# BogdanDIA/gr-dvbt

Measured on AMD Instinct MI355X. Metric: RX Msamples/s (baseband in -> TS out), higher is better.
Workload: dtype u8 (Viterbi/RS) + f32 (front end)

## Files before the change

gr_dvbt_amd/csrc/dvbt_blocks.inc:

```

namespace {

struct PinBuf {
  void *p = nullptr; size_t cap = 0;
  int reserve(size_t n) { if (n <= cap) return DVBT_OK; if (p) (void)hipHostFree(p); p = nullptr; cap = 0; HIPCHK(hipHostMalloc(&p, n + 64)); cap = n; return DVBT_OK; }
  ~PinBuf() { if (p) (void)hipHostFree(p); }
};
struct BlockCtx {
  hipStream_t s = nullptr; DevBuf din, dout, aux; PinBuf pin_in, pin_out;
  struct Pending { void *host; size_t off, bytes; };
  std::vector<Pending> pending; size_t pin_in_used = 0, pin_out_used = 0;
  int init() { int r = need_device(); if (r) return r; HIPCHK(hipStreamCreate(&s)); return DVBT_OK; }
  static bool is_pinned(const void *host)
  {
    hipPointerAttribute_t a;
    if (hipPointerGetAttributes(&a, host) != hipSuccess) { (void)hipGetLastError(); return false; }
    return a.type == hipMemoryTypeHost;
  }
  int put(DevBuf &b, const void *host, size_t bytes, size_t offset = 0)
  {
    int r = b.reserve(offset + bytes); if (r) return r;
    if (!bytes) return DVBT_OK;
    if (is_pinned(host)) { HIPCHK(hipMemcpyAsync((char *)b.p + offset, host, bytes, hipMemcpyHostToDevice, s)); return DVBT_OK; }
    if (pin_in_used + bytes > pin_in.cap) {
// ... 177 lines not shown
  if (n > 4096) return fail(DVBT_ERR_CAPACITY, "at most 4096 items per call");
  WCHK(h->c.aux.reserve(64 * 4096 * 4));
  HIPCHK(hipMemcpyAsync((char *)h->c.aux.p + slot, h->idx.data(), (size_t)n * 4, hipMemcpyHostToDevice, s));
  InnerParams ip; memset(&ip, 0, sizeof ip); ip.payload = (int)P; ip.m = 4;
  hipLaunchKernelGGL(inner_kernel<2>, dim3(n), dim3(INNER_THREADS), inner_lds_bytes(P), s, (const float2 *)nullptr, (const uint8_t *)din, ip,
                     (const RxState *)nullptr, n, (const int *)((char *)h->c.aux.p + slot), (const float2 *)nullptr, (const unsigned char *)nullptr,
                     (const uint16_t *)h->T.H, (const uint16_t *)h->T.Hinv, (uint8_t *)nullptr, (uint8_t *)nullptr, (uint8_t *)dout);
  return DVBT_OK;
}
extern "C" int dvbt_symbol_inner_interleaver_work(dvbt_symbol_inner_interleaver *h, int nout, int nin, const void *in, void *out, dvbt_sideband *sb)
{
  if (!h || !in || !out) return fail(DVBT_ERR_INVALID, "null argument");
  sb_begin(sb);
  int n = nout < nin ? nout : nin; if (n <= 0) return 0;
  size_t P = h->p.nsize;
  WCHK(sym_indices(h, n, sb));
  WCHK(h->c.put(h->c.din, in, (size_t)n * P)); WCHK(h->c.dout.reserve((size_t)n * P));
  WCHK(sym_run(h, n, h->c.din.p, h->c.dout.p, h->c.s));
  WCHK(h->c.get(out, h->c.dout.p, (size_t)n * P)); WCHK(h->c.sync());
  if (sb) sb->n_consumed = n;
  return n;
}
extern "C" int dvbt_symbol_inner_interleaver_work_device(dvbt_symbol_inner_interleaver *h, int nout, int nin, const void *in, void *out, dvbt_sideband *sb, void *stream)
{
  if (!h || !in || !out) return fail(DVBT_ERR_INVALID, "null argument");
  sb_begin(sb);
  int n = nout < nin ? nout : nin; if (n <= 0) return 0;
  WCHK(sym_indices(h, n, sb));
  WCHK(sym_run(h, n, in, out, pick(stream, h->c)));
  if (sb) sb->n_consumed = n;
  return n;
}
extern "C" void dvbt_symbol_inner_interleaver_destroy(dvbt_symbol_inner_interleaver *h) { delete h; }

struct dvbt_bit_inner_deinterleaver { dvbt_bit_inner_deinterleaver_params p; BlockCtx c; Dims d; };
extern "C" int dvbt_bit_inner_deinterleaver_create(const dvbt_bit_inner_deinterleaver_params *p, dvbt_bit_inner_deinterleaver **out)
{
  BLK_CREATE_PROLOGUE(dvbt_bit_inner_deinterleaver);
  h->p = *p;
  h->d = make_dims(p->constellation, p->hierarchy, 0, 0, p->transmission_mode);
  if (!h->d.valid || p->nsize <= 0 || p->nsize % 126 || p->nsize > 49152) BLK_FAIL(DVBT_ERR_INVALID, "nsize must be a positive multiple of 126");
  if (p->hierarchy != DVBT_NH && h->d.m == 2) BLK_FAIL(DVBT_ERR_INVALID, "hierarchical QPSK does not exist (the reference's constructor divides by d_v - 2 = 0)");
  *out = h; return DVBT_OK;
}
extern "C" int dvbt_bit_inner_deinterleaver_forecast(const dvbt_bit_inner_deinterleaver *, int n, int *req) { if (req) *req = n; return DVBT_OK; }
static void bit_run(dvbt_bit_inner_deinterleaver *h, int n, const void *din, void *dout, hipStream_t s, void *dout_lp = nullptr)
{
  const size_t P = h->p.nsize;
  InnerParams ip; memset(&ip, 0, sizeof ip); ip.payload = (int)P; ip.m = h->d.m; ip.hier = h->p.hierarchy != DVBT_NH ? 1 : 0;
  hipLaunchKernelGGL(inner_kernel<4>, dim3(n), dim3(INNER_THREADS), inner_lds_bytes(P), s, (const float2 *)nullptr, (const uint8_t *)din, ip,
                     (const RxState *)nullptr, n, (const int *)nullptr, (const float2 *)nullptr, (const unsigned char *)nullptr,
                     (const uint16_t *)nullptr, (const uint16_t *)nullptr, (uint8_t *)nullptr, (uint8_t *)nullptr, (uint8_t *)dout, (uint8_t *)dout_lp);
}
extern "C" int dvbt_bit_inner_deinterleaver_work_hier(dvbt_bit_inner_deinterleaver *h, int nout, int nin, const void *in, void *out_hp, void *out_lp, dvbt_sideband *sb)
{
  if (!h || !in || !out_hp || !out_lp) return fail(DVBT_ERR_INVALID, "null argument");
  if (h->p.hierarchy == DVBT_NH) return fail(DVBT_ERR_STATE, "a non-hierarchical bit_inner_deinterleaver has one output");
  sb_begin(sb);
  int n = nout < nin ? nout : nin; if (n <= 0) return 0;
  size_t P = h->p.nsize;
  WCHK(h->c.put(h->c.din, in, (size_t)n * P)); WCHK(h->c.dout.reserve((size_t)n * P)); WCHK(h->c.aux.reserve((size_t)n * P));
  bit_run(h, n, h->c.din.p, h->c.dout.p, h->c.s, h->c.aux.p);
  WCHK(h->c.get(out_hp, h->c.dout.p, (size_t)n * P)); WCHK(h->c.get(out_lp, h->c.aux.p, (size_t)n * P)); WCHK(h->c.sync());
  if (sb) sb->n_consumed = n;
  return n;
}
extern "C" int dvbt_bit_inner_deinterleaver_work_hier_device(dvbt_bit_inner_deinterleaver *h, int nout, int nin, const void *in, void *out_hp, void *out_lp, dvbt_sideband *sb, void *stream)
{
  if (!h || !in || !out_hp || !out_lp) return fail(DVBT_ERR_INVALID, "null argument");
  if (h->p.hierarchy == DVBT_NH) return fail(DVBT_ERR_STATE, "a non-hierarchical bit_inner_deinterleaver has one output");
  sb_begin(sb);
  int n = nout < nin ? nout : nin; if (n <= 0) return 0;
  bit_run(h, n, in, out_hp, pick(stream, h->c), out_lp);
  if (sb) sb->n_consumed = n;
  return n;
}
extern "C" int dvbt_bit_inner_deinterleaver_work(dvbt_bit_inner_deinterleaver *h, int nout, int nin, const void *in, void *out, dvbt_sideband *sb)
{
  if (!h || !in || !out) return fail(DVBT_ERR_INVALID, "null argument");
  sb_begin(sb);
  int n = nout < nin ? nout : nin; if (n <= 0) return 0;
  size_t P = h->p.nsize;
  WCHK(h->c.put(h->c.din, in, (size_t)n * P)); WCHK(h->c.dout.reserve((size_t)n * P));
  bit_run(h, n, h->c.din.p, h->c.dout.p, h->c.s);
  WCHK(h->c.get(out, h->c.dout.p, (size_t)n * P)); WCHK(h->c.sync());
  if (sb) sb->n_consumed = n;
  return n;
}
extern "C" int dvbt_bit_inner_deinterleaver_work_device(dvbt_bit_inner_deinterleaver *h, int nout, int nin, const void *in, void *out, dvbt_sideband *sb, void *stream)
{
  if (!h || !in || !out) return fail(DVBT_ERR_INVALID, "null argument");
  sb_begin(sb);
  int n = nout < nin ? nout : nin; if (n <= 0) return 0;
  bit_run(h, n, in, out, pick(stream, h->c));
  if (sb) sb->n_consumed = n;
  return n;
}
extern "C" void dvbt_bit_inner_deinterleaver_destroy(dvbt_bit_inner_deinterleaver *h) { delete h; }

struct dvbt_viterbi_decoder {
  dvbt_viterbi_decoder_params p; BlockCtx c; Dims d; VitParams vp;
  size_t hist = 0; long long in_total = 0, steps = 0; int d_init = 0;
  static constexpr size_t kTail = 8192;
  VitProof proof; int *carry = nullptr; int cur = 0; bool have_carry = false; long long grid0 = 0;
  ~dvbt_viterbi_decoder() { if (carry) (void)hipFree(carry); }
};
extern "C" int dvbt_viterbi_decoder_create(const dvbt_viterbi_decoder_params *p, dvbt_viterbi_decoder **out)
{
  BLK_CREATE_PROLOGUE(dvbt_viterbi_decoder);
  h->p = *p;
  h->d = make_dims(p->constellation, p->hierarchy, p->code_rate, 0, 0);
  if (!h->d.valid || p->bsize <= 0 || (2 * h->d.k * p->bsize) % 16 || (p->bsize * h->d.n) % h->d.m || (p->bsize * h->d.k) % 8)
    BLK_FAIL(DVBT_ERR_INVALID, "bsize must make bsize*n/m and bsize*k/8 integral and 2*k*bsize a multiple of 16");
  h->vp = make_vit_params(h->d, p->bsize, 11 * V3_BLK);
  if (hipMalloc((void **)&h->carry, 2 * V3_SLOT * sizeof(int)) != hipSuccess) BLK_FAIL(DVBT_ERR_HIP, "hipMalloc (viterbi_decoder carry)");
  BLK_CHK(h->proof.reserve(256));
  *out = h; return DVBT_OK;
}
extern "C" int dvbt_viterbi_decoder_forecast(const dvbt_viterbi_decoder *h, int n, int *req)
{ if (!h || !req) return DVBT_ERR_INVALID; *req = n * 8 * h->d.n / (h->d.k * h->d.m); return DVBT_OK; }
static int viterbi_call(dvbt_viterbi_decoder *h, int nout, int nin, const void *in, void *out, dvbt_sideband *sb, bool dev, hipStream_t s)
{
  sb_begin(sb);
  const int d_nout = h->vp.d_nbits / 16, d_nsym = h->vp.d_nsymbols;
  int nblocks = nout / d_nout;
  if (nblocks * d_nsym > nin) nblocks = nin / d_nsym;
  if (nblocks <= 0) return 0;
  const dvbt_tag *t = find_tag(sb, DVBT_TAG_SUPERFRAME_START, 0, (int64_t)nblocks * d_nsym);
  if (t) {
    h->d_init = 0; h->steps = 0; h->in_total = 0; h->hist = 0; h->have_carry = false; h->grid0 = 0;
    if (t->rel_offset > 0) { if (sb) sb->n_consumed = (int)t->rel_offset; return 0; }
    HIPCHK(hipMemsetAsync(h->proof.ctl + V3_CTL_ACC, 0, 3 * sizeof(int), s));
  }
  const size_t nbytes = (size_t)nblocks * d_nsym, hist = h->hist;
  WCHK(h->c.din.reserve_keep(dvbt_viterbi_decoder::kTail + nbytes + 64, hist, s));
  if (dev) WCHK(h->c.put_dev(h->c.din, in, nbytes, hist, s)); else { HIPCHK(hipMemcpyAsync((char *)h->c.din.p + hist, in, nbytes, hipMemcpyHostToDevice, s)); }
  const long long in_base = h->in_total - (long long)hist;
  long long out_lo = h->steps / 8 - h->d.ntb; if (out_lo < 0) out_lo = 0;
  h->steps += (long long)nblocks * (h->vp.d_nbits / 2);
  h->in_total += (long long)nbytes;
  long long out_hi = h->steps / 8 - h->d.ntb; if (out_hi < 0) out_hi = 0;
  const long long produced = out_hi - out_lo;
  if (produced > 0) {
    uint8_t *o = (uint8_t *)out;
    if (!dev) { WCHK(h->c.dout.reserve((size_t)produced)); o = (uint8_t *)h->c.dout.p; }
    const int B = h->vp.chunk_bytes;
    const long long g0 = h->have_carry ? h->grid0 : 0, chunks = (out_hi - g0 + B - 1) / B;
    if (chunks + 2 > h->proof.cap) { HIPCHK(hipStreamSynchronize(s)); int acc[3]; HIPCHK(hipMemcpy(acc, h->proof.ctl + V3_CTL_ACC, sizeof acc, hipMemcpyDeviceToHost));
                                     WCHK(h->proof.reserve(2 * chunks + 2)); HIPCHK(hipMemcpy(h->proof.ctl + V3_CTL_ACC, acc, sizeof acc, hipMemcpyHostToDevice)); }
    V3Aux ax = h->proof.aux();
    ax.grid0 = g0; ax.carry_in = h->have_carry ? h->carry + h->cur * V3_SLOT : nullptr;
    const long long b0_last = g0 + (chunks - 1) * B;
    ax.carry_rel = (int)((out_hi - b0_last) / V3_BLK) * V3_BLK; ax.carry_out = h->carry + (h->cur ^ 1) * V3_SLOT;
    launch_viterbi(s, (const uint8_t *)h->c.din.p, o, (const RxState *)nullptr, h->steps, h->vp, in_base, out_lo, produced, &ax, VIT_REPAIR);
    h->cur ^= 1; h->have_carry = true; h->grid0 = b0_last + ax.carry_rel;
    if (!dev) WCHK(h->c.get(out, h->c.dout.p, (size_t)produced));
  }
  {
    const size_t total = hist + nbytes, keep = total < dvbt_viterbi_decoder::kTail ? total : dvbt_viterbi_decoder::kTail;
    if (total > keep) {
      WCHK(h->c.aux.reserve(dvbt_viterbi_decoder::kTail));
      HIPCHK(hipMemcpyAsync(h->c.aux.p, (const char *)h->c.din.p + total - keep, keep, hipMemcpyDeviceToDevice, s));
      HIPCHK(hipMemcpyAsync(h->c.din.p, h->c.aux.p, keep, hipMemcpyDeviceToDevice, s));
    }
    h->hist = keep;
  }
  if (!dev) WCHK(h->c.sync());
  if (h->d_init == 0) { add_tag(sb, 0, DVBT_TAG_SUPERFRAME_START, 1); h->d_init = 1; }
  if (sb) sb->n_consumed = (int)nbytes;
  return (int)produced;
}
extern "C" int dvbt_viterbi_decoder_work(dvbt_viterbi_decoder *h, int nout, int nin, const void *in, void *out, dvbt_sideband *sb)
{
  if (!h || !in || !out) return fail(DVBT_ERR_INVALID, "null argument");
  return viterbi_call(h, nout, nin, in, out, sb, false, h->c.s);
}
extern "C" int dvbt_viterbi_decoder_work_device(dvbt_viterbi_decoder *h, int nout, int nin, const void *in, void *out, dvbt_sideband *sb, void *stream)
{
  if (!h || !in || !out) return fail(DVBT_ERR_INVALID, "null argument");
  return viterbi_call(h, nout, nin, in, out, sb, true, pick(stream, h->c));
}
extern "C" int dvbt_viterbi_decoder_set_warm_windows(dvbt_viterbi_decoder *h, int windows)
{
  if (!h) return fail(DVBT_ERR_INVALID, "null handle");
  if (windows == 0) windows = V3_WARM;
  if (windows < 2 * V3_BLK || windows > 576 || windows % V3_BLK != 0) return fail(DVBT_ERR_INVALID, "warm-up must be 0 (default) or a multiple of 24 in [48, 576]");
  h->vp.warm = windows;
  return DVBT_OK;
}
extern "C" int dvbt_viterbi_decoder_proof(dvbt_viterbi_decoder *h, dvbt_viterbi_proof *out)
{
  if (!h || !out) return fail(DVBT_ERR_INVALID, "null argument");
  int acc[3] = {0, 0, 0};
  HIPCHK(hipMemcpy(acc, h->proof.ctl + V3_CTL_ACC, sizeof acc, hipMemcpyDeviceToHost));
  out->chunks = acc[0]; out->decoded_again = acc[1]; out->sequential = acc[2]; out->not_proven = -1;
  return DVBT_OK;
}
extern "C" void dvbt_viterbi_decoder_destroy(dvbt_viterbi_decoder *h) { delete h; }

struct dvbt_convolutional_deinterleaver { dvbt_convolutional_deinterleaver_params p; BlockCtx c; size_t hist = 0; long long pos = 0; };
extern "C" int dvbt_convolutional_deinterleaver_create(const dvbt_convolutional_deinterleaver_params *p, dvbt_convolutional_deinterleaver **out)
{
  BLK_CREATE_PROLOGUE(dvbt_convolutional_deinterleaver);
  h->p = *p;
  if (p->I != 12 || p->M != 17 || p->blocks != 136) BLK_FAIL(DVBT_ERR_INVALID, "only the DVB-T outer interleaver I=12, M=17, blocks=136 (every RX flowgraph; assert at convolutional_deinterleaver_impl.cc:68)");
  *out = h; return DVBT_OK;
}
extern "C" int dvbt_convolutional_deinterleaver_forecast(const dvbt_convolutional_deinterleaver *h, int n, int *req)
{ if (!h || !req) return DVBT_ERR_INVALID; *req = n * h->p.I * h->p.blocks; return DVBT_OK; }
static int convdeint_call(dvbt_convolutional_deinterleaver *h, int nout, int nin, const void *in, void *out, dvbt_sideband *sb, bool dev, hipStream_t s)
{
  sb_begin(sb);
  const int item = h->p.I * h->p.blocks;
  int n = nout & ~1;
  if ((long long)n * item > nin) n = (nin / item) & ~1;
  if (n <= 0) return 0;
  const dvbt_tag *t = find_tag(sb, DVBT_TAG_SUPERFRAME_START, 0, (int64_t)n * item);
  if (t && t->rel_offset > 0) { if (sb) sb->n_consumed = (int)t->rel_offset; return 0; }
  const size_t nbytes = (size_t)n * item, hist = h->hist, keep_max = 2244;
  WCHK(h->c.din.reserve_keep(keep_max + nbytes + 64, hist, s));
  if (dev) WCHK(h->c.put_dev(h->c.din, in, nbytes, hist, s)); else { HIPCHK(hipMemcpyAsync((char *)h->c.din.p + hist, in, nbytes, hipMemcpyHostToDevice, s)); }
  uint8_t *o = (uint8_t *)out;
  if (!dev) { WCHK(h->c.dout.reserve(nbytes)); o = (uint8_t *)h->c.dout.p; }
  hipLaunchKernelGGL(conv_deint_kernel, dim3(512), dim3(256), 0, s, (const uint8_t *)h->c.din.p, (long long)hist, h->pos, (long long)nbytes, o);
  if (!dev) WCHK(h->c.get(out, h->c.dout.p, nbytes));
  h->pos += (long long)nbytes;
  {
    const size_t total = hist + nbytes, keep = total < keep_max ? total : keep_max;
    if (total > keep) {
      WCHK(h->c.aux.reserve(keep_max));
      HIPCHK(hipMemcpyAsync(h->c.aux.p, (const char *)h->c.din.p + total - keep, keep, hipMemcpyDeviceToDevice, s));
      HIPCHK(hipMemcpyAsync(h->c.din.p, h->c.aux.p, keep, hipMemcpyDeviceToDevice, s));
    }
    h->hist = keep;
  }
  if (!dev) WCHK(h->c.sync());
  if (sb) sb->n_consumed = (int)nbytes;
  return n;
}
extern "C" int dvbt_convolutional_deinterleaver_work(dvbt_convolutional_deinterleaver *h, int nout, int nin, const void *in, void *out, dvbt_sideband *sb)
{
  if (!h || !in || !out) return fail(DVBT_ERR_INVALID, "null argument");
  return convdeint_call(h, nout, nin, in, out, sb, false, h->c.s);
}
extern "C" int dvbt_convolutional_deinterleaver_work_device(dvbt_convolutional_deinterleaver *h, int nout, int nin, const void *in, void *out, dvbt_sideband *sb, void *stream)
{
  if (!h || !in || !out) return fail(DVBT_ERR_INVALID, "null argument");
  return convdeint_call(h, nout, nin, in, out, sb, true, pick(stream, h->c));
}
extern "C" void dvbt_convolutional_deinterleaver_destroy(dvbt_convolutional_deinterleaver *h) { delete h; }

struct dvbt_reed_solomon_dec { dvbt_reed_solomon_dec_params p; BlockCtx c; Tables T; int *cnt = nullptr; ~dvbt_reed_solomon_dec() { if (cnt) (void)hipFree(cnt); } };
extern "C" int dvbt_reed_solomon_dec_create(const dvbt_reed_solomon_dec_params *p, dvbt_reed_solomon_dec **out)
{
  BLK_CREATE_PROLOGUE(dvbt_reed_solomon_dec);
  h->p = *p;
  if (p->p != 2 || p->m != 8 || p->gfpoly != 0x11d || p->n != 255 || p->k != 239 || p->t != 8 || p->s != 51 || p->blocks <= 0)
    BLK_FAIL(DVBT_ERR_INVALID, "only RS(255,239,t=8) over GF(2^8)/0x11d shortened by 51 (the DVB-T outer code)");
  BLK_CHK(h->T.build_rs());
  if (hipMalloc((void **)&h->cnt, 8) != hipSuccess || hipMemset(h->cnt, 0, 8) != hipSuccess) BLK_FAIL(DVBT_ERR_HIP, "hipMalloc");
  *out = h; return DVBT_OK;
}
extern "C" int dvbt_reed_solomon_dec_forecast(const dvbt_reed_solomon_dec *, int n, int *req) { if (req) *req = n; return DVBT_OK; }
static void rs_run(dvbt_reed_solomon_dec *h, long long words, const void *din, void *dout, hipStream_t s)
{
  hipLaunchKernelGGL(deint_rs_kernel, dim3((unsigned)((words + 63) / 64)), dim3(64), 0, s, (const uint8_t *)din, (uint8_t *)nullptr,
                     (uint8_t *)dout, (RxState *)nullptr, words, 1, 0ll, h->T.rs_tables(), h->p.oracle_compat, h->cnt, h->cnt + 1);
}
extern "C" int dvbt_reed_solomon_dec_work(dvbt_reed_solomon_dec *h, int nout, int nin, const void *in, void *out, dvbt_sideband *sb)
{
  if (!h || !in || !out) return fail(DVBT_ERR_INVALID, "null argument");
  sb_begin(sb);
  int n = nout < nin ? nout : nin; if (n <= 0) return 0;
  long long words = (long long)n * h->p.blocks;
  WCHK(h->c.put(h->c.din, in, (size_t)words * 204)); WCHK(h->c.dout.reserve((size_t)words * 188));
  rs_run(h, words, h->c.din.p, h->c.dout.p, h->c.s);
  WCHK(h->c.get(out, h->c.dout.p, (size_t)words * 188)); WCHK(h->c.sync());
  if (sb) sb->n_consumed = n;
  return n;
}
extern "C" int dvbt_reed_solomon_dec_work_device(dvbt_reed_solomon_dec *h, int nout, int nin, const void *in, void *out, dvbt_sideband *sb, void *stream)
{
  if (!h || !in || !out) return fail(DVBT_ERR_INVALID, "null argument");
  sb_begin(sb);
  int n = nout < nin ? nout : nin; if (n <= 0) return 0;
  rs_run(h, (long long)n * h->p.blocks, in, out, pick(stream, h->c));
  if (sb) sb->n_consumed = n;
  return n;
}
extern "C" void dvbt_reed_solomon_dec_destroy(dvbt_reed_solomon_dec *h) { delete h; }

struct dvbt_energy_descramble { dvbt_energy_descramble_params p; BlockCtx c; Tables T; int d_index = 0; RxState *dstate = nullptr; unsigned ring = 0; ~dvbt_energy_descramble() { if (dstate) (void)hipFree(dstate); } };
extern "C" int dvbt_energy_descramble_create(const dvbt_energy_descramble_params *p, dvbt_energy_descramble **out)
{
  BLK_CREATE_PROLOGUE(dvbt_energy_descramble);
  h->p = *p;
  BLK_CHK(h->T.build_rs());
  *out = h; return DVBT_OK;
}
extern "C" int dvbt_energy_descramble_forecast(const dvbt_energy_descramble *, int n, int *req) { if (req) *req = 4 * (n / 1504); return DVBT_OK; }
static int descramble_call(dvbt_energy_descramble *h, int nout, int nin, const void *in, void *out, dvbt_sideband *sb, bool dev, hipStream_t s)
{
  sb_begin(sb);
  nout -= nout % (4 * 1504);
  if (nout <= 0 || nin < nout / 1504) return 0;
  uint8_t probe[16];
  if (dev) {
// ... 261 lines not shown
```

gr_dvbt_amd/csrc/dvbt_hip.hip:

```cpp
#include <hip/hip_runtime.h>
#include <cstdio>
#include <cstdarg>
#include <cstdlib>
#include <cstring>
#include <string>
#include <vector>
#include <map>
#include <deque>
#include <algorithm>
#include "../../include/dvbt_hip.h"
#include "dvbt_tables.hpp"
#include "ts_ring.hpp"
#include "k_frontend.hpp"
#include "k_drift.hpp"
#include "k_backend.hpp"
#include "k_symbol8k.hpp"
#include "k_symbol2k.hpp"
#include "k_resample.hpp"
#include "k_viterbi3.hpp"
#include "k_soft4.hpp"
#include "k_tx.hpp"
#include "k_txblocks.hpp"

using namespace dvbt;
// ... 31 lines not shown
  o->fft_length = d.N; o->cp_length = d.cp; o->Kmax = d.Kmax; o->payload_length = d.payload; o->zeros_on_left = d.zl;
  o->m = d.m; o->cr_k = d.k; o->cr_n = d.n; o->norm = d.norm; o->ntraceback = d.ntb; o->info_bits_per_symbol = d.info_bits_per_symbol;
  return DVBT_OK;
}

template <class T> static int upload(const std::vector<T> &v, T **dptr)
{
  HIPCHK(hipMalloc((void **)dptr, v.size() * sizeof(T) + 16));
  HIPCHK(hipMemcpy(*dptr, v.data(), v.size() * sizeof(T), hipMemcpyHostToDevice));
  return DVBT_OK;
}

struct DevBuf {
  void *p = nullptr; size_t cap = 0;
  int reserve(size_t n) { if (n <= cap) return DVBT_OK; if (p) (void)hipFree(p); p = nullptr; cap = 0; HIPCHK(hipMalloc(&p, n + 64)); cap = n; return DVBT_OK; }
  int reserve_keep(size_t n, size_t keep, hipStream_t st)
  {
    if (n <= cap) return DVBT_OK;
    void *q = nullptr; HIPCHK(hipMalloc(&q, n + 64));
    if (p && keep) HIPCHK(hipMemcpyAsync(q, p, keep, hipMemcpyDeviceToDevice, st));
    if (p) { HIPCHK(hipStreamSynchronize(st)); (void)hipFree(p); }
    p = q; cap = n; return DVBT_OK;
  }
  ~DevBuf() { if (p) (void)hipFree(p); }
};

struct Tables {
  Dims d;
  float2 *tw = nullptr; uint16_t *perm = nullptr;
  int16_t *cpilot = nullptr, *tps = nullptr; float *known = nullptr, *pref = nullptr;
  uint16_t *pay_c = nullptr, *pay_L = nullptr, *pay_R = nullptr, *tps_L = nullptr, *tps_R = nullptr;
  uint16_t *pil_k = nullptr, *pay_Li = nullptr, *pay_Ri = nullptr, *tps_Li = nullptr, *tps_Ri = nullptr; uint8_t *pay_d = nullptr, *tps_d = nullptr; int np[4] = {0, 0, 0, 0};
  uint16_t *tps_bch = nullptr;
  uint32_t *pay_pack = nullptr;
  uint16_t *H = nullptr, *Hinv = nullptr; float2 *points = nullptr; uint8_t *label_tab = nullptr; int nlev = 0; float inv_step = 0.f, guard = 0.f, hshift = 0.f;
  uint8_t *mul_alpha = nullptr, *gexp = nullptr, *glog = nullptr, *prbs = nullptr;
  bool front = false, inner = false, rs = false;

  int build_fft(int N)
  {
    std::vector<float> tw_h = fft_twiddles(N);
    std::vector<float2> t2(N);
    for (int i = 0; i < N; i++) t2[i] = make_float2(tw_h[2 * i], tw_h[2 * i + 1]);
    int r = upload(t2, &tw); if (r) return r;
    return upload(fft_out_perm(N), &perm);
  }
  int build_front()
  {
    std::vector<int> c = cpilot_table(d), t = tps_table(d);
    std::vector<int16_t> c16(c.begin(), c.end()), t16(t.begin(), t.end());
    std::vector<float> pr = pilot_ref_table(d), kn(d.n_cp - 1);
    for (int i = 0; i + 1 < d.n_cp; i++) { float df = pr[c[i + 1]] - pr[c[i]]; kn[i] = df * df; }
    int r;
    if ((r = upload(c16, &cpilot)) || (r = upload(t16, &tps)) || (r = upload(pr, &pref)) || (r = upload(kn, &known))) return r;
    std::vector<uint16_t> pc, pl, prr, tl, trr, pk((size_t)4 * DEMOD_NP, 0), pli, pri, tli, tri;
    std::vector<uint8_t> pd, td;
    std::vector<uint32_t> pp;
    for (int s = 0; s < 4; s++) {
      PatternTables pt = pattern_tables(d, s);
      if ((int)pt.pay_c.size() != d.payload) return fail(DVBT_ERR_INVALID, "payload carrier table size mismatch");
      if ((int)pt.pil_k.size() > DEMOD_NP) return fail(DVBT_ERR_INVALID, "estimation carrier table overflow");
      np[s] = (int)pt.pil_k.size();
      for (size_t i = 0; i < pt.pil_k.size(); i++) pk[(size_t)s * DEMOD_NP + i] = (uint16_t)(pt.pil_k[i] | (pr[pt.pil_k[i]] < 0.f ? 0x8000 : 0));
      pli.insert(pli.end(), pt.pay_Li.begin(), pt.pay_Li.end()); pri.insert(pri.end(), pt.pay_Ri.begin(), pt.pay_Ri.end());
      pd.insert(pd.end(), pt.pay_d.begin(), pt.pay_d.end());
      for (size_t i = 0; i < pt.pay_c.size(); i++) pp.push_back((uint32_t)pt.pay_c[i] | ((uint32_t)pt.pay_Li[i] << 13) | ((uint32_t)pt.pay_d[i] << 23));
      tli.insert(tli.end(), pt.tps_Li.begin(), pt.tps_Li.end()); tri.insert(tri.end(), pt.tps_Ri.begin(), pt.tps_Ri.end());
      td.insert(td.end(), pt.tps_d.begin(), pt.tps_d.end());
      pc.insert(pc.end(), pt.pay_c.begin(), pt.pay_c.end()); pl.insert(pl.end(), pt.pay_L.begin(), pt.pay_L.end());
      prr.insert(prr.end(), pt.pay_R.begin(), pt.pay_R.end()); tl.insert(tl.end(), pt.tps_L.begin(), pt.tps_L.end());
      trr.insert(trr.end(), pt.tps_R.begin(), pt.tps_R.end());
    }
    if ((r = upload(pc, &pay_c)) || (r = upload(pl, &pay_L)) || (r = upload(prr, &pay_R)) || (r = upload(tl, &tps_L)) || (r = upload(trr, &tps_R))) return r;
    if ((r = upload(pk, &pil_k)) || (r = upload(pli, &pay_Li)) || (r = upload(pri, &pay_Ri)) || (r = upload(pd, &pay_d)) || (r = upload(tli, &tps_Li)) ||
        (r = upload(tri, &tps_Ri)) || (r = upload(td, &tps_d)) || (r = upload(pp, &pay_pack))) return r;
    if ((r = upload(tps_bch_table_host(), &tps_bch))) return r;
    front = true;
    return DVBT_OK;
  }
  int build_inner(float gain)
  {
    int r;
    if (!H) {
      std::vector<uint16_t> h = symbol_H(d), hi(h.size());
      for (size_t q = 0; q < h.size(); q++) hi[h[q]] = (uint16_t)q;
      if ((r = upload(h, &H)) || (r = upload(hi, &Hinv))) return r;
    }
    std::vector<float> p = constellation_points(d, gain);
    std::vector<float2> p2(64, make_float2(0.f, 0.f));
    for (int i = 0; i < d.csize; i++) p2[i] = make_float2(p[2 * i], p[2 * i + 1]);
    std::vector<uint8_t> lab(64, 0);
    nlev = 0; hshift = 0.f;
    if (gain > 0.f) {
      int n = 1 << (d.m / 2);
      float step = 2.0f * gain * d.norm;
      const float sh = (float)(d.alpha - 1) * gain * d.norm;
      bool ok = true;
      for (int i = 0; i < d.csize && ok; i++) {
        const float ux = p2[i].x - (p2[i].x > 0 ? sh : -sh), uy = p2[i].y - (p2[i].y > 0 ? sh : -sh);
        float fi = ux / step + 0.5f * (n - 1), fq = uy / step + 0.5f * (n - 1);
        int ii = (int)std::lround(fi), qq = (int)std::lround(fq);
        if (ii < 0 || ii >= n || qq < 0 || qq >= n || std::fabs(fi - ii) > 1e-3f || std::fabs(fq - qq) > 1e-3f) ok = false;
        else lab[ii * 8 + qq] = (uint8_t)i;
      }
      if (ok) { nlev = n; inv_step = 1.0f / step; guard = 1.0e4f * step; hshift = sh; }
    }
    if (points) { (void)hipFree(points); points = nullptr; }
    if (label_tab) { (void)hipFree(label_tab); label_tab = nullptr; }
    if ((r = upload(p2, &points)) || (r = upload(lab, &label_tab))) return r;
    inner = true;
    return DVBT_OK;
  }
  InnerParams inner_params(int payload) const { InnerParams ip; ip.payload = payload; ip.m = d.m; ip.csize = d.csize; ip.nlev = nlev; ip.inv_step = inv_step; ip.guard = guard;
                                                  ip.hshift = hshift; ip.hier = d.hierarchy != 0 ? 1 : 0; return ip; }
  int build_rs()
  {
    std::vector<uint8_t> ex(512), lg(256), mul = rs_division_table();
    gf_tables(ex.data(), lg.data());
    int r;
    if ((r = upload(ex, &gexp)) || (r = upload(lg, &glog)) || (r = upload(mul, &mul_alpha)) || (r = upload(energy_prbs(), &prbs))) return r;
    rs = true;
    return DVBT_OK;
  }
  DemodTables demod_tables() const { DemodTables T; T.cpilot = cpilot; T.known_diff = known; T.tps = tps; T.pilot_ref = pref;
    T.pay_c = pay_c; T.pay_L = pay_L; T.pay_R = pay_R; T.tps_L = tps_L; T.tps_R = tps_R;
    T.pil_k = pil_k; for (int i = 0; i < 4; i++) T.np[i] = np[i];
    T.pay_Li = pay_Li; T.pay_Ri = pay_Ri; T.pay_d = pay_d; T.tps_Li = tps_Li; T.tps_Ri = tps_Ri; T.tps_d = tps_d; T.pay_pack = pay_pack; return T; }
  RsTables rs_tables() const { RsTables T; T.div_tab = mul_alpha; T.gexp = gexp; T.glog = glog; return T; }
  ~Tables()
  {
    void *all[] = {tw, perm, cpilot, tps, known, pref, pay_c, pay_L, pay_R, tps_L, tps_R, pil_k, pay_Li, pay_Ri, pay_d, tps_Li, tps_Ri, tps_d, pay_pack, tps_bch, H, Hinv, points, label_tab, mul_alpha, gexp, glog, prbs};
    for (void *q : all) if (q) (void)hipFree(q);
  }
};

#define V3_NTB_SWITCH(ntb, CALL) switch (ntb) { case 5: CALL(5); break; case 9: CALL(9); break; case 10: CALL(10); break; case 15: CALL(15); break; default: CALL(24); break; }
struct VitProof {
  int *snap = nullptr, *ctl = nullptr; long long cap = 0;
  int reserve(long long chunks)
  {
    if (chunks <= cap) return DVBT_OK;
    if (snap) (void)hipFree(snap); if (ctl) (void)hipFree(ctl);
    snap = ctl = nullptr; cap = 0;
    HIPCHK(hipMalloc((void **)&snap, v3_snap_words(chunks) * sizeof(int))); HIPCHK(hipMalloc((void **)&ctl, v3_ctl_words(chunks) * sizeof(int)));
    HIPCHK(hipMemset(ctl, 0, v3_ctl_words(chunks) * sizeof(int)));
    cap = chunks; return DVBT_OK;
  }
  V3Aux aux() const { V3Aux a; memset(&a, 0, sizeof a); a.snap = snap; a.ctl = ctl; a.cap = cap; a.carry_rel = -1; return a; }
  ~VitProof() { if (snap) (void)hipFree(snap); if (ctl) (void)hipFree(ctl); }
};
enum { VIT_PLAIN = -1, VIT_REPAIR = 0, VIT_REPAIR_COUNT = 1, VIT_PROOF_ONLY = 2, VIT_FORCE_SEQ = 3, VIT_FORCE_CONFLICT = 4 };
constexpr unsigned V3_REPAIR_GRID = 64;

static void launch_viterbi(hipStream_t s, const uint8_t *in, uint8_t *out, const RxState *st, long long steps_fixed, const VitParams &vp,
                           long long in_base, long long out_lo, long long max_out_bytes, const V3Aux *ax = nullptr, int mode = VIT_PLAIN)
{
  const bool proof = ax && mode != VIT_PLAIN;
  const long long grid0 = proof ? ax->grid0 : out_lo;
  long long chunks = (out_lo + max_out_bytes - grid0 + vp.chunk_bytes - 1) / vp.chunk_bytes;
  if (chunks < 1) chunks = 1;
  const dim3 grid((unsigned)((chunks + 4 * V3_WGW - 1) / (4 * V3_WGW))), blk(64 * V3_WGW);
  V3Aux none; memset(&none, 0, sizeof none);
  if (proof) {
    V3Aux a = *ax;
    if (mode == VIT_FORCE_CONFLICT) { a.debug = 1; mode = VIT_REPAIR_COUNT; }
    const dim3 cgrid((unsigned)((chunks + 255) / 256));
    if (vp.warm == V3_WARM) {
#define V3_CALL(N) hipLaunchKernelGGL((viterbi3_kernel<N, V3_WARM, 1>), grid, blk, 0, s, in, out, st, steps_fixed, vp, a, in_base, out_lo)
      V3_NTB_SWITCH(vp.ntb, V3_CALL)
#undef V3_CALL
    } else {
#define V3_CALL(N) hipLaunchKernelGGL((viterbi3_kernel<N, 0, 1>), grid, blk, 0, s, in, out, st, steps_fixed, vp, a, in_base, out_lo)
      V3_NTB_SWITCH(vp.ntb, V3_CALL)
#undef V3_CALL
    }
    if (chunks <= V3_FIX_SMALL && mode != VIT_PROOF_ONLY) {
#define V3_CALL(N) hipLaunchKernelGGL(viterbi_fix_kernel<N>, dim3(1), blk, 0, s, in, out, st, steps_fixed, vp, a, in_base, out_lo, mode == VIT_FORCE_SEQ ? 1 : 0)
      V3_NTB_SWITCH(vp.ntb, V3_CALL)
#undef V3_CALL
      if (mode != VIT_REPAIR) {
        hipLaunchKernelGGL(viterbi_check_kernel, dim3(1), dim3(256), 0, s, a, st, steps_fixed, vp, 1);
        hipLaunchKernelGGL(viterbi_count_kernel, cgrid, dim3(256), 0, s, a, st, steps_fixed, vp);
      }
      return;
    }
    hipLaunchKernelGGL(viterbi_check_kernel, cgrid, dim3(256), 0, s, a, st, steps_fixed, vp, 0);
    if (mode == VIT_REPAIR || mode == VIT_REPAIR_COUNT) {
#define V3_CALL(N) hipLaunchKernelGGL(viterbi_repair_kernel<N>, dim3(V3_REPAIR_GRID), blk, 0, s, in, out, st, steps_fixed, vp, a, in_base, out_lo)
      V3_NTB_SWITCH(vp.ntb, V3_CALL)
#undef V3_CALL
    }
    if (mode != VIT_PROOF_ONLY) {
      const int force = mode == VIT_FORCE_SEQ ? 1 : 0;
#define V3_CALL(N) hipLaunchKernelGGL(viterbi_repair_seq_kernel<N>, dim3(1), dim3(64), 0, s, in, out, st, steps_fixed, vp, a, in_base, out_lo, force)
      V3_NTB_SWITCH(vp.ntb, V3_CALL)
#undef V3_CALL
    }
    if (mode != VIT_REPAIR) {
      hipLaunchKernelGGL(viterbi_check_kernel, dim3(1), dim3(256), 0, s, a, st, steps_fixed, vp, 1);
      hipLaunchKernelGGL(viterbi_count_kernel, cgrid, dim3(256), 0, s, a, st, steps_fixed, vp);
    }
    return;
  }
  if (vp.warm != V3_WARM) {
#define V3_CALL(N) hipLaunchKernelGGL((viterbi3_kernel<N, 0, 0>), grid, blk, 0, s, in, out, st, steps_fixed, vp, none, in_base, out_lo)
    V3_NTB_SWITCH(vp.ntb, V3_CALL)
#undef V3_CALL
    return;
  }
#define V3_CALL(N) hipLaunchKernelGGL((viterbi3_kernel<N, V3_WARM, 0>), grid, blk, 0, s, in, out, st, steps_fixed, vp, none, in_base, out_lo)
  V3_NTB_SWITCH(vp.ntb, V3_CALL)
#undef V3_CALL
}

__global__ void tail_patch_kernel(RxState *st, long long items)
{
  st->n_rs_items = items; st->n_rs_words = items * 8; st->stream_rs_items = items;
  st->rs_fail = 0; st->rs_corr = 0; st->rs_list_n = 0; st->sym_off = 0;
}

static FrontParams make_front_params(const Dims &d, float snr_db)
{
  FrontParams p; memset(&p, 0, sizeof p);
  p.N = d.N; p.cp = d.cp; p.K = d.K; p.zl = d.zl; p.payload = d.payload; p.n_cp = d.n_cp; p.n_tps = d.n_tps; p.fi_start = d.fi_start;
  p.R = ACQ_R;
  float snr = (float)pow(10, snr_db / 10.0);
  float rho = (float)(snr / (snr + 1.0));
  p.half_rho = (float)(rho / 2.0);
  return p;
}
static int set_lds(const void *fn, size_t bytes)
{
  if (bytes > 48 * 1024) HIPCHK(hipFuncSetAttribute(fn, hipFuncAttributeMaxDynamicSharedMemorySize, (int)bytes));
  return DVBT_OK;
}

enum { ST_ACQ = 0, ST_FFT, ST_DEMOD, ST_INNER, ST_VIT, ST_RS, ST_END, ST_COUNT };
static const char *kStageNames[] = {"acq", "fft", "demod", "inner", "viterbi", "rs"};

struct ResamplerDesign {
  int ri = 0, rd = 0, nt = 0; std::vector<float> taps; float *br = nullptr;
  int build(int interp, int decim)
  {
    if (interp <= 0 || decim <= 0) return fail(DVBT_ERR_INVALID, "bad resampler ratio");
    taps = resampler_taps(interp, decim, ri, rd);
    std::vector<float> b = resampler_branches(taps, ri, nt);
    if ((long long)ri * nt > RS_MAX_BRANCH_FLOATS || 256ll * rd / ri + nt + 2 > RS_TILE_IN) return fail(DVBT_ERR_INVALID, "resampler ratio outside the supported range");
    HIPCHK(hipMalloc((void **)&br, b.size() * sizeof(float)));
    HIPCHK(hipMemcpy(br, b.data(), b.size() * sizeof(float), hipMemcpyHostToDevice));
    return DVBT_OK;
  }
  ~ResamplerDesign() { if (br) (void)hipFree(br); }
};

struct dvbt_rx {
  dvbt_rx_params prm; Dims d; Tables T; FrontParams fp; VitParams vp;
  hipStream_t own_stream = nullptr, cur_stream = nullptr;
  hipStream_t front_stream = nullptr; hipEvent_t front_ev[2] = {nullptr, nullptr};
  size_t max_samples = 0; int max_calls = 0;
  float2 *d_iq = nullptr;
  ResamplerDesign rsd; float2 *rs_iq = nullptr; size_t chain_max = 0;
  AcqState *acq_carry = nullptr; bool use_carry = false;
  float2 *g_init = nullptr; float *l_init = nullptr; float2 *g_trk = nullptr; float *l_trk = nullptr;
  SymMeta *meta = nullptr; RxState *st = nullptr, *st_host = nullptr; TpsState *tps_state = nullptr;
  static constexpr int NCTX = 3;
  RxState *st_ctx[NCTX] = {nullptr, nullptr, nullptr}; SymMeta *meta_ctx[NCTX] = {nullptr, nullptr, nullptr}; int ctx = 0;
  int *trk_flags_ctx[NCTX] = {nullptr, nullptr, nullptr}, *sym_ticket_ctx[NCTX] = {nullptr, nullptr, nullptr}, *drift_flags_ctx[NCTX] = {nullptr, nullptr, nullptr}; RxState *st_host_ctx[NCTX] = {nullptr, nullptr, nullptr};
  hipStream_t aux_stream = nullptr; hipEvent_t aux_ev = nullptr;
  int *trk_cp_a = nullptr, *trk_cp_b = nullptr, *trk_flags = nullptr; float *trk_eps = nullptr; TpsEdge *tps_edges = nullptr;
  int *centre = nullptr, *anchor_pos = nullptr;
  float2 *acq_tap = nullptr, *fft_out = nullptr, *eq = nullptr, *tpsval = nullptr; SymInfo *info = nullptr; int *maj = nullptr, *sym_index = nullptr;
  uint8_t *labels = nullptr, *symdeint_tap = nullptr, *bitdeint = nullptr, *vit = nullptr, *deint_tap = nullptr, *rs_out = nullptr, *ts_out = nullptr;
  uint8_t *bitdeint_lp = nullptr;
  uint8_t *bd_log = nullptr; std::vector<dvbt_period_tap> plog; size_t plog_bytes = 0;
  VitProof vproof; bool vit_checked = false;
  size_t vit_cap = 0; RsDefer *rs_defer = nullptr; int rs_defer_cap = 0;
  unsigned long long *rs_sync = nullptr;
  unsigned soft_grid = 0;
  float *csi = nullptr; int8_t *soft_a = nullptr; uint16_t *soft_tab = nullptr; unsigned *soft_scratch = nullptr;
  int timing = 0;
  bool pending = false;
  hipEvent_t ev[ST_COUNT]; double acc_ms[ST_COUNT] = {0}; long n_timed = 0; bool ev_ready = false, ev_recorded = false;
  dvbt_rx_report last; bool have_last = false;
  dvbt_rx_cut cut = {0, 0, 0};
  float2 *tps_prev = nullptr, *tps_prev_snap[2] = {nullptr, nullptr}; TpsState *tps_snap[2] = {nullptr, nullptr};  DescrRun *descr_runs = nullptr; int *descr_nruns = nullptr;
  int n_periods = 1; size_t seg_offset = 0;
  std::vector<dvbt_lock_period> periods;
  DriftBufs drift = {nullptr, nullptr, nullptr, nullptr, nullptr, nullptr, nullptr, nullptr}; double *drift_mem = nullptr;
  struct GraphEntry { const void *iq; size_t n; hipStream_t s; long long sym_off; int delay, phase; hipGraphExec_t exec; };
  std::vector<GraphEntry> graphs;
  int ncu = 256;
  long long n_small = 0, n_general = 0;
  int sym_grid = 512;
  int *sym_ticket = nullptr;
};

constexpr long long kVitMaxChunk = 3000;
static int vit_chunk_bytes(const dvbt_rx *h, long long max_vit);

static void drop_graphs(dvbt_rx *h)
{
  for (auto &ge : h->graphs) if (ge.exec) (void)hipGraphExecDestroy(ge.exec);
  h->graphs.clear();
}

static void rx_free(dvbt_rx *h)
{
  void *all[] = {h->bd_log, h->bitdeint_lp, h->st_ctx[0], h->st_ctx[1], h->st_ctx[2], h->meta_ctx[0], h->meta_ctx[1], h->meta_ctx[2], h->tps_prev_snap[0], h->tps_prev_snap[1], h->tps_snap[0], h->tps_snap[1], h->csi, h->soft_a, h->soft_tab, h->soft_scratch, h->rs_defer, h->rs_sync, h->drift_mem, h->drift.delta, h->drift_flags_ctx[0], h->drift_flags_ctx[1], h->drift_flags_ctx[2], h->tps_prev, h->descr_runs, h->descr_nruns, h->centre, h->anchor_pos, h->sym_ticket_ctx[0], h->sym_ticket_ctx[1], h->sym_ticket_ctx[2], h->tps_edges, h->trk_cp_a, h->trk_cp_b, h->trk_flags_ctx[0], h->trk_flags_ctx[1], h->trk_flags_ctx[2], h->trk_eps, h->d_iq, h->rs_iq, h->acq_carry, h->g_init, h->l_init, h->g_trk, h->l_trk, h->tps_state, h->acq_tap, h->fft_out, h->eq, h->tpsval,
                 h->info, h->maj, h->sym_index, h->labels, h->symdeint_tap, h->bitdeint, h->vit, h->deint_tap, h->rs_out, h->ts_out};
  for (void *q : all) if (q) (void)hipFree(q);
  for (auto &ge : h->graphs) if (ge.exec) (void)hipGraphExecDestroy(ge.exec);
  for (int i = 0; i < dvbt_rx::NCTX; i++) if (h->st_host_ctx[i]) (void)hipHostFree(h->st_host_ctx[i]);
  if (h->aux_ev) (void)hipEventDestroy(h->aux_ev);
  if (h->aux_stream) (void)hipStreamDestroy(h->aux_stream);
  if (h->ev_ready) for (int i = 0; i < ST_COUNT; i++) (void)hipEventDestroy(h->ev[i]);
  if (h->own_stream) (void)hipStreamDestroy(h->own_stream);
  for (int i = 0; i < 2; i++) if (h->front_ev[i]) (void)hipEventDestroy(h->front_ev[i]);
  if (h->front_stream) (void)hipStreamDestroy(h->front_stream);
  delete h;
}

extern "C" int dvbt_rx_create(const dvbt_rx_params *p, dvbt_rx **out)
{
  if (!p || !out) return fail(DVBT_ERR_INVALID, "null argument");
  int r = need_device(); if (r) return r;
  Dims d = make_dims(p->constellation, p->hierarchy, p->code_rate, p->guard_interval, p->transmission_mode);
  if (!d.valid) return fail(DVBT_ERR_INVALID, "bad DVB-T parameters");
  if (p->viterbi_bsize <= 0 || (2 * d.k * p->viterbi_bsize) % 16 != 0 || (p->viterbi_bsize * d.n) % d.m != 0)
    return fail(DVBT_ERR_INVALID, "viterbi_bsize must make bsize*n/m integral and 2*k*bsize a multiple of 16");
  if (d.hierarchy != 0 && d.m == 2) return fail(DVBT_ERR_INVALID, "hierarchical QPSK does not exist (the reference's bit_inner_deinterleaver divides by d_v - 2 = 0 in its constructor)");
  if (d.hierarchy != 0 && p->soft_decision) return fail(DVBT_ERR_INVALID, "soft decisions are built for the non-hierarchical modes");
  if (p->hier_stream < 0 || p->hier_stream > 1) return fail(DVBT_ERR_INVALID, "hier_stream must be 0 (HP) or 1 (LP)");
  if (p->viterbi_warm_windows != 0 && (p->viterbi_warm_windows < 2 * V3_BLK || p->viterbi_warm_windows > V3_WARM_MAX || p->viterbi_warm_windows % V3_BLK != 0))
    return fail(DVBT_ERR_INVALID, "viterbi_warm_windows must be 0 (default) or a multiple of 24 in [48, 1152]");
  if (p->viterbi_warm_windows != 0 && p->soft_decision) return fail(DVBT_ERR_INVALID, "viterbi_warm_windows applies to the hard-decision decoder");
  if (p->viterbi_verify < VIT_PLAIN || p->viterbi_verify > VIT_FORCE_CONFLICT) return fail(DVBT_ERR_INVALID, "viterbi_verify must lie in [-1, 4]");
  if (p->viterbi_verify > 0 && p->soft_decision) return fail(DVBT_ERR_INVALID, "viterbi_verify applies to the hard-decision decoder");
  HIPCHK(hipSetDevice(p->device));
  dvbt_rx *h = new dvbt_rx();
  h->prm = *p; h->d = d; h->T.d = d;
  size_t chain_max = p->max_samples;
  if (p->resample_interp > 0 || p->resample_decim > 0) {
    int r2 = h->rsd.build(p->resample_interp, p->resample_decim); if (r2) { delete h; return r2; }
    chain_max = (size_t)(((unsigned long long)p->max_samples * h->rsd.ri + h->rsd.rd - 1) / h->rsd.rd);
  }
  if (chain_max < (size_t)(2 * d.N + d.cp + 16)) { delete h; return fail(DVBT_ERR_INVALID, "max_samples smaller than one acquisition window"); }
  h->chain_max = chain_max;
  h->fp = make_front_params(d, p->snr_db);
  int cb = p->viterbi_chunk_bytes > 0 ? p->viterbi_chunk_bytes : 768;
  h->vp = make_vit_params(d, p->viterbi_bsize, cb);
  if (p->viterbi_warm_windows > 0) h->vp.warm = p->viterbi_warm_windows;
  h->max_samples = p->max_samples;
  h->max_calls = (int)((chain_max - (2 * d.N + d.cp + 16)) / (d.N + d.cp) + 1);
#define RXCHK(x) do { int r_ = (x); if (r_) { rx_free(h); return r_; } } while (0)
#define RXHIP(x) do { hipError_t e_ = (x); if (e_ != hipSuccess) { g_err = std::string(#x) + ": " + hipGetErrorString(e_); rx_free(h); return DVBT_ERR_HIP; } } while (0)
  RXCHK(h->T.build_fft(d.N)); RXCHK(h->T.build_front()); RXCHK(h->T.build_inner(1.0f)); RXCHK(h->T.build_rs());
  RXHIP(hipStreamCreate(&h->own_stream));
  if (p->front_priority) {
    int least = 0, greatest = 0; RXHIP(hipDeviceGetStreamPriorityRange(&least, &greatest));
    RXHIP(hipStreamCreateWithPriority(&h->front_stream, hipStreamNonBlocking, greatest));
    for (int i = 0; i < 2; i++) RXHIP(hipEventCreateWithFlags(&h->front_ev[i], hipEventDisableTiming));
  }
  if (h->rsd.ri) RXHIP(hipMalloc((void **)&h->rs_iq, sizeof(float2) * (chain_max + 16)));
  const size_t C = (size_t)h->max_calls, N = d.N, P = d.payload;
  RXHIP(hipMalloc((void **)&h->g_init, sizeof(float2) * ACQ_INIT_TRIES_MAX * N)); RXHIP(hipMalloc((void **)&h->l_init, sizeof(float) * ACQ_INIT_TRIES_MAX * N));
  RXHIP(hipMalloc((void **)&h->g_trk, sizeof(float2) * C * 2 * ACQ_R)); RXHIP(hipMalloc((void **)&h->l_trk, sizeof(float) * C * 2 * ACQ_R));
  for (int i = 0; i < dvbt_rx::NCTX; i++) { RXHIP(hipMalloc((void **)&h->meta_ctx[i], sizeof(SymMeta) * C)); RXHIP(hipMalloc((void **)&h->st_ctx[i], sizeof(RxState))); RXHIP(hipMemset(h->st_ctx[i], 0, sizeof(RxState))); }
  h->meta = h->meta_ctx[0]; h->st = h->st_ctx[0]; h->ctx = 0;
  RXHIP(hipMalloc((void **)&h->trk_cp_a, sizeof(int) * C)); RXHIP(hipMalloc((void **)&h->trk_cp_b, sizeof(int) * C));
  RXHIP(hipMalloc((void **)&h->trk_eps, sizeof(float) * C));
  for (int i = 0; i < dvbt_rx::NCTX; i++) { RXHIP(hipMalloc((void **)&h->trk_flags_ctx[i], sizeof(int) * 16)); RXHIP(hipMemset(h->trk_flags_ctx[i], 0, sizeof(int) * 16)); }
  h->trk_flags = h->trk_flags_ctx[0];
  RXHIP(hipStreamCreate(&h->aux_stream)); RXHIP(hipEventCreateWithFlags(&h->aux_ev, hipEventDisableTiming));
  RXHIP(hipMalloc((void **)&h->tps_prev, sizeof(float2) * d.n_tps)); RXHIP(hipMemset(h->tps_prev, 0, sizeof(float2) * d.n_tps));
  for (int i = 0; i < 2; i++) { RXHIP(hipMalloc((void **)&h->tps_prev_snap[i], sizeof(float2) * d.n_tps)); RXHIP(hipMalloc((void **)&h->tps_snap[i], sizeof(TpsState))); }
  RXHIP(hipMalloc((void **)&h->descr_runs, sizeof(DescrRun) * DESCR_MAX_RUNS)); RXHIP(hipMalloc((void **)&h->descr_nruns, sizeof(int)));
  RXHIP(hipMalloc((void **)&h->centre, sizeof(int) * (C + 1))); RXHIP(hipMalloc((void **)&h->anchor_pos, sizeof(int) * (C / ACQ_ANCHOR + 4)));
  RXHIP(hipMalloc((void **)&h->tps_edges, sizeof(TpsEdge) * (C / TPS_SEG + 2)));
  for (int i = 0; i < dvbt_rx::NCTX; i++) { RXHIP(hipHostMalloc((void **)&h->st_host_ctx[i], sizeof(RxState))); memset(h->st_host_ctx[i], 0, sizeof(RxState)); }
  h->st_host = h->st_host_ctx[0];
  RXHIP(hipMalloc((void **)&h->acq_carry, sizeof(AcqState))); RXHIP(hipMalloc((void **)&h->tps_state, sizeof(TpsState)));
  RXHIP(hipMalloc((void **)&h->labels, C * P + 64));
  RXHIP(hipMalloc((void **)&h->tpsval, sizeof(float2) * C * d.n_tps)); RXHIP(hipMalloc((void **)&h->info, sizeof(SymInfo) * C));
  RXHIP(hipMalloc((void **)&h->maj, sizeof(int) * C)); RXHIP(hipMalloc((void **)&h->sym_index, sizeof(int) * C));
  RXHIP(hipMalloc((void **)&h->bitdeint, C * P + 64));
  if (d.hierarchy != 0) RXHIP(hipMalloc((void **)&h->bitdeint_lp, C * P + 64));
  { int ncu = 256; (void)hipDeviceGetAttribute(&ncu, hipDeviceAttributeMultiprocessorCount, h->prm.device); h->sym_grid = s8_grid(ncu); h->ncu = ncu; }
  if (p->viterbi_verify != VIT_PLAIN && !p->soft_decision) {
    const long long mv = (long long)C * P * d.m * d.k / (8 * d.n) + 1;
    long long chunks;
    if (p->viterbi_chunk_bytes > 0) chunks = mv / vit_chunk_bytes(h, mv) + 2;
    else { const long long slots = (long long)h->ncu * V3_WAVES_PER_CU * 4; chunks = slots * ((mv + slots * kVitMaxChunk - 1) / (slots * kVitMaxChunk)) + 4; }
    RXCHK(h->vproof.reserve(chunks));
  }
  h->vit_cap = C * P * d.m * d.k / (8 * d.n) + 4096 + (2u << 20);
  h->rs_defer_cap = (int)((h->vit_cap / 204 / 64 + 2) * (RS_LANE_MIN - 1));
  RXHIP(hipMalloc((void **)&h->rs_defer, sizeof(RsDefer) * (size_t)h->rs_defer_cap));
  RXHIP(hipMalloc((void **)&h->rs_sync, sizeof(unsigned long long) * (h->vit_cap / 204 / 64 + 2)));
  RXHIP(hipMalloc((void **)&h->vit, h->vit_cap)); RXHIP(hipMalloc((void **)&h->rs_out, h->vit_cap)); RXHIP(hipMalloc((void **)&h->ts_out, h->vit_cap));
  RXHIP(hipMemset(h->st, 0, sizeof(RxState)));
  for (int i = 0; i < ST_COUNT; i++) RXHIP(hipEventCreate(&h->ev[i]));
  h->ev_ready = true;
  for (int i = 0; i < dvbt_rx::NCTX; i++) { RXHIP(hipMalloc((void **)&h->sym_ticket_ctx[i], 64)); RXHIP(hipMemset(h->sym_ticket_ctx[i], 0, 64)); }
  h->sym_ticket = h->sym_ticket_ctx[0];
  if (p->soft_decision) {
    RXHIP(hipMalloc((void **)&h->eq, sizeof(float2) * C * P)); RXHIP(hipMalloc((void **)&h->csi, sizeof(float) * C * P));
    RXHIP(hipMalloc((void **)&h->soft_a, C * P * d.m + 64)); RXHIP(hipMalloc((void **)&h->soft_tab, sizeof(uint16_t) * 2 * P * d.m));
    const long long max_vit_soft = (long long)C * P * d.m * d.k / (8 * d.n) + 1;
    h->soft_grid = s4_grid_bound(max_vit_soft);
    RXHIP(hipMalloc((void **)&h->soft_scratch, sizeof(unsigned) * (size_t)h->soft_grid * S4_WAVES * S4_SLOT_WORDS));
    hipLaunchKernelGGL(soft_tab_kernel, dim3(64), dim3(256), 0, h->own_stream, h->T.inner_params(d.payload), (const uint16_t *)h->T.H, (const uint16_t *)h->T.Hinv, h->soft_tab);
    RXHIP(hipStreamSynchronize(h->own_stream));
  }
  {
    RXHIP(hipMalloc((void **)&h->drift_mem, sizeof(double) * (C * (DRIFT_TAB + 4) + 8)));
    h->drift.tabs = h->drift_mem; h->drift.ex_run = h->drift.tabs + C * DRIFT_TAB; h->drift.ex_entry = h->drift.ex_run + C;
    h->drift.d = h->drift.ex_entry + C; h->drift.S = h->drift.d + C; h->drift.A0 = h->drift.S + C;
    RXHIP(hipMalloc((void **)&h->drift.delta, sizeof(float) * C * (N / 32))); for (int i = 0; i < dvbt_rx::NCTX; i++) { RXHIP(hipMalloc((void **)&h->drift_flags_ctx[i], 16)); RXHIP(hipMemset(h->drift_flags_ctx[i], 0, 16)); }
    h->drift.flags = h->drift_flags_ctx[0];
  }
  RXCHK(set_lds((const void *)symbol8k_kernel<false, false>, S8_LDS_BYTES)); RXCHK(set_lds((const void *)symbol8k_kernel<false, true>, S8_LDS_BYTES));
  RXCHK(set_lds((const void *)symbol8k_kernel<true, false>, S8_LDS_BYTES)); RXCHK(set_lds((const void *)symbol8k_kernel<true, true>, S8_LDS_BYTES));
  RXCHK(set_lds((const void *)symbol2k_kernel<false, false>, S2_LDS_BYTES)); RXCHK(set_lds((const void *)symbol2k_kernel<false, true>, S2_LDS_BYTES));
  RXCHK(set_lds((const void *)symbol2k_kernel<true, false>, S2_LDS_BYTES)); RXCHK(set_lds((const void *)symbol2k_kernel<true, true>, S2_LDS_BYTES));
  RXCHK(set_lds((const void *)inner_kernel<6>, inner_lds_bytes(P)));
  RXCHK(set_lds((const void *)acq_anchor_kernel, acq_anchor_lds_bytes((int)N, d.cp)));
  RXCHK(set_lds((const void *)acq_small_kernel, (size_t)acq_small_cpc(d.cp) * 2 * (d.cp + 2 * ACQ_R) * sizeof(float2)));
  *out = h;
  return DVBT_OK;
}

extern "C" int dvbt_rx_set_cut(dvbt_rx *h, const dvbt_rx_cut *cut)
{
  if (!h || !cut) return fail(DVBT_ERR_INVALID, "null argument");
  if (cut->stream_symbol_offset < 0 || cut->stream_symbol_offset % 272) return fail(DVBT_ERR_INVALID, "stream_symbol_offset must be a non-negative multiple of 272 (whole superframes)");
  if (cut->start_delay_symbols < 0 || cut->start_delay_symbols >= 272 || cut->descr_call_phase < 0 || cut->descr_call_phase > 16) return fail(DVBT_ERR_INVALID, "start_delay_symbols must lie in [0, 272), descr_call_phase in [0, 16]");
  h->cut = *cut;
  return DVBT_OK;
}

extern "C" int dvbt_rx_enable_timing(dvbt_rx *h, int enable)
{
  if (!h) return DVBT_ERR_INVALID;
  h->timing = enable == 2 ? 2 : (enable != 0 ? 1 : 0);
  drop_graphs(h);
  if (enable) { for (int i = 0; i <= ST_END; i++) h->acc_ms[i] = 0.0; h->n_timed = 0; }
  return DVBT_OK;
}

static int rx_reserve_vit(dvbt_rx *h, size_t cap)
{
  if (cap <= h->vit_cap) return DVBT_OK;
  HIPCHK(hipDeviceSynchronize());
  drop_graphs(h);
  const size_t old = h->vit_cap;
  uint8_t **bufs[] = {&h->vit, &h->rs_out, &h->ts_out, &h->deint_tap};
  for (uint8_t **b : bufs) {
    if (!*b) continue;
    uint8_t *q = nullptr; HIPCHK(hipMalloc((void **)&q, cap));
    HIPCHK(hipMemcpy(q, *b, old, hipMemcpyDeviceToDevice));
    (void)hipFree(*b); *b = q;
  }
  const int dcap = (int)((cap / 204 / 64 + 2) * (RS_LANE_MIN - 1));
  { RsDefer *q = nullptr; HIPCHK(hipMalloc((void **)&q, sizeof(RsDefer) * (size_t)dcap)); (void)hipFree(h->rs_defer); h->rs_defer = q; h->rs_defer_cap = dcap; }
  { unsigned long long *q = nullptr; HIPCHK(hipMalloc((void **)&q, sizeof(unsigned long long) * (cap / 204 / 64 + 2)));
    HIPCHK(hipMemcpy(q, h->rs_sync, sizeof(unsigned long long) * (old / 204 / 64 + 2), hipMemcpyDeviceToDevice)); (void)hipFree(h->rs_sync); h->rs_sync = q; }
  h->vit_cap = cap;
  return DVBT_OK;
}

static int ensure_taps(dvbt_rx *h)
{
  const size_t C = (size_t)h->max_calls, N = h->d.N, P = h->d.payload;
  if (!h->acq_tap) HIPCHK(hipMalloc((void **)&h->acq_tap, sizeof(float2) * C * N));
  if (!h->fft_out) HIPCHK(hipMalloc((void **)&h->fft_out, sizeof(float2) * C * N));
  if (!h->eq) HIPCHK(hipMalloc((void **)&h->eq, sizeof(float2) * C * P));
  if (!h->symdeint_tap) HIPCHK(hipMalloc((void **)&h->symdeint_tap, C * P + 64));
  if (!h->deint_tap) HIPCHK(hipMalloc((void **)&h->deint_tap, h->vit_cap));
  return DVBT_OK;
}
extern "C" int dvbt_rx_enable_taps(dvbt_rx *h, int enable)
{
  if (!h) return DVBT_ERR_INVALID;
  if (h->pending) return fail(DVBT_ERR_STATE, "dvbt_rx_enable_taps: a segment is in flight (dvbt_rx_segment_finish first)");
  drop_graphs(h);
  if (enable == 2 && !h->bd_log) HIPCHK(hipMalloc((void **)&h->bd_log, (size_t)h->max_calls * h->d.payload + 64));
  if (enable) return ensure_taps(h);
  if (h->bd_log) { (void)hipFree(h->bd_log); h->bd_log = nullptr; }
  void **all[] = {(void **)&h->acq_tap, (void **)&h->fft_out, h->prm.soft_decision ? (void **)nullptr : (void **)&h->eq, (void **)&h->symdeint_tap, (void **)&h->deint_tap};
  for (void **q : all) if (q && *q) { (void)hipFree(*q); *q = nullptr; }
  return DVBT_OK;
}

struct EnqOpt {
  bool acq_only = false;
  int init_tries = ACQ_INIT_TRIES;
  bool skip_acq = false;
  bool use_carry = false;
  float carry_avg = 0.f;
  long long hist = 0;
  bool continuation = false;
  bool keep_last = false;
  size_t vit_off = 0;
  bool tail = true;
  long long avail = 0;
  bool no_small = false;
  bool tps_init = false;
  bool cut_set = false;
  long long sym_off = 0; int delay = 0;
};

static int prepare_chain(dvbt_rx *h, const float2 *iq, size_t nsamples, hipStream_t s, const float2 **chain, size_t *chain_n)
{
  if (nsamples > h->max_samples) return fail(DVBT_ERR_CAPACITY, "segment longer than max_samples");
  *chain = iq; *chain_n = nsamples;
  if (h->rsd.ri) {
    const long long cnt = (long long)(((unsigned long long)nsamples * h->rsd.ri + h->rsd.rd - 1) / h->rsd.rd);
    hipLaunchKernelGGL(resample_scale_kernel, dim3((unsigned)((cnt + 255) / 256)), dim3(256), 0, s, iq, 0ll, (long long)nsamples, 0ll, cnt, h->rsd.ri, h->rsd.rd,
                       h->rsd.nt, (const float *)h->rsd.br, h->prm.front_scale == 0.f ? 1.0f : h->prm.front_scale, h->rs_iq);
    *chain = h->rs_iq; *chain_n = (size_t)cnt;
  }
  return DVBT_OK;
}

static int vit_chunk_bytes(const dvbt_rx *h, long long max_vit)
{
  long long B = h->prm.viterbi_chunk_bytes;
  if (B <= 0) {
    const long long slots = (long long)h->ncu * V3_WAVES_PER_CU * 4;
    long long rounds = (max_vit + slots * kVitMaxChunk - 1) / (slots * kVitMaxChunk);
    if (rounds < 1) rounds = 1;
    B = (max_vit + slots * rounds - 1) / (slots * rounds);
    if (B < 256) B = 256;
  }
  if (h->prm.viterbi_verify != VIT_PLAIN && !h->prm.soft_decision) B = std::min<long long>((B + V3_BLK - 1) / V3_BLK * V3_BLK, (1ll << 30) / V3_BLK * V3_BLK);
  return (int)B;
}

static int enqueue_tail(dvbt_rx *h, hipStream_t s, long long max_words, long long words_fixed)
{
  if (words_fixed >= 0) {
    const long long items = (words_fixed / 8) & ~1ll;
    hipLaunchKernelGGL(tail_patch_kernel, dim3(1), dim3(1), 0, s, h->st, items);
  }
  hipLaunchKernelGGL(deint_rs_kernel, dim3((unsigned)((max_words + 63) / 64)), dim3(64), 0, s, (const uint8_t *)h->vit, h->deint_tap, h->rs_out,
                     h->st, 0ll, 0, 0ll, h->T.rs_tables(), h->prm.rs_oracle_compat, &h->st->rs_fail, &h->st->rs_corr, h->rs_defer, &h->st->rs_list_n, h->rs_defer_cap,
                     h->rs_sync);
  hipLaunchKernelGGL(rs_fix_kernel, dim3(512), dim3(64), 0, s, (const RsDefer *)h->rs_defer, (const int *)&h->st->rs_list_n, h->rs_defer_cap, h->rs_out,
                     h->T.rs_tables(), h->prm.rs_oracle_compat, &h->st->rs_fail, &h->st->rs_corr, h->rs_sync);
  if (h->prm.descramble) {
    hipLaunchKernelGGL(descramble_scan_kernel, dim3(1), dim3(1024), 0, s, (const uint8_t *)h->rs_out, h->st, h->descr_runs, h->descr_nruns,
                       (const unsigned long long *)h->rs_sync, h->cut.descr_call_phase - 1);
    hipLaunchKernelGGL(descramble_runs_kernel, dim3(1024), dim3(256), 0, s, (const uint8_t *)h->rs_out, (const uint8_t *)h->T.prbs,
                       (const RxState *)h->st, (const DescrRun *)h->descr_runs, (const int *)h->descr_nruns, h->ts_out);
  }
  return DVBT_OK;
}

static int enqueue(dvbt_rx *h, const float2 *iq, size_t nsamples, hipStream_t s, const EnqOpt &o = EnqOpt())
{
  const Dims &d = h->d;
  if (nsamples > h->chain_max) return fail(DVBT_ERR_CAPACITY, "segment longer than max_samples");
  if (nsamples < (size_t)(2 * d.N + d.cp + 16)) return fail(DVBT_ERR_INVALID, "segment shorter than one acquisition window");
  FrontParams fp = h->fp;
  const long long cut_sym_off = o.cut_set ? o.sym_off : (long long)h->cut.stream_symbol_offset;
  const int cut_delay = o.cut_set ? o.delay : h->cut.start_delay_symbols;
  fp.hunt_known = cut_delay > 0 ? 1 : 0;
  fp.si_start = cut_delay % 68; fp.fi_start = (d.fi_start + cut_delay / 68) % 4;
  fp.ncalls = (int)((nsamples - (2 * d.N + d.cp + 16)) / (d.N + d.cp) + 1);
  fp.hist = o.hist; fp.keep_last = o.keep_last ? 1 : 0; fp.avail = o.avail > 0 ? o.avail : (long long)nsamples;
  const int C = fp.ncalls, N = d.N;
  h->cur_stream = s;
  hipStream_t const s_user = s;
  const bool split = h->front_stream && !o.acq_only && !o.skip_acq && !o.continuation && h->timing != 1 && C >= 512 && !h->prm.launch_graph;
  if (split) { HIPCHK(hipEventRecord(h->front_ev[0], s_user)); HIPCHK(hipStreamWaitEvent(h->front_stream, h->front_ev[0], 0)); s = h->front_stream; }
  auto join_front = [&]() -> int { if (split && s != s_user) { HIPCHK(hipEventRecord(h->front_ev[1], s)); s = s_user; HIPCHK(hipStreamWaitEvent(s, h->front_ev[1], 0)); } return DVBT_OK; };
  const bool tm = h->timing == 1 && !o.acq_only, tmv = h->timing != 0 && !o.acq_only;
  if (tm) HIPCHK(hipEventRecord(h->ev[ST_ACQ], s));
  if (o.skip_acq) {
    if (!o.continuation && !o.tps_init) HIPCHK(hipMemsetAsync(h->tps_state, 0, sizeof(TpsState), s));
  } else {
  const AcqState *carry = nullptr;
  int tries = C < o.init_tries ? C : o.init_tries;
  hipLaunchKernelGGL(acq_metric_kernel, dim3((N + 255) / 256, tries), dim3(256), 0, s, iq, fp, (const RxState *)h->st, 0, h->g_init, h->l_init, 0);
  const AcqReset rz = {h->trk_flags, h->sym_ticket, (o.acq_only || o.continuation || o.tps_init) ? nullptr : reinterpret_cast<int *>(h->tps_state), (int)(sizeof(TpsState) / 4),
                       o.carry_avg, o.use_carry ? 1 : 0};
  hipLaunchKernelGGL(acq_init_fsm_kernel, dim3(1), dim3(1024), (size_t)N * 5, s, fp, h->st, (const float2 *)h->g_init, (const float *)h->l_init, carry, 0, tries, rz);
  if (o.acq_only && !o.no_small && C <= ACQ_SMALL_MAX_CALLS) {
    const int cpc = acq_small_cpc(d.cp);
    h->n_small++;
    hipLaunchKernelGGL(acq_small_kernel, dim3(1), dim3(64 * (1 + cpc / 2)), (size_t)cpc * 2 * (d.cp + 2 * ACQ_R) * sizeof(float2), s, iq, fp, h->st, h->meta, cpc, h->drift.flags);
  } else {
  if (o.acq_only) h->n_general++;
  {
    const int n_anchors = (C - 1) / ACQ_ANCHOR;
    if (n_anchors > 0) hipLaunchKernelGGL(acq_anchor_kernel, dim3(n_anchors), dim3(1024), acq_anchor_lds_bytes(N, d.cp), s, iq, fp, (const RxState *)h->st, h->anchor_pos);
    hipLaunchKernelGGL(acq_centre_kernel, dim3((C + 1023) / 1024), dim3(1024), 0, s, fp, (const RxState *)h->st, (const int *)h->anchor_pos, n_anchors, h->centre);
  }
  hipLaunchKernelGGL(acq_track_metric_kernel, dim3((C + ACQ_TM_CALLS - 1) / ACQ_TM_CALLS), dim3(256), 0, s, iq, fp, (const RxState *)h->st, (const int *)h->centre, h->g_trk, h->l_trk);
  constexpr int kIters = TRK_ROUNDS;
  hipLaunchKernelGGL(acq_track_fused_kernel, dim3((C + TRK_OWN - 1) / TRK_OWN), dim3(256), 0, s, fp, (const RxState *)h->st, (const float2 *)h->g_trk,
                     (const float *)h->l_trk, h->trk_cp_a, h->trk_eps, h->trk_flags, (const int *)h->centre);
  hipLaunchKernelGGL(acq_finalize_kernel, dim3((C + 1023) / 1024), dim3(1024), 0, s, fp, h->st, (const int *)h->trk_cp_a, (const float *)h->trk_eps,
                     (const int *)h->trk_flags, kIters - 1, h->meta, h->trk_flags + kIters, (const float *)h->l_trk, (const int *)h->centre);
  hipLaunchKernelGGL(acq_track_light_kernel, dim3(1), dim3(64), 0, s, fp, h->st, (const float2 *)h->g_trk, (const float *)h->l_trk, h->meta,
                     (const int *)(h->trk_flags + kIters), h->trk_flags + kIters + 1, (const int *)h->centre, iq);
  hipLaunchKernelGGL(acq_track_kernel, dim3(1), dim3(64), 0, s, fp, h->st, (const float2 *)h->g_trk, (const float *)h->l_trk, h->meta,
                     (const int *)(h->trk_flags + kIters + 1), (AcqState *)nullptr, (const int *)h->centre, iq);
  }
  if (o.acq_only) {
    HIPCHK(hipMemcpyAsync(h->st_host, h->st, sizeof(RxState), hipMemcpyDeviceToHost, s));
    HIPCHK(hipGetLastError());
    return DVBT_OK;
  }
  }
  if (tm) HIPCHK(hipEventRecord(h->ev[ST_FFT], s));
  const bool drift_off = o.skip_acq && h->st_host->drift_known_off;
  if (!drift_off) {
    const DriftBufs &D = h->drift;
    hipLaunchKernelGGL(drift_prep_kernel, dim3((C + 255) / 256), dim3(256), 0, s, fp, (const RxState *)h->st, (const SymMeta *)h->meta, D);
    hipLaunchKernelGGL(drift_exact_kernel, dim3(1), dim3(1024), 0, s, fp, (const RxState *)h->st, (const SymMeta *)h->meta, D);
    const dim3 rg((C + 255) / 256);
    hipLaunchKernelGGL(drift_round_kernel<0>, rg, dim3(256), 0, s, fp, (const RxState *)h->st, (const SymMeta *)h->meta, D, (const double *)nullptr, D.d);
    hipLaunchKernelGGL(drift_round_kernel<1>, rg, dim3(256), 0, s, fp, (const RxState *)h->st, (const SymMeta *)h->meta, D, (const double *)D.d, D.S);
    hipLaunchKernelGGL(drift_round_kernel<1>, rg, dim3(256), 0, s, fp, (const RxState *)h->st, (const SymMeta *)h->meta, D, (const double *)D.S, D.d);
    hipLaunchKernelGGL(drift_round_kernel<2>, rg, dim3(256), 0, s, fp, (const RxState *)h->st, (const SymMeta *)h->meta, D, (const double *)D.d, D.S);
    hipLaunchKernelGGL(drift_table_kernel, dim3(C), dim3(N / 32 < 256 ? N / 32 : 256), 0, s, fp, (const RxState *)h->st, (const SymMeta *)h->meta, D);
  }
  const bool taps = h->acq_tap || h->fft_out || h->eq;
#define SYM_ARGS iq, fp, (const RxState *)h->st, (const SymMeta *)h->meta, (const float2 *)h->T.tw, h->acq_tap, h->fft_out, h->T.demod_tables(), h->eq, h->tpsval, h->info, \
                 h->T.inner_params(d.payload), (const float2 *)h->T.points, (const unsigned char *)h->T.label_tab, h->labels, h->sym_ticket, (const float *)h->drift.delta, (const int *)h->drift.flags, h->csi
  const int g8 = std::min(h->sym_grid, C), g2 = std::min(h->sym_grid, (C + S2_Q - 1) / S2_Q);
  if (N == S8_N && !taps) {
    hipLaunchKernelGGL((symbol8k_kernel<false, false>), dim3(g8), dim3(S8_T), S8_LDS_BYTES, s, SYM_ARGS);
    if (!drift_off) hipLaunchKernelGGL((symbol8k_kernel<false, true>), dim3(g8), dim3(S8_T), S8_LDS_BYTES, s, SYM_ARGS);
  } else if (N == S8_N) {
    hipLaunchKernelGGL((symbol8k_kernel<true, false>), dim3(g8), dim3(S8_T), S8_LDS_BYTES, s, SYM_ARGS);
    if (!drift_off) hipLaunchKernelGGL((symbol8k_kernel<true, true>), dim3(g8), dim3(S8_T), S8_LDS_BYTES, s, SYM_ARGS);
  } else if (N == S2_N && !taps) {
    hipLaunchKernelGGL((symbol2k_kernel<false, false>), dim3(g2), dim3(S2_T * S2_Q), S2_LDS_BYTES, s, SYM_ARGS);
    if (!drift_off) hipLaunchKernelGGL((symbol2k_kernel<false, true>), dim3(g2), dim3(S2_T * S2_Q), S2_LDS_BYTES, s, SYM_ARGS);
  } else if (N == S2_N) {
    hipLaunchKernelGGL((symbol2k_kernel<true, false>), dim3(g2), dim3(S2_T * S2_Q), S2_LDS_BYTES, s, SYM_ARGS);
    if (!drift_off) hipLaunchKernelGGL((symbol2k_kernel<true, true>), dim3(g2), dim3(S2_T * S2_Q), S2_LDS_BYTES, s, SYM_ARGS);
  }
#undef SYM_ARGS
  if (tm) HIPCHK(hipEventRecord(h->ev[ST_DEMOD], s));
  if (!o.continuation) {
    hipLaunchKernelGGL(tps_vote_kernel, dim3((C + 63) / 64), dim3(256), 0, s, (const float2 *)h->tpsval, d.n_tps, (const RxState *)h->st, 0,
                       (const float2 *)nullptr, h->maj, fp.keep_last);
    hipLaunchKernelGGL(tps_fsm_par_kernel, dim3((C + TPS_THREADS * TPS_SEG - 1) / (TPS_THREADS * TPS_SEG)), dim3(TPS_THREADS), 0, s, fp, (const RxState *)h->st, (const SymInfo *)h->info,
                       (const int *)h->maj, h->sym_index, h->tps_edges, h->trk_flags + 8, &h->st->tps_bits, (const unsigned short *)h->T.tps_bch,
                       o.tps_init ? (const TpsState *)h->tps_state : (const TpsState *)nullptr);
    hipLaunchKernelGGL(tps_tail_kernel, dim3(1), dim3(256), 0, s, fp, h->st, (const SymInfo *)h->info, (const int *)h->maj, h->tps_state, h->sym_index,
                       (const TpsEdge *)h->tps_edges, (const int *)(h->trk_flags + 8), h->trk_flags + 9, 0, h->vp, cut_sym_off);
  } else {
    hipLaunchKernelGGL(tps_vote_kernel, dim3((C + 63) / 64), dim3(256), 0, s, (const float2 *)h->tpsval, d.n_tps, (const RxState *)h->st, 0,
                       (const float2 *)h->tps_prev, h->maj, fp.keep_last);
    hipLaunchKernelGGL(tps_tail_kernel, dim3(1), dim3(256), 0, s, fp, h->st, (const SymInfo *)h->info, (const int *)h->maj, h->tps_state, h->sym_index,
                       (const TpsEdge *)nullptr, (const int *)nullptr, (int *)nullptr, 1, h->vp, cut_sym_off);
  }
  if (tm) HIPCHK(hipEventRecord(h->ev[ST_INNER], s));
  InnerParams ip = h->T.inner_params(d.payload);
  long long max_vit = (long long)C * d.payload * d.m * d.k / (8 * d.n) + 1;
  if (o.vit_off + (size_t)max_vit > h->vit_cap) return fail(DVBT_ERR_CAPACITY, "Viterbi stream buffer too small for the segment's lock periods");
  if (h->prm.soft_decision) {
    const float step = 2.0f * d.norm;
    hipLaunchKernelGGL(soft_demap_kernel, dim3(C), dim3(256), (size_t)d.payload * d.m, s, (const float2 *)h->eq, (const float *)h->csi, (const RxState *)h->st, ip, (const float2 *)h->T.points,
                       1.0f / (step * step), (const int *)h->sym_index, (const uint16_t *)h->soft_tab, h->soft_a);
    { int r = join_front(); if (r) return r; }
    if (tmv) HIPCHK(hipEventRecord(h->ev[ST_VIT], s));
    const S4Plan sp = s4_plan(max_vit, d.ntb);
    const unsigned grid = std::min(s4_grid(max_vit, d.ntb), h->soft_grid);
    hipLaunchKernelGGL(viterbi_soft4_kernel, dim3(grid), dim3(64 * S4_WAVES), 0, s, (const int8_t *)h->soft_a, h->vit + o.vit_off, (const RxState *)h->st, h->vp,
                       h->soft_scratch, sp.B, sp.nsteps);
  } else {
  hipLaunchKernelGGL(inner_kernel<6>, dim3(C), dim3(INNER_THREADS), inner_lds_bytes((size_t)d.payload), s, (const float2 *)nullptr, (const uint8_t *)h->labels, ip,
                     (const RxState *)h->st, 0, (const int *)h->sym_index, (const float2 *)nullptr, (const unsigned char *)nullptr,
                     (const uint16_t *)h->T.H, (const uint16_t *)h->T.Hinv, (uint8_t *)nullptr, h->symdeint_tap, h->bitdeint, h->bitdeint_lp);
  { int r = join_front(); if (r) return r; }
  if (tmv) HIPCHK(hipEventRecord(h->ev[ST_VIT], s));
  VitParams vp = h->vp;
  vp.chunk_bytes = vit_chunk_bytes(h, max_vit);
  const bool proof = h->vproof.snap && h->prm.viterbi_verify != VIT_PLAIN;
  V3Aux ax = h->vproof.aux();
  if (proof) {
    if (max_vit / vp.chunk_bytes + 2 > h->vproof.cap) return fail(DVBT_ERR_CAPACITY, "Viterbi proof: state buffer too small for this segment's chunks");
    h->vit_checked = true;
  }
  launch_viterbi(s, (const uint8_t *)((h->prm.hier_stream && h->bitdeint_lp) ? h->bitdeint_lp : h->bitdeint), h->vit + o.vit_off, (const RxState *)h->st, 0ll, vp, 0ll, 0ll, max_vit,
                 proof ? &ax : nullptr, h->prm.viterbi_verify);
  }
  if (tmv) HIPCHK(hipEventRecord(h->ev[ST_RS], s));
  if (o.tail) { int r = enqueue_tail(h, s, max_vit / 204 + 1, -1); if (r) return r; }
  if (tm) HIPCHK(hipEventRecord(h->ev[ST_END], s));
  if (tmv) h->ev_recorded = true;
  HIPCHK(hipMemcpyAsync(h->st_host, h->st, sizeof(RxState), hipMemcpyDeviceToHost, s));
  HIPCHK(hipGetLastError());
  h->pending = true;
  return DVBT_OK;
}

extern "C" int dvbt_rx_segment_enqueue_device(dvbt_rx *h, const void *iq_device, size_t nsamples, void *stream)
{
  if (!h || !iq_device) return fail(DVBT_ERR_INVALID, "null argument");
  HIPCHK(hipSetDevice(h->prm.device));
  hipStream_t s = stream ? (hipStream_t)stream : h->own_stream;
  const float2 *chain; size_t chain_n;
  int r = prepare_chain(h, (const float2 *)iq_device, nsamples, s, &chain, &chain_n); if (r) return r;
  h->n_periods = 1; h->seg_offset = 0;
  if (h->prm.launch_graph && !h->timing && !h->rsd.ri && !(h->acq_tap || h->fft_out || h->symdeint_tap || h->deint_tap)) {
    for (auto &ge : h->graphs)
      if (ge.iq == chain && ge.n == chain_n && ge.s == s && ge.sym_off == h->cut.stream_symbol_offset && ge.delay == h->cut.start_delay_symbols && ge.phase == h->cut.descr_call_phase) {
        HIPCHK(hipGraphLaunch(ge.exec, s));
        h->cur_stream = s; h->pending = true;
        return DVBT_OK;
      }
    if (h->graphs.size() < 16) {
      hipGraph_t gr = nullptr; hipGraphExec_t ex = nullptr;
      HIPCHK(hipStreamBeginCapture(s, hipStreamCaptureModeThreadLocal));
      const int r = enqueue(h, chain, chain_n, s);
      const hipError_t e = hipStreamEndCapture(s, &gr);
      if (r) { if (gr) (void)hipGraphDestroy(gr); return r; }
      if (e != hipSuccess || !gr) return fail(DVBT_ERR_HIP, std::string("hipStreamEndCapture: ") + hipGetErrorString(e));
      const hipError_t e2 = hipGraphInstantiate(&ex, gr, nullptr, nullptr, 0);
      (void)hipGraphDestroy(gr);
      if (e2 != hipSuccess) return fail(DVBT_ERR_HIP, std::string("hipGraphInstantiate: ") + hipGetErrorString(e2));
      h->graphs.push_back(dvbt_rx::GraphEntry{chain, chain_n, s, (long long)h->cut.stream_symbol_offset, h->cut.start_delay_symbols, h->cut.descr_call_phase, ex});
      HIPCHK(hipGraphLaunch(ex, s));
      h->cur_stream = s; h->pending = true;
      return DVBT_OK;
    }
  }
  return enqueue(h, chain, chain_n, s);
}

static void fill_report(dvbt_rx *h, const RxState &s, dvbt_rx_report &r)
{
  memset(&r, 0, sizeof r);
  r.status = s.status; r.n_symbols = s.n_symbols; r.first_out_symbol = s.first_out; r.n_out_symbols = s.n_out_symbols;
  r.cp_start0 = s.cp_start0; r.first_call = s.call0;
  r.resume_sample = ((s.status & 2) && !(s.status & 1)) ? (int64_t)(s.call0 + s.n_symbols) * (h->d.N + h->d.cp) + (h->d.N + h->d.cp) / 2 : 0;
  r.n_viterbi_bytes = s.n_vit_bytes; r.n_rs_items = s.n_rs_items; r.n_rs_bytes = s.n_rs_words * 188;
  r.n_ts_bytes = s.n_ts_bytes; r.rs_fail_words = s.rs_fail; r.rs_corrected_symbols = s.rs_corr;
  r.stream_symbol_offset = s.sym_off; r.ts_first_packet = s.ts_first_packet; r.stream_rs_items = s.stream_rs_items;
  r.tps_valid = (int32_t)(s.tps_bits >> 63); r.tps_bits = s.tps_bits & ~(1ull << 63);
  if (r.tps_valid) {
    auto fld = [&](int first, int last) { int v = 0; for (int i = first; i <= last; i++) v = (v << 1) | (int)((s.tps_bits >> i) & 1ull); return v; };
    r.tps_length_indicator = fld(17, 22); r.tps_constellation = fld(25, 26); r.tps_hierarchy = fld(27, 29);
    r.tps_code_rate_hp = fld(30, 32); r.tps_code_rate_lp = fld(33, 35); r.tps_guard_interval = fld(36, 37);
    r.tps_transmission_mode = fld(38, 39); r.tps_cell_id = fld(40, 47);
    const dvbt_rx_params &q = h->prm;
    r.tps_mismatch = (r.tps_constellation != q.constellation ? 1 : 0) | (r.tps_hierarchy != q.hierarchy ? 2 : 0) | (r.tps_code_rate_hp != q.code_rate ? 4 : 0) |
                     (r.tps_guard_interval != q.guard_interval ? 8 : 0) | (r.tps_transmission_mode != q.transmission_mode ? 16 : 0);
    if (r.tps_mismatch) r.status |= 16;
  }
}

extern "C" int dvbt_rx_segment_finish(dvbt_rx *h, dvbt_rx_report *rep)
{
  if (!h) return fail(DVBT_ERR_INVALID, "null handle");
  if (!h->pending) return fail(DVBT_ERR_STATE, "no segment enqueued");
  HIPCHK(hipStreamSynchronize(h->cur_stream));
  h->pending = false;
  if (h->timing && h->ev_recorded) {
    for (int i = h->timing == 2 ? ST_VIT : 0; i < (h->timing == 2 ? ST_RS : ST_END); i++) { float ms = 0; if (hipEventElapsedTime(&ms, h->ev[i], h->ev[i + 1]) == hipSuccess) h->acc_ms[i] += ms; }
    float ms = 0; if (h->timing == 1 && hipEventElapsedTime(&ms, h->ev[0], h->ev[ST_END]) == hipSuccess) h->acc_ms[ST_END] += ms;
    h->n_timed++; h->ev_recorded = false;
  }
  dvbt_rx_report r;
  fill_report(h, *h->st_host, r);
  r.n_lock_periods = r.first_out_symbol >= 0 ? 1 : 0;
  h->last = r; h->have_last = true;
  if (rep) *rep = r;
  return DVBT_OK;
}

struct LockPeriod { size_t off; int n_symbols; float avg_in; bool carry; int call0, cp_start0; bool lost; };
static void set_ctx(dvbt_rx *h, int k)
{
  if (k != h->ctx && !h->graphs.empty()) drop_graphs(h);
  h->ctx = k; h->st = h->st_ctx[k]; h->meta = h->meta_ctx[k]; h->trk_flags = h->trk_flags_ctx[k]; h->sym_ticket = h->sym_ticket_ctx[k]; h->drift.flags = h->drift_flags_ctx[k];
  h->st_host = h->st_host_ctx[k];
}

static int segment_periods(dvbt_rx *h, const float2 *chain, size_t chain_n, hipStream_t s, dvbt_rx_report *rep)
{
  const Dims &d = h->d;
  const size_t L = (size_t)(d.N + d.cp), win = (size_t)(2 * d.N + d.cp + 16);
  std::vector<LockPeriod> per;
  h->plog.clear(); h->plog_bytes = 0;
  bool capped = false;
  h->periods.clear();
  struct Book {
    size_t acc = 0; int delivering = 0, processed = 0; bool any = false; dvbt_rx_report first_rep; RxState last_st; int total_symbols = 0; size_t last_off = 0;
  } bk, snap[2];
  memset(&bk.first_rep, 0, sizeof bk.first_rep); bk.first_rep.first_out_symbol = -1;
  memset(&bk.last_st, 0, sizeof bk.last_st); bk.last_st.first_out = -1; bk.last_st.status = 1;
  bool snap_assumed[2] = {false, false};
  bool need_full = false;
  int ctx_last = -1;
  auto acq_ctx = [&]() -> int {
    const int k = ctx_last < 0 ? h->ctx : (ctx_last == 0 ? 1 : 0);
    if (k != h->ctx) set_ctx(h, k);
    return DVBT_OK;
  };
  hipStream_t s2 = h->aux_stream;
  HIPCHK(hipEventRecord(h->aux_ev, s)); HIPCHK(hipStreamWaitEvent(s2, h->aux_ev, 0));
  struct Pend { bool on = false; size_t p = 0, vit_off = 0; int ctx = 0; hipStream_t st = nullptr; } pend;
  unsigned long long tps_keep = 0;
  int snap_period[2] = {-1, -1}, sn = 0;
  auto decode_finish = [&]() -> int {
    if (!pend.on) return DVBT_OK;
    HIPCHK(hipStreamSynchronize(pend.st));
    pend.on = false; h->pending = false;
    const size_t p = pend.p;
    const RxState &st = *h->st_host_ctx[pend.ctx];
    if (st.tps_bits) tps_keep = st.tps_bits;
    bk.processed++; bk.any = true; bk.last_st = st; bk.last_off = per[p].off;
    h->periods[p].first_out_symbol = 0;
    if (h->bd_log) {
      size_t base = 0; for (size_t q = 0; q < p; q++) base += (size_t)std::max(per[q].n_symbols, 0);
      if (h->plog.size() <= p) h->plog.resize(p + 1, dvbt_period_tap{0, 0, 0, 0});
      dvbt_period_tap e = {(int64_t)(base * d.payload), 0, (int64_t)pend.vit_off, 0};
      if (st.first_out >= 0 && st.n_out_symbols > 0) {
        e.bitdeint_bytes = (int64_t)st.n_out_symbols * d.payload; e.viterbi_bytes = st.n_vit_bytes;
        HIPCHK(hipMemcpy(h->bd_log + e.bitdeint_offset, (h->prm.hier_stream && h->bitdeint_lp) ? h->bitdeint_lp : h->bitdeint, (size_t)e.bitdeint_bytes, hipMemcpyDeviceToDevice));
        h->plog_bytes = std::max(h->plog_bytes, (size_t)(e.bitdeint_offset + e.bitdeint_bytes));
      }
      h->plog[p] = e;
    }
    if (st.first_out >= 0) {
      h->periods[p].first_out_symbol = st.first_out + 1;
      if (bk.delivering == 0) { fill_report(h, st, bk.first_rep); bk.first_rep.segment_offset = (int64_t)per[p].off; }
      bk.acc = pend.vit_off + (size_t)st.n_vit_bytes; bk.delivering++;
    }
    return DVBT_OK;
  };
  auto decode_launch = [&](size_t p, bool later, bool reuse, hipStream_t ds) -> int {
    const int usable = per[p].n_symbols - (later ? 0 : 1);
    bk.total_symbols += per[p].n_symbols;
    if (usable < 1) return DVBT_OK;
    if (!reuse) { int r = acq_ctx(); if (r) return r; }
    EnqOpt o; o.use_carry = per[p].carry; o.carry_avg = per[p].avg_in; o.hist = (long long)per[p].off; o.avail = (long long)(chain_n - per[p].off); o.continuation = bk.processed > 0; o.keep_last = later; o.tail = false; o.skip_acq = reuse;
// ... 554 lines not shown
```

gr_dvbt_amd/csrc/k_backend.hpp:

```cpp
#pragma once
#include <hip/hip_runtime.h>
#include <stdint.h>
#include "k_frontend.hpp"

namespace dvbt {

struct InnerParams { int payload, m, csize; int nlev; float inv_step, guard; float hshift; int hier; };
__device__ __forceinline__ float hier_unshift(float x, float hshift) { return copysignf(fmaxf(fabsf(x) - hshift, 0.f), x); }

__device__ __forceinline__ int demap_all(float2 v, const float2 *pts, int csize)
{
  float dr = v.x - pts[0].x, di = v.y - pts[0].y;
  float best = dr * dr + di * di; int idx = 0;
  for (int j = 1; j < csize; j++) {
    dr = v.x - pts[j].x; di = v.y - pts[j].y;
    float d = dr * dr + di * di;
    if (d < best) { best = d; idx = j; }
  }
  return idx;
}

__device__ __forceinline__ int demap_fast(float2 v, const float2 *pts, const unsigned char *label_of, const InnerParams &p)
{
  const bool in_range = p.nlev != 0 && fabsf(v.x) < p.guard && fabsf(v.y) < p.guard;
  const int n = p.nlev;
  const float gx = p.hshift != 0.f ? hier_unshift(v.x, p.hshift) : v.x, gy = p.hshift != 0.f ? hier_unshift(v.y, p.hshift) : v.y;
  int ji = (int)floorf(gx * p.inv_step + 0.5f * (float)n), jq = (int)floorf(gy * p.inv_step + 0.5f * (float)n);
  ji = ji < 0 ? 0 : ji > n - 1 ? n - 1 : ji; jq = jq < 0 ? 0 : jq > n - 1 ? n - 1 : jq;
  const int L00 = label_of[ji * 8 + jq];
  const float px0 = pts[L00].x, py0 = pts[L00].y;
  int ji2 = ji + (v.x > px0 ? 1 : -1), jq2 = jq + (v.y > py0 ? 1 : -1);
  ji2 = (ji2 < 0 || ji2 > n - 1) ? ji : ji2; jq2 = (jq2 < 0 || jq2 > n - 1) ? jq : jq2;
  const int L10 = label_of[ji2 * 8 + jq], L01 = label_of[ji * 8 + jq2], L11 = label_of[ji2 * 8 + jq2];
  const float px1 = pts[L10].x, py1 = pts[L01].y;
  const float dx0 = v.x - px0, dx1 = v.x - px1, dy0 = v.y - py0, dy1 = v.y - py1;
  const float ax0 = dx0 * dx0, ax1 = dx1 * dx1, ay0 = dy0 * dy0, ay1 = dy1 * dy1;
  const float d00 = ax0 + ay0, d01 = ax0 + ay1, d10 = ax1 + ay0, d11 = ax1 + ay1;
  const float best = fminf(fminf(d00, d01), fminf(d10, d11));
  int idx = 255;
  idx = d00 == best ? min(idx, L00) : idx; idx = d01 == best ? min(idx, L01) : idx;
  idx = d10 == best ? min(idx, L10) : idx; idx = d11 == best ? min(idx, L11) : idx;
  return in_range ? idx : -1;
}
__device__ __forceinline__ int demap_one(float2 v, const float2 *pts, const unsigned char *label_of, const InnerParams &p)
{
  const int f = demap_fast(v, pts, label_of, p);
  return f >= 0 ? f : demap_all(v, pts, p.csize);
}

constexpr int IB = 126, IBS = 132;
__host__ __device__ inline size_t inner_lds_bytes(size_t payload) { return ((((payload + IB - 1) / IB) * IBS + 15) & ~(size_t)15) + 64 * 8 + 64; }
__device__ __forceinline__ int ipos(int d) { const int b = d / IB; return d + b * (IBS - IB); }

#ifndef DVBT_INNER_THREADS
#define DVBT_INNER_THREADS 256
#endif
template <int VB> __device__ __forceinline__ void bit_deint_words(const uint8_t *v, uint8_t *o, int payload, int tid)
{
  constexpr int hv = VB / 2;
  const int nitems = (payload / 126) * 32;
  for (int it = tid; it < nitems; it += DVBT_INNER_THREADS) {
    const int blk = it >> 5, j = it & 31;
    const unsigned *bw = reinterpret_cast<const unsigned *>(v + blk * 132);
    unsigned val = 0;
#pragma unroll
    for (int k = 0; k < VB; k++) {
      constexpr int offs[6] = {0, 63, 105, 42, 21, 84};
      const int eidx = k / hv + 2 * (k % hv);
      int w = 4 * j - offs[eidx]; if (w < 0) w += 126;
      const unsigned lo = bw[w >> 2], hi = bw[(w >> 2) + 1];
      const unsigned word = __builtin_amdgcn_alignbyte(hi, lo, (unsigned)(w & 3));
      val |= ((word >> (VB - 1 - eidx)) & 0x01010101u) << (VB - 1 - k);
    }
    uint8_t *dst = o + blk * 126 + 4 * j;
    *reinterpret_cast<uint16_t *>(dst) = (uint16_t)val;
    if (j < 31) *reinterpret_cast<uint16_t *>(dst + 2) = (uint16_t)(val >> 16);
  }
}

__device__ __forceinline__ void bit_deint_hier(const uint8_t *v, uint8_t *o_hp, uint8_t *o_lp, int payload, int m, int tid)
{
  constexpr int offs[6] = {0, 63, 105, 42, 21, 84};
  for (int idx = tid; idx < payload; idx += DVBT_INNER_THREADS) {
    const int blk = idx / 126, i = idx - blk * 126;
    const uint8_t *bb = v + blk * 132;
    auto bit = [&](int f) -> int { const int e = f / 126, j = f - e * 126; int w = j - offs[e]; if (w < 0) w += 126; return (bb[w] >> (m - 1 - e)) & 1; };
    const int t0 = m * i;
    const int hp = (bit((t0 & 1) * 126 + t0 / 2) << 1) | bit(((t0 + 1) & 1) * 126 + (t0 + 1) / 2);
    int lp = 0;
    for (int k = 2; k < m - 2; k++) {
      const int t = t0 + k, e = (t % (m - 2)) / ((m - 2) / 2) + 2 * (t % ((m - 2) / 2)) + 2, f = e * 126 + t / (m - 2);
      lp = (lp << 1) | (f < m * 126 ? bit(f) : 0);
    }
    o_hp[idx] = (uint8_t)hp;
    if (o_lp) o_lp[idx] = (uint8_t)lp;
  }
}

constexpr int INNER_NB = 12;
constexpr int INNER_THREADS = DVBT_INNER_THREADS;
template <int MODE> __global__ __launch_bounds__(INNER_THREADS) void inner_kernel(const float2 *__restrict__ eq, const uint8_t *__restrict__ in_bytes, InnerParams p,
                                                   const RxState *st, int nitems_fixed, const int *__restrict__ sym_index,
                                                   const float2 *__restrict__ points, const unsigned char *__restrict__ label_tab,
                                                   const uint16_t *__restrict__ H, const uint16_t *__restrict__ Hinv,
                                                   uint8_t *__restrict__ tap_demap, uint8_t *__restrict__ tap_symdeint,
                                                   uint8_t *__restrict__ out, uint8_t *__restrict__ out_lp = nullptr)
{
  extern __shared__ __attribute__((aligned(16))) unsigned char smem_raw[];
  uint8_t *v = smem_raw;
  float2 *pts = reinterpret_cast<float2 *>(smem_raw + ((((p.payload + IB - 1) / IB) * IBS + 15) & ~15));
  unsigned char *label_of = reinterpret_cast<unsigned char *>(pts + 64);
  const int u = blockIdx.x, tid = threadIdx.x;
  constexpr int mode = MODE;
  int first = 0, nout = nitems_fixed;
  if (st) { first = st->first_out; nout = st->n_out_symbols; if (first < 0) return; }
  if (u >= nout) return;
  const int s = first + u;
  if (mode & 1) {
    for (int j = tid; j < p.csize; j += INNER_THREADS) pts[j] = points[j];
    if (tid < 64) label_of[tid] = label_tab[tid];
  }
  __syncthreads();
  const bool odd = (mode & 2) ? (sym_index[s] & 1) : false;
  const float2 *e = eq ? eq + (size_t)s * p.payload : nullptr;
  const uint8_t *ib = in_bytes ? in_bytes + (size_t)s * p.payload : nullptr;
  const uint16_t *ptab = odd ? H : Hinv;
  for (int q0 = tid; q0 < p.payload; q0 += INNER_NB * INNER_THREADS) {
    unsigned pk[INNER_NB];
#pragma unroll
    for (int k = 0; k < INNER_NB; k++) {
      const int q = q0 + k * INNER_THREADS, qc = q < p.payload ? q : p.payload - 1;
      pk[k] = (mode & 2) ? (unsigned)ptab[qc] : (unsigned)qc;
      if (!(mode & 1)) pk[k] |= (unsigned)ib[qc] << 16;
    }
#pragma unroll
    for (int k = 0; k < INNER_NB; k++) {
      const int q = q0 + k * INNER_THREADS;
      if (q < p.payload) {
        const int lab = (mode & 1) ? demap_one(e[q], pts, label_of, p) : (int)(pk[k] >> 16);
        const int dst = (int)(pk[k] & 0xffffu);
        const int blk = dst / IB, r = dst - blk * IB, at = blk * IBS + r;
        v[at] = (uint8_t)lab;
        if (r < IBS - IB) v[at + IB] = (uint8_t)lab;
        if (tap_demap && (mode & 1)) tap_demap[(size_t)u * p.payload + q] = (uint8_t)lab;
      }
    }
  }
  __syncthreads();
  uint8_t *o = out + (size_t)u * p.payload;
  if (tap_symdeint) for (int q = tid; q < p.payload; q += INNER_THREADS) tap_symdeint[(size_t)u * p.payload + q] = v[ipos(q)];
  if (!(mode & 4)) { for (int q = tid; q < p.payload; q += INNER_THREADS) o[q] = v[ipos(q)]; return; }
  if (p.hier) bit_deint_hier(v, o, out_lp ? out_lp + (size_t)u * p.payload : nullptr, p.payload, p.m, tid);
  else if (p.m == 2) bit_deint_words<2>(v, o, p.payload, tid);
  else if (p.m == 4) bit_deint_words<4>(v, o, p.payload, tid);
  else bit_deint_words<6>(v, o, p.payload, tid);
}

struct VitParams {
  int m, k, n, plen, ntb, bsize;
  int d_nsymbols;
  int d_nbits;
  int chunk_bytes;
  int payload;
  unsigned punct_mask;
  int warm;
  unsigned long long prefix_nib;
  unsigned long long magic_plen, magic_m;
  unsigned long long punct_rep;
  unsigned magic16_plen;
  uint8_t punct[16], prefix[16];
};

__device__ __forceinline__ void plan_body(RxState *st, const VitParams &vp, long long sym_off)
{
  const long long ibits = (long long)vp.payload * vp.m * vp.k / vp.n;
  const long long nin_g = (sym_off + (long long)st->n_out_symbols) * vp.payload;
  const long long nblocks_g = nin_g / vp.d_nsymbols;
  long long nin = nblocks_g * vp.d_nsymbols - sym_off * vp.payload;
  long long steps = nblocks_g * (vp.d_nbits / 2) - sym_off * ibits;
  if (nin < 0 || steps < 0) { nin = 0; steps = 0; }
  st->n_vit_in = nin;
  st->n_vit_steps = steps;
  long long nb_g = nblocks_g * (vp.d_nbits / 2) / 8 - vp.ntb;
  if (nb_g < 0) nb_g = 0;
  long long nb = steps / 8 - vp.ntb;
  if (nb < 0) nb = 0;
  st->n_vit_bytes = nb;
  const long long items_g = (nb_g / 1632) & ~1ll;
  long long words = items_g * 8 - sym_off * ibits / (8 * 204);
  if (words < 0) words = 0;
  st->stream_rs_items = items_g;
  st->n_rs_words = words;
  st->n_rs_items = words / 8;
  st->sym_off = sym_off;
  st->n_ts_bytes = 0; st->rs_fail = 0; st->rs_corr = 0; st->ts_first_packet = 0; st->rs_list_n = 0;
}
__global__ __launch_bounds__(256) void tps_tail_kernel(FrontParams p, RxState *st, const SymInfo *info, const int *maj, TpsState *ts, int *sym_index,
                                                      const TpsEdge *edges, const int *first_cand, int *need_seq, int clear_d_init, VitParams vp, long long sym_off)
{
  int seq = 1;
  if (edges) seq = tps_finalize_body(st, edges, first_cand, need_seq, p.keep_last, ts);
  if (seq) tps_fsm_body(p, st, 0, info, maj, ts, sym_index, (int *)nullptr, (const unsigned char *)nullptr, clear_d_init);
  if (threadIdx.x == 0) plan_body(st, vp, sym_off);
}

struct RsTables { const uint8_t *div_tab;  const uint8_t *gexp;  const uint8_t *glog;  };

constexpr int RS_SYN_STRIDE = 65;
__device__ inline int rs_decode_word_wave(uint8_t *cw, const uint8_t *syn, const uint8_t *gexp, const uint8_t *glog,
                                          int compat, uint8_t *scr, int lane)
{
  auto gmul = [&](int a, int b) -> int { return (a == 0 || b == 0) ? 0 : gexp[glog[a] + glog[b]]; };
  auto gdiv = [&](int a, int b) -> int { return (a == 0 || b == 0) ? 0 : gexp[255 + glog[a] - glog[b]]; };
  auto wxor = [&](int v) -> int { for (int o = 16; o > 0; o >>= 1) v ^= __shfl_xor(v, o); return v; };
  int sig = lane == 0 ? 1 : 0, bb = sig, el = 0;
  for (int r = 1; r <= 16; r++) {
    int term = (lane < r && lane <= 16) ? gmul(sig, syn[(r - 1 - lane) * RS_SYN_STRIDE]) : 0;
    const int discr = __shfl(wxor(term), 0);
    int bup = __shfl_up(bb, 1); if (lane == 0) bup = 0;
    if (discr == 0) bb = bup;
    else {
      const int T = sig ^ gmul(discr, bup);
      if (2 * el <= r - 1) { el = r - el; bb = gdiv(sig, discr); } else bb = bup;
      sig = lane <= 16 ? T : 0;
    }
  }
  const unsigned long long nz = __ballot(sig != 0 && lane <= 16);
  const int deg_sigma = nz ? 63 - __clzll(nz) : 0;
  uint8_t *s_sig = scr, *s_root = scr + 17, *s_om = scr + 34;
  if (lane <= 16) s_sig[lane] = (uint8_t)sig;
  __builtin_amdgcn_fence(__ATOMIC_SEQ_CST, "wavefront");
  int found[4]; int nroots = 0;
  unsigned long long bal[4];
  for (int k = 0; k < 4; k++) {
    const int i = lane + 1 + 64 * k;
    int q = 1;
    if (i <= 255) {
      for (int j = 1; j <= deg_sigma; j++) { int sg = s_sig[j]; if (sg) q ^= gexp[(glog[sg] + (j * i) % 255) % 255]; }
    }
    found[k] = (i <= 255) && (q == 0);
    bal[k] = __ballot(found[k]);
  }
  {
    int before = 0;
    for (int k = 0; k < 4; k++) {
      if (found[k]) { int rank = before + __popcll(bal[k] & ((1ull << lane) - 1)); if (rank < 17 && rank < deg_sigma) s_root[rank] = (uint8_t)(lane + 1 + 64 * k); }
      before += __popcll(bal[k]);
    }
    nroots = before < deg_sigma ? before : deg_sigma;
  }
  if (nroots != deg_sigma) return -1;
  {
    int tmp = 0;
    if (lane < 16) { int jm = deg_sigma < lane ? deg_sigma : lane; for (int j = jm; j >= 0; j--) tmp ^= gmul(syn[(lane - j) * RS_SYN_STRIDE], s_sig[j]); s_om[lane] = (uint8_t)tmp; }
    const unsigned long long oz = __ballot(lane < 16 && tmp != 0);
    __builtin_amdgcn_fence(__ATOMIC_SEQ_CST, "wavefront");
    const int deg_omega = oz ? 63 - __clzll(oz) : 0;
    int err = 0, den = 1, loc = 0;
    if (lane < nroots) {
      const int root = s_root[lane];
      int num1 = 0;
      for (int i = deg_omega; i >= 0; i--) { int om = s_om[i]; if (om) num1 ^= gexp[(glog[om] + (i * root) % 255) % 255]; }
      const int num2 = gexp[(255 - root) % 255];
      den = 0;
      const int deg_max = deg_sigma < 15 ? deg_sigma : 15;
      for (int i = 1; i <= deg_max; i += 2) { int sg = s_sig[i]; if (sg) den ^= gexp[(glog[sg] + ((i - 1) * root) % 255) % 255]; }
      err = gdiv(gmul(num1, num2), den);
      loc = (compat && lane == 0) ? 0 : root - 1;
    }
    const unsigned long long dz = __ballot(lane < nroots && den == 0);
    const int kz = dz ? 63 - __clzll(dz) : -1;
    if (lane < nroots && lane > kz && loc >= 51) cw[loc - 51] ^= (uint8_t)err;
    __builtin_amdgcn_fence(__ATOMIC_SEQ_CST, "wavefront");
    return kz >= 0 ? -1 : nroots;
  }
}


__device__ inline int rs_decode_word_lane(uint8_t *cw, const uint8_t *syn_col , const uint8_t *gexp, const uint8_t *glog, int compat,
                                          uint8_t *root_col , bool active)
{
  auto gmul = [&](int a, int b) -> int { return (a == 0 || b == 0) ? 0 : gexp[glog[a] + glog[b]]; };
  int syn[16];
#pragma unroll
  for (int i = 0; i < 16; i++) syn[i] = active ? syn_col[i * RS_SYN_STRIDE] : 0;
  int sg[17], bb[17];
#pragma unroll
  for (int i = 0; i < 17; i++) { sg[i] = i == 0 ? 1 : 0; bb[i] = sg[i]; }
  int el = 0;
#pragma unroll
  for (int r = 1; r <= 16; r++) {
    int discr = 0;
#pragma unroll
    for (int i = 0; i < r; i++) discr ^= gmul(sg[i], syn[r - i - 1]);
    if (__any(discr != 0)) {
      const int dl = glog[discr];
      const bool grow = discr != 0 && 2 * el <= r - 1;
      int T[17];
      T[0] = sg[0];
#pragma unroll
      for (int i = 0; i < 16; i++) T[i + 1] = sg[i + 1] ^ ((discr == 0 || bb[i] == 0) ? 0 : gexp[dl + glog[bb[i]]]);
#pragma unroll
      for (int i = 16; i >= 0; i--) {
        const int shifted = i == 0 ? 0 : bb[i - 1];
        const int divd = (sg[i] == 0 || discr == 0) ? 0 : gexp[255 + glog[sg[i]] - dl];
        bb[i] = grow ? divd : shifted;
      }
      if (grow) el = r - el;
// ... 351 lines not shown
```

gr_dvbt_amd/csrc/k_viterbi3.hpp:

```cpp
#pragma once
#include <hip/hip_runtime.h>
#include <stdint.h>
#include <limits.h>
#include <string.h>
#include "dvbt_tables.hpp"
#include "k_backend.hpp"

namespace dvbt {

inline VitParams make_vit_params(const Dims &d, int bsize, int chunk_bytes)
{
  VitParams v; memset(&v, 0, sizeof v);
  v.m = d.m; v.k = d.k; v.n = d.n; v.plen = d.plen; v.ntb = d.ntb; v.bsize = bsize;
  v.d_nsymbols = bsize * d.n / d.m; v.d_nbits = 2 * d.k * bsize;
  v.chunk_bytes = chunk_bytes > 0 ? chunk_bytes : 768; v.payload = d.payload; v.warm = 72;
  memcpy(v.punct, d.punct, 16); memcpy(v.prefix, d.prefix, 16);
  v.punct_mask = 0; v.prefix_nib = 0;
  for (int i = 0; i < d.plen; i++) { v.punct_mask |= (unsigned)d.punct[i] << i; v.prefix_nib |= (unsigned long long)d.prefix[i] << (4 * i); }
  v.magic_plen = ~0ull / (unsigned)d.plen + 1; v.magic_m = ~0ull / (unsigned)d.m + 1;
  for (int i = 0; i < 64; i++) v.punct_rep |= (unsigned long long)d.punct[i % d.plen] << i;
  v.magic16_plen = (65536u + (unsigned)d.plen - 1) / (unsigned)d.plen;
  return v;
}

// ... 113 lines not shown
#else
#define V3_YIELD()
#endif

__device__ __forceinline__ int lo16(int x) { return (x << 16) >> 16; }
__device__ __forceinline__ int hi16(int x) { return x >> 16; }
template <int CTRL> __device__ __forceinline__ int max_dpp(int v) { return max(v, dppb<CTRL>(v)); }
template <int CTRL> __device__ __forceinline__ int min_dpp(int v) { return min(v, dppb<CTRL>(v)); }

template <int PE, bool RENORM> __device__ __forceinline__ int v3_window_end(int (&v)[2], const V3Lane &L)
{
  const int kp = pk_max((v[0] & (int)0xfe00fe00) | L.kc[PE / 2][0], (v[1] & (int)0xfe00fe00) | L.kc[PE / 2][1]);
  int k = max(lo16(kp), hi16(kp));
  k = max_dpp<DPP_XOR1>(k); k = max_dpp<DPP_XOR2>(k); k = max_dpp<DPP_HALF_MIRROR>(k); k = max_dpp<DPP_MIRROR>(k);
  if (RENORM) {
    const unsigned sub = (unsigned)((k & ~0x1ff) - (48 << 8));
    const int mn = (int)__builtin_amdgcn_perm(sub, sub, 0x01000100u);
    v[0] = pk_sub(v[0], mn); v[1] = pk_sub(v[1], mn);
  }
  return k;
}

template <int NW> constexpr int V3_ROW = NW * 4 * 64;
template <int NW> constexpr int V3_RMASK = (V3_RINGW * V3_ROW<NW> - 1) & ~63;
struct V3Trace {
  int z[2];
  int wsh[2];
  int osh[2];
  unsigned long long ok[2];
  int oend[2];
  int ob[2];
};
__device__ __forceinline__ void v3_hop_read(const V3Trace &T, const unsigned char *tab, unsigned (&t)[2])
{
#pragma unroll
  for (int q = 0; q < 2; q++) t[q] = tab[T.z[q]];
}
template <int NW> __device__ __forceinline__ void v3_hop_merge(V3Trace &T, const unsigned (&t)[2])
{
#pragma unroll
  for (int q = 0; q < 2; q++) {
    T.wsh[q] -= V3_ROW<NW>;
    asm("v_bfi_b32 %0, %1, %2, %3" : "=v"(T.z[q]) : "s"(V3_RMASK<NW>), "v"(T.wsh[q]), "v"(t[q]));
  }
}
template <int NW> __device__ __forceinline__ void v3_hop(V3Trace &T, const unsigned char *tab) { unsigned t[2]; v3_hop_read(T, tab, t); v3_hop_merge<NW>(T, t); }
__device__ __forceinline__ void v3_trace_read(const V3Trace &T, const unsigned char *tab, unsigned (&t)[2])
{
#pragma unroll
  for (int q = 0; q < 2; q++) t[q] = tab[T.z[q]];
}
template <bool MASKED> __device__ __forceinline__ void v3_trace_store(const V3Trace &T, const unsigned (&t)[2], uint8_t *outb)
{
#pragma unroll
  for (int q = 0; q < 2; q++) {
    const unsigned zz = (t[q] ^ (((t[q] >> 4) & 1u) * 12u)) & 63u;
    unsigned by = (((zz | (zz << 6)) >> T.osh[q]) & 0xfcu) | (t[q] >> 6);
    if (MASKED) {
      unsigned long long sv;
      asm volatile("s_and_saveexec_b64 %0, %1\n\tglobal_store_byte %2, %3, off\n\ts_mov_b64 exec, %0" : "=&s"(sv) : "s"(T.ok[q]), "v"(outb + T.ob[q]), "v"(by) : "memory", "scc");
    } else if ((T.ok[q] >> (threadIdx.x & 63)) & 1) outb[T.ob[q]] = (unsigned char)by;
  }
}
__device__ __forceinline__ void v3_trace_out(const V3Trace &T, const unsigned char *tab, uint8_t *outb) { unsigned t[2]; v3_trace_read(T, tab, t); v3_trace_store<false>(T, t, outb); }

__device__ __forceinline__ void v3_load_words(const unsigned *wp_, unsigned (&W)[8])
{
  const uint4 *wp = reinterpret_cast<const uint4 *>(wp_);
  const uint4 t0 = wp[0], t1 = wp[1];
  W[0] = t0.x; W[1] = t0.y; W[2] = t0.z; W[3] = t0.w; W[4] = t1.x; W[5] = t1.y; W[6] = t1.z; W[7] = t1.w;
}
template <int V6, bool HOPS, int HOP0, int NTB, int NW, bool PREF> __device__ __forceinline__ void v3_fwd_window(int (&v)[2], const V3Lane &L, const unsigned *wrow, unsigned char *tab, unsigned char *tabw,
                                                                                           unsigned char *bests, int j0, int dd, int pl, V3Trace &T, unsigned (&W)[8], unsigned (&Wn)[8], uint8_t *outb)
{
  constexpr bool HOPA = HOPS && HOP0 + 2 * V6 < NTB - 1, HOPB = HOPS && HOP0 + 2 * V6 + 1 < NTB - 1;
  constexpr bool FINA = HOPS && HOP0 + 2 * V6 == NTB - 1, FINB = HOPS && HOP0 + 2 * V6 + 1 == NTB - 1;
  unsigned th[2], tout[2];
  if (HOPA) v3_hop_read(T, tab, th);
  if (FINA) v3_trace_read(T, tab, tout);
  const int jr = (j0 + V6) & (V3_RINGW - 1);
#if V3_EXP & 256
  for (int i = 0; i < 8; i++) { W[i] = (unsigned)(j0 * 0x01010101 + i * 0x00020406 + pl); asm volatile("" : "+v"(W[i])); }
#else
  if (PREF) v3_load_words(wrow + (V6 + 1) * 8, Wn);
#endif
  constexpr int P0 = (8 * V6) % 6;
  int raw[2];
#if V3_EXP & 32
  if (V6 & 1) __builtin_amdgcn_s_setprio(1); else __builtin_amdgcn_s_setprio(0);
#endif
#if V3_EXP & 128
  __builtin_amdgcn_s_sleep(1);
#endif
  v3_step<(P0 + 0) % 6, 0>(v, W[0], L, raw); V3_YIELD(); v3_step<(P0 + 1) % 6, 0>(v, W[1], L, raw); V3_YIELD(); v3_step<(P0 + 2) % 6, 3>(v, W[2], L, raw); V3_YIELD();
  if (HOPA) { v3_hop_merge<NW>(T, th); if (HOPB) v3_hop_read(T, tab, th); }
  if (FINB) v3_trace_read(T, tab, tout);
  if (FINA) v3_trace_store<true>(T, tout, outb);
  v3_step<(P0 + 3) % 6, 0>(v, W[3], L, raw); V3_YIELD(); v3_step<(P0 + 4) % 6, 0>(v, W[4], L, raw); V3_YIELD(); v3_step<(P0 + 5) % 6, 1>(v, W[5], L, raw); V3_YIELD();
  v3_step<(P0 + 6) % 6, 4>(v, W[6], L, raw); V3_YIELD(); v3_step<(P0 + 7) % 6, 2>(v, W[7], L, raw);
  if (HOPB) v3_hop_merge<NW>(T, th);
  if (FINB) v3_trace_store<true>(T, tout, outb);
  if (!(V3_EXP & 4)) *reinterpret_cast<unsigned *>(tabw + jr * V3_ROW<NW>) = __builtin_amdgcn_perm((unsigned)raw[1], (unsigned)raw[0], 0x06040200u);
  if (V3_EXP & 2) { if (raw[0] == 0x12345) bests[jr] = 1; return; }
  const int s = v3_window_end<(P0 + 2) % 6, (V6 & 1) == 1>(v, L);
  bests[dd * V3_RINGW + jr] = (unsigned char)s;
}
template <bool HOPS, int HOP0, int NTB, int NW, bool MORE> __device__ __forceinline__ void v3_fwd_six(int (&v)[2], const V3Lane &L, const unsigned *wrow, unsigned char *tab, unsigned char *tabw,
                                                                                  unsigned char *bests, int j0, int dd, int pl, V3Trace &T, unsigned (&Wa)[8], unsigned (&Wb)[8], uint8_t *outb)
{
  v3_fwd_window<0, HOPS, HOP0, NTB, NW, true>(v, L, wrow, tab, tabw, bests, j0, dd, pl, T, Wa, Wb, outb); v3_fwd_window<1, HOPS, HOP0, NTB, NW, true>(v, L, wrow, tab, tabw, bests, j0, dd, pl, T, Wb, Wa, outb);
  v3_fwd_window<2, HOPS, HOP0, NTB, NW, true>(v, L, wrow, tab, tabw, bests, j0, dd, pl, T, Wa, Wb, outb); v3_fwd_window<3, HOPS, HOP0, NTB, NW, true>(v, L, wrow, tab, tabw, bests, j0, dd, pl, T, Wb, Wa, outb);
  v3_fwd_window<4, HOPS, HOP0, NTB, NW, true>(v, L, wrow, tab, tabw, bests, j0, dd, pl, T, Wa, Wb, outb); v3_fwd_window<5, HOPS, HOP0, NTB, NW, MORE>(v, L, wrow, tab, tabw, bests, j0, dd, pl, T, Wb, Wa, outb);
}

#if V3_EXP & 16
__device__ unsigned long long *v3_dbg;
#endif

constexpr int V3_SLOT = 32;
constexpr int V3_CTL_CHUNKS = 0;
constexpr int V3_CTL_MISMATCH = 1;
constexpr int V3_CTL_CONFLICT = 2;
constexpr int V3_CTL_UNPROVEN = 3;
constexpr int V3_CTL_SEQ = 4;
constexpr int V3_CTL_ACC = 8;
constexpr int V3_CTL_HDR = 16;
struct V3Aux {
  int *snap;
  int *ctl;
  long long cap;
  long long grid0;
  const int *carry_in;
  int *carry_out; int carry_rel;
  int debug;
};
__device__ __forceinline__ int *v3_own(const V3Aux &ax, long long c) { return ax.snap + (3 * c) * V3_SLOT; }
__device__ __forceinline__ int *v3_pred(const V3Aux &ax, long long c) { return ax.snap + (3 * c + 1) * V3_SLOT; }
__device__ __forceinline__ int *v3_fix(const V3Aux &ax, long long c) { return ax.snap + (3 * c + 2) * V3_SLOT; }
inline size_t v3_snap_words(long long cap) { return (size_t)(cap + 2) * 3 * V3_SLOT; }
inline size_t v3_ctl_words(long long cap) { return (size_t)V3_CTL_HDR + 2 * (size_t)(cap + 2); }

struct V3Lds { unsigned char *tab; unsigned *wbuf; unsigned char *bests; const unsigned *lut; int wv; };
__device__ __forceinline__ void v3_init_lut(unsigned *lut, int lane)
{
  if (lane < 16) {
    const int k0 = (lane >> 2) & 1, k1 = (lane >> 3) & 1, t1 = (lane >> 1) & 1, t0 = lane & 1;
    const int u0 = k0 ? 1 - 2 * t1 : 0, u1 = k1 ? 1 - 2 * (k0 ? t0 : t1) : 0;
    const unsigned d0 = (unsigned)(2 * (u0 + u1)) & 0xff, d1 = (unsigned)(2 * (-u0 + u1)) & 0xff;
    const unsigned d2 = (unsigned)(2 * (u0 - u1)) & 0xff, d3 = (unsigned)(2 * (-u0 - u1)) & 0xff;
    lut[lane] = d0 | (d1 << 8) | (d2 << 16) | (d3 << 24);
  }
}

template <int NTB, int WARM, int MODE, int NW>
__device__ __forceinline__ void v3_decode(const uint8_t *__restrict__ in, uint8_t *__restrict__ out, long long total_steps, long long total_out, const VitParams &vp,
                                          long long in_base, long long out_lo, long long b0, bool dec_active, const V3Lds &S, const V3Lane &L, int (&v)[2], int (&endv)[2],
                                          int *own, int *predn, const int *inject, int *carry, int carry_rel)
{
  unsigned char *const tab = S.tab; unsigned *const wbuf = S.wbuf; unsigned char *const bests = S.bests; const unsigned *const lut = S.lut;
  unsigned *const cbits = wbuf;
  constexpr int V3_CBS = V3_BLK * 8;
  static_assert(V3_CBW <= V3_CBS, "bit stream does not fit the step-word row");
  const int lane = threadIdx.x & 63, dd = lane >> 4, pl = lane & 15;
  const int rowl = S.wv * 256 + dd * 64;
  unsigned char *const tabw = tab + rowl + pl * 4;
  const int B = vp.chunk_bytes, m = vp.m;
  constexpr int ntb = NTB;
  const long long b1 = (b0 + B < total_out) ? b0 + B : total_out;
  const int warm = MODE == 2 ? 0 : WARM > 0 ? WARM : vp.warm;
  const long long w0 = b0 + 2 - warm;
  const int J = ((warm + B + ntb - 1 + V3_BLK - 1) / V3_BLK) * V3_BLK;
  const long long n_in_bytes = (total_steps * 2 / vp.plen * vp.n + vp.m - 1) / vp.m;
  const int nload = ((384 + 2 * m - 2) / m + 3 + 15) / 16;

  uint8_t *const outb = out + (b0 - out_lo);
  const int ob_end = !dec_active ? INT_MIN : (int)(b1 - b0 > INT_MIN / 2 ? b1 - b0 : INT_MIN / 2);
  const int ob_lo = MODE != 1 || out_lo <= b0 ? 0 : (int)(out_lo - b0 < INT_MAX / 2 ? out_lo - b0 : INT_MAX / 2);
  const long long tb0 = 8 * (w0 - 1) - 2;
  constexpr int BLKBITS = 2 * 8 * V3_BLK;
  const int inc_q = BLKBITS / vp.plen, inc_ph = BLKBITS - inc_q * vp.plen;
  const unsigned magic16_m = (65536u + (unsigned)m - 1) / (unsigned)m;

  int u_first, u_last;
  {
    const long long r = total_steps - 8 * V3_BLK - tb0;
    int first = tb0 >= 0 ? 0 : (int)((-tb0 + 7) >> 3 < J ? (-tb0 + 7) >> 3 : J), last = !dec_active || r < 0 ? -1 : (int)(r >> 3 < J ? r >> 3 : J);
    u_first = max(max(__builtin_amdgcn_readlane(first, 0), __builtin_amdgcn_readlane(first, 16)), max(__builtin_amdgcn_readlane(first, 32), __builtin_amdgcn_readlane(first, 48)));
    u_last = min(min(__builtin_amdgcn_readlane(last, 0), __builtin_amdgcn_readlane(last, 16)), min(__builtin_amdgcn_readlane(last, 32), __builtin_amdgcn_readlane(last, 48)));
  }
  auto pfx = [&](int ph) { return (int)__popc(vp.punct_mask & ((1u << ph) - 1u)); };
  int ph0 = 0, pf0 = 0, bo0 = 0, off = 0; long long byte0 = 0; uint4 q = make_uint4(0, 0, 0, 0);
  auto stage_load = [&](int jb) {
    const long long tb = tb0 + (long long)jb * 8;
    if (jb > 0 && jb - V3_BLK >= u_first) {
      const int pf_old = pf0;
      ph0 += inc_ph;
      const int wrap = ph0 >= vp.plen ? 1 : 0;
      ph0 -= wrap ? vp.plen : 0;
      pf0 = pfx(ph0);
      const int r = bo0 + (inc_q + wrap) * vp.n + pf0 - pf_old;
      const int dby = (int)(((unsigned)r * magic16_m) >> 16);
      bo0 = r - dby * m; byte0 += dby;
    } else {
      const unsigned long long pbit = 2ull * (unsigned long long)(tb > 0 ? tb : 0);
      const unsigned long long pq = __umul64hi(pbit, vp.magic_plen);
      ph0 = (int)(pbit - pq * (unsigned)vp.plen); pf0 = pfx(ph0);
      const unsigned long long rb = pq * (unsigned)vp.n + (unsigned)pf0;
      const unsigned long long by = __umul64hi(rb, vp.magic_m);
      byte0 = (long long)by; bo0 = (int)(rb - by * (unsigned)m);
    }
    off = (int)(((unsigned long long)(uintptr_t)in + (unsigned long long)(byte0 - in_base)) & 3ull);
    const long long src = byte0 - off + pl * 16;
    q = make_uint4(0, 0, 0, 0);
    if (dec_active && pl < nload) {
      if (src >= in_base && src + 16 <= n_in_bytes) q = *reinterpret_cast<const uint4 *>(in + (src - in_base));
      else {
        unsigned w[4] = {0, 0, 0, 0};
        for (int i = 0; i < 16; i++) {
          const long long bb = src + i;
          const unsigned bv = (bb >= in_base && bb < n_in_bytes) ? in[bb - in_base] : 0;
          w[i >> 2] |= bv << (8 * (i & 3));
        }
        q = make_uint4(w[0], w[1], w[2], w[3]);
      }
    }
  };
  auto stage_words = [&](int jb) {
    {
      const unsigned mk = (1u << m) - 1;
      auto grp = [&](unsigned d) { return ((d & mk) << (3 * m)) | (((d >> 8) & mk) << (2 * m)) | (((d >> 16) & mk) << m) | ((d >> 24) & mk); };
      const unsigned g0 = grp(q.x), g1 = grp(q.y), g2 = grp(q.z), g3 = grp(q.w);
      unsigned *cb = cbits + dd * V3_CBS;
      if (pl < nload) {
        if (m == 2) cb[pl] = (g0 << 24) | (g1 << 16) | (g2 << 8) | g3;
        else if (m == 4) { cb[2 * pl] = (g0 << 16) | g1; cb[2 * pl + 1] = (g2 << 16) | g3; }
        else { cb[3 * pl] = (g0 << 8) | (g1 >> 16); cb[3 * pl + 1] = (g1 << 16) | (g2 >> 8); cb[3 * pl + 2] = (g2 << 24) | g3; }
      }
    }
    __builtin_amdgcn_fence(__ATOMIC_SEQ_CST, "wavefront");
    constexpr int SPL = V3_BLK * 8 / 16;
    const long long tb = tb0 + (long long)jb * 8;
    const int ub0 = pl * SPL;
    int lo = 0, hi = SPL;
    int x = ph0 + 2 * ub0;
    if (jb < u_first || jb > u_last) {
      const long long tbr = tb > 0 ? tb : 0;
      const long long t = tb + ub0;
      if (t < 0) lo = (-t < SPL) ? (int)(-t) : SPL;
      const long long rem = total_steps - t;
      hi = !dec_active ? 0 : rem <= 0 ? 0 : rem < SPL ? (int)rem : SPL;
      if (hi < lo) hi = lo;
      x = ph0 + 2 * (int)((t + lo) - tbr);
      if (x < 0) x = 0;
    }
    const int dq = (int)(((unsigned)x * vp.magic16_plen) >> 16);
    const int ph = x - dq * vp.plen;
    const int pos = off * m + bo0 + dq * vp.n + pfx(ph) - pf0;
    const unsigned kmask = ((unsigned)(vp.punct_rep >> ph) << (2 * lo)) & (((1u << (2 * hi)) - 1u) & ~((1u << (2 * lo)) - 1u));
    const unsigned *cb = cbits + dd * V3_CBS;
    const unsigned cw0 = cb[pos >> 5], cw1 = cb[(pos >> 5) + 1];
    unsigned win = (unsigned)(((((unsigned long long)cw0) << 32) | cw1) >> (32 - (pos & 31)));
    unsigned idx[SPL], sw[SPL];
#pragma unroll
    for (int i = 0; i < SPL; i++) {
      const unsigned k2 = (kmask >> (2 * i)) & 3u;
      idx[i] = (k2 << 2) | (win >> 30);
      win <<= __popc(k2);
    }
#pragma unroll
    for (int i = 0; i < SPL; i++) sw[i] = lut[idx[i]];
    static_assert(SPL % 4 == 0, "a lane's step words are whole 16-byte groups (its offset dd * 768 + pl * 48 bytes is 16-byte aligned)");
    uint4 *const wdst = reinterpret_cast<uint4 *>(wbuf + dd * (V3_BLK * 8) + ub0);
#pragma unroll
    for (int i = 0; i < SPL / 4; i++) wdst[i] = make_uint4(sw[4 * i], sw[4 * i + 1], sw[4 * i + 2], sw[4 * i + 3]);
    __builtin_amdgcn_fence(__ATOMIC_SEQ_CST, "wavefront");
  };
  V3Trace T;
  int tsh[2];
#pragma unroll
  for (int c = 0; c < 2; c++) {
    T.oend[c] = c * 16 + pl < V3_BLK ? ob_end : INT_MIN; tsh[c] = (2 * ((c * 16 + pl + 1) % 3) + 4) % 6; T.osh[c] = (6 - 2 * ((c * 16 + pl + 3 * ntb - (ntb - 1)) % 3)) % 6;
  }
  static_assert(V3_BLK % 3 == 0, "phases per lane");
  auto bests_read = [&](int jp, unsigned (&bb)[2]) {
#pragma unroll
    for (int c = 0; c < 2; c++) bb[c] = bests[dd * V3_RINGW + ((jp + c * 16 + pl) & (V3_RINGW - 1))];
  };
  auto trace_init = [&](int jp, const unsigned (&bb)[2]) {
#pragma unroll
    for (int c = 0; c < 2; c++) {
      const int jj = jp + c * 16 + pl;
      T.ob[c] = jj - (warm + ntb - 1);
      T.ok[c] = __builtin_amdgcn_ballot_w64(T.ob[c] >= ob_lo && T.ob[c] < T.oend[c]);
      T.wsh[c] = jj * V3_ROW<NW> + rowl;
      const unsigned R = (bb[c] | (bb[c] << 6)) >> tsh[c];
      T.z[c] = (int)((R ^ 51u ^ (((R >> 4) & 1u) * 12u)) & 63u) | (T.wsh[c] & V3_RMASK<NW>);
    }
  };
  unsigned bb[2];

  stage_load(0);
  for (int jb = 0; jb < J; jb += V3_BLK) {
    if (MODE == 1 && dec_active) {
      if (jb == warm) { if (inject) { v[0] = inject[0]; v[1] = inject[1]; } own[0] = v[0]; own[1] = v[1]; }
      if (jb == warm + B) { predn[0] = v[0]; predn[1] = v[1]; }
      if (carry && jb == warm + carry_rel) { carry[0] = v[0]; carry[1] = v[1]; }
    }
    if (MODE == 2) {
      if (jb == 0 && dec_active) { own[0] = v[0]; own[1] = v[1]; }
      if (jb == B) { endv[0] = v[0]; endv[1] = v[1]; }
      if (carry && dec_active && jb == carry_rel) { carry[0] = v[0]; carry[1] = v[1]; }
    }
    bests_read(jb - V3_BLK, bb);
    if (!(V3_EXP & 8) || jb == 0) stage_words(jb);
    if (jb + V3_BLK < J && !(V3_EXP & 8)) stage_load(jb + V3_BLK);
    const bool tr = jb > 0 && !(V3_EXP & 1);
    if (tr) trace_init(jb - V3_BLK, bb);
    const unsigned *wrow = wbuf + dd * (V3_BLK * 8);
    unsigned Wa[8], Wb[8];
    v3_load_words(wrow, Wa);
    if (tr) {
      v3_fwd_six<true, 0, NTB, NW, true>(v, L, wrow, tab, tabw, bests, jb, dd, pl, T, Wa, Wb, outb);
      v3_fwd_six<true, 12, NTB, NW, true>(v, L, wrow + 48, tab, tabw, bests, jb + 6, dd, pl, T, Wa, Wb, outb);
    } else {
      v3_fwd_six<false, 0, NTB, NW, true>(v, L, wrow, tab, tabw, bests, jb, dd, pl, T, Wa, Wb, outb);
      v3_fwd_six<false, 0, NTB, NW, true>(v, L, wrow + 48, tab, tabw, bests, jb + 6, dd, pl, T, Wa, Wb, outb);
    }
    static_assert(V3_BLK == 24, "the second half of the block is written out: two groups of six windows, straight-line like the first half");
    static_assert(NTB - 1 < 24, "the chains' last read takes a hop slot of the first twelve windows");
    v3_fwd_six<false, 0, NTB, NW, true>(v, L, wrow + 96, tab, tabw, bests, jb + 12, dd, pl, T, Wa, Wb, outb);
    v3_fwd_six<false, 0, NTB, NW, false>(v, L, wrow + 144, tab, tabw, bests, jb + 18, dd, pl, T, Wa, Wb, outb);
  }
  __builtin_amdgcn_fence(__ATOMIC_SEQ_CST, "wavefront");
  bests_read(J - V3_BLK, bb);
  trace_init(J - V3_BLK, bb);
  for (int h = 0; h < ntb - 1; h++) v3_hop<NW>(T, tab);
  v3_trace_out(T, tab, outb);
}

template <int NW> struct V3Shared {
  alignas(16) unsigned char tab[V3_RINGW * V3_ROW<NW>];
  alignas(16) unsigned wbuf[NW][4 * V3_BLK * 8];
  unsigned char bests[NW][4 * V3_RINGW];
  unsigned lut[16];
};
static_assert(sizeof(V3Shared<4>) <= 81920 && V3_RMASK<4> == 0xffc0 && V3_RMASK<1> == 0x3fc0, "two four-wave workgroups per CU beside the symbol kernel's 76 KB");
#define V3_LDS_DECL(NW) __shared__ V3Shared<NW> sh_;
#define V3_LDS(NW, wv) V3Lds{sh_.tab, sh_.wbuf[wv], sh_.bests[wv], sh_.lut, wv}

template <int NTB, int WARM = V3_WARM, int MODE = 0> __global__ __launch_bounds__(64 * V3_WGW) void viterbi3_kernel(const uint8_t *__restrict__ in, uint8_t *__restrict__ out, const RxState *st,
                                                      long long steps_fixed, VitParams vp, V3Aux ax, long long in_base, long long out_lo)
{
  V3_LDS_DECL(V3_WGW)
  const int wv = V3_WGW > 1 ? (int)(threadIdx.x >> 6) : 0;
  const V3Lds S = V3_LDS(V3_WGW, wv);
  const int lane = threadIdx.x & 63, dd = lane >> 4, pl = lane & 15;
  const long long total_steps = st ? st->n_vit_steps : steps_fixed;
  const long long total_out = total_steps / 8 - vp.ntb;
  const int B = vp.chunk_bytes;
  if (MODE == 1 && blockIdx.x == 0 && threadIdx.x == 0) {
    ax.ctl[V3_CTL_MISMATCH] = 0; ax.ctl[V3_CTL_CONFLICT] = 0; ax.ctl[V3_CTL_UNPROVEN] = -1; ax.ctl[V3_CTL_SEQ] = 0;
  }
  const long long grid0 = MODE == 1 ? ax.grid0 : out_lo;
  const long long chunk0 = ((long long)blockIdx.x * V3_WGW + wv) * 4;
  if (grid0 + chunk0 * B >= total_out) return;
  const long long c = chunk0 + dd, b0 = grid0 + c * B;
  const bool dec_active = b0 < total_out;
  v3_init_lut(sh_.lut, lane);
#if V3_EXP & 16
  const unsigned long long dbg_t0 = wall_clock64();
#endif
  V3Lane L; v3_init_lane(pl, L);
  int v[2] = {L.arm_org[0][0], L.arm_org[0][1]}, endv[2];
  int *own = nullptr, *predn = nullptr, *carry = nullptr; const int *inject = nullptr;
  if (MODE == 1) {
    own = v3_own(ax, c) + 2 * pl; predn = v3_pred(ax, c + 1) + 2 * pl;
    if (c == 0 && ax.carry_in) inject = ax.carry_in + 2 * pl;
    if (ax.carry_out && b0 + B >= total_out) carry = ax.carry_out + 2 * pl;
  }
  v3_decode<NTB, WARM, MODE, V3_WGW>(in, out, total_steps, total_out, vp, in_base, out_lo, b0, dec_active, S, L, v, endv, own, predn, inject, carry, ax.carry_rel);
#if V3_EXP & 16
  if (lane == 0) {
    unsigned id, xcc;
    asm volatile("s_getreg_b32 %0, hwreg(HW_REG_HW_ID)" : "=s"(id));
    asm volatile("s_getreg_b32 %0, hwreg(HW_REG_XCC_ID)" : "=s"(xcc));
    unsigned long long *d = v3_dbg + 3 * ((long long)blockIdx.x * V3_WGW + wv);
    d[0] = (id & 0xffffu) | ((xcc & 0xfu) << 16); d[1] = dbg_t0; d[2] = wall_clock64();
  }
#endif
}

__device__ __forceinline__ long long v3_nchunks(long long total_out, long long grid0, int B) { return total_out > grid0 ? (total_out - grid0 + B - 1) / B : 0; }
__device__ __forceinline__ bool v3_slots_equal(const int *a_, const int *b_)
{
  const int4 *a = reinterpret_cast<const int4 *>(a_), *b = reinterpret_cast<const int4 *>(b_);
  bool same = true;
#pragma unroll
  for (int i = 0; i < 8; i++) { const int4 x = a[i], y = b[i]; same = same && x.x == y.x && x.y == y.y && x.z == y.z && x.w == y.w; }
  return same;
}

__global__ __launch_bounds__(256) void viterbi_check_kernel(V3Aux ax, const RxState *st, long long steps_fixed, VitParams vp, int pass)
{
  const long long total_steps = st ? st->n_vit_steps : steps_fixed;
  const long long nch = v3_nchunks(total_steps / 8 - vp.ntb, ax.grid0, vp.chunk_bytes);
  if (blockIdx.x == 0 && threadIdx.x == 0) { ax.ctl[V3_CTL_CHUNKS] = (int)(nch < INT_MAX ? nch : INT_MAX); if (pass == 1) ax.ctl[V3_CTL_UNPROVEN] = 0; }
  const long long c = (long long)blockIdx.x * 256 + threadIdx.x + 1;
  if (c >= nch || c > ax.cap) return;
  const bool same = v3_slots_equal(v3_own(ax, c), v3_pred(ax, c));
  if (pass == 0) {
    ax.ctl[V3_CTL_HDR + (ax.cap + 2) + c] = 0;
    if (!same) ax.ctl[V3_CTL_HDR + atomicAdd(ax.ctl + V3_CTL_MISMATCH, 1)] = (int)c;
  }
}
__global__ __launch_bounds__(256) void viterbi_count_kernel(V3Aux ax, const RxState *st, long long steps_fixed, VitParams vp)
{
  const long long total_steps = st ? st->n_vit_steps : steps_fixed;
  const long long nch = v3_nchunks(total_steps / 8 - vp.ntb, ax.grid0, vp.chunk_bytes);
  const long long c = (long long)blockIdx.x * 256 + threadIdx.x + 1;
  if (c >= nch || c > ax.cap) return;
  if (!v3_slots_equal(v3_own(ax, c), v3_pred(ax, c))) atomicAdd(ax.ctl + V3_CTL_UNPROVEN, 1);
}

__device__ __forceinline__ bool v3_row_equal(const int (&a)[2], const int (&b)[2], int dd)
{
  const unsigned long long ne = __ballot(a[0] != b[0] || a[1] != b[1]);
  return ((ne >> (16 * dd)) & 0xffffull) == 0;
}

template <int NTB, int NW> __device__ __forceinline__ void v3_repair_rows(const uint8_t *__restrict__ in, uint8_t *__restrict__ out, long long total_steps, const VitParams &vp, const V3Aux &ax,
                                                                  long long in_base, long long out_lo, const V3Lds &S, const V3Lane &L, long long rows, long long row0, int n)
{
  const int lane = threadIdx.x & 63, dd = lane >> 4, pl = lane & 15;
  const long long total_out = total_steps / 8 - vp.ntb;
  const int B = vp.chunk_bytes;
  const long long nch = v3_nchunks(total_out, ax.grid0, B);
  for (long long i0 = row0; i0 < n; i0 += rows) {
    const bool act = i0 + dd < n;
    const long long c = act ? ax.ctl[V3_CTL_HDR + i0 + dd] : 1;
    const long long b0 = ax.grid0 + c * B;
    int v[2], endv[2] = {0, 0};
    { const int *p = v3_pred(ax, c) + 2 * pl; v[0] = p[0]; v[1] = p[1]; }
    int *carry = (act && ax.carry_out && b0 + B >= total_out) ? ax.carry_out + 2 * pl : nullptr;
    v3_decode<NTB, 0, 2, NW>(in, out, total_steps, total_out, vp, in_base, out_lo, b0, act && b0 < total_out, S, L, v, endv, v3_own(ax, c) + 2 * pl, nullptr, nullptr, carry, ax.carry_rel);
    int pn[2] = {endv[0], endv[1]};
    if (act && c + 1 < nch) { const int *p = v3_pred(ax, c + 1) + 2 * pl; pn[0] = p[0]; pn[1] = p[1]; }
    if (!v3_row_equal(endv, pn, dd) || ((ax.debug & 1) && act && c + 1 < nch)) {
      int *f = v3_fix(ax, c + 1) + 2 * pl; f[0] = endv[0]; f[1] = endv[1];
      if (pl == 0) { ax.ctl[V3_CTL_HDR + (ax.cap + 2) + c + 1] = 1; atomicAdd(ax.ctl + V3_CTL_CONFLICT, 1); }
    }
    __builtin_amdgcn_fence(__ATOMIC_SEQ_CST, "wavefront");
  }
}
template <int NTB> __global__ __launch_bounds__(64 * V3_WGW) void viterbi_repair_kernel(const uint8_t *__restrict__ in, uint8_t *__restrict__ out, const RxState *st,
                                                      long long steps_fixed, VitParams vp, V3Aux ax, long long in_base, long long out_lo)
{
  V3_LDS_DECL(V3_WGW)
  const int n = ax.ctl[V3_CTL_MISMATCH];
  const int wv = V3_WGW > 1 ? (int)(threadIdx.x >> 6) : 0;
  const long long rows = (long long)gridDim.x * V3_WGW * 4, row0 = ((long long)blockIdx.x * V3_WGW + wv) * 4;
  if (row0 >= n) return;
  const V3Lds S = V3_LDS(V3_WGW, wv);
  v3_init_lut(sh_.lut, threadIdx.x & 63);
  V3Lane L; v3_init_lane(threadIdx.x & 15, L);
  v3_repair_rows<NTB, V3_WGW>(in, out, st ? st->n_vit_steps : steps_fixed, vp, ax, in_base, out_lo, S, L, rows, row0, n);
}

template <int NTB, int NW> __device__ __forceinline__ void v3_seq_walk(const uint8_t *__restrict__ in, uint8_t *__restrict__ out, long long total_steps, const VitParams &vp, const V3Aux &ax,
                                                               long long in_base, long long out_lo, const V3Lds &S, const V3Lane &L, int force)
{
  const int lane = threadIdx.x & 63, dd = lane >> 4, pl = lane & 15;
  if (lane == 0) { ax.ctl[V3_CTL_ACC] += ax.ctl[V3_CTL_CHUNKS]; ax.ctl[V3_CTL_ACC + 1] += ax.ctl[V3_CTL_MISMATCH]; }
  if (!force && ax.ctl[V3_CTL_CONFLICT] == 0) return;
  const long long total_out = total_steps / 8 - vp.ntb;
  const int B = vp.chunk_bytes;
  long long nch = v3_nchunks(total_out, ax.grid0, B);
  if (nch > ax.cap) nch = ax.cap;
  const int *cflag = ax.ctl + V3_CTL_HDR + (ax.cap + 2);
  int done = 0;
  long long pos = 0;
  for (;;) {
    long long cn = -1;
    for (long long c0 = pos + 1; c0 < nch && cn < 0; c0 += 64) {
      const long long c = c0 + lane;
      bool hit = false;
      if (c < nch) hit = cflag[c] != 0 || (force && !v3_slots_equal(v3_own(ax, c), v3_pred(ax, c)));
      const unsigned long long b = __ballot(hit);
      if (b) cn = c0 + __builtin_ctzll(b);
    }
    if (cn < 0) break;
    long long c = cn;
    int v[2];
    { const int *p = (cflag[c] ? v3_fix(ax, c) : v3_pred(ax, c)) + 2 * pl; v[0] = p[0]; v[1] = p[1]; }
    for (;;) {
      const long long b0 = ax.grid0 + c * B;
      const bool act = dd == 0;
      int st0[2] = {v[0], v[1]}, endv[2] = {0, 0};
      if (act) { int *p = v3_pred(ax, c) + 2 * pl; p[0] = v[0]; p[1] = v[1]; }
      int *carry = (act && ax.carry_out && b0 + B >= total_out) ? ax.carry_out + 2 * pl : nullptr;
      v3_decode<NTB, 0, 2, NW>(in, out, total_steps, total_out, vp, in_base, out_lo, b0, act, S, L, st0, endv, v3_own(ax, c) + 2 * pl, nullptr, nullptr, carry, ax.carry_rel);
      __builtin_amdgcn_fence(__ATOMIC_SEQ_CST, "wavefront");
      done++;
      if (c + 1 >= nch) { pos = nch; break; }
      int on[2]; { const int *p = v3_own(ax, c + 1) + 2 * pl; on[0] = p[0]; on[1] = p[1]; }
      const bool eq = (__ballot(on[0] != endv[0] || on[1] != endv[1]) & 0xffffull) == 0;
      if (act) { int *p = v3_pred(ax, c + 1) + 2 * pl; p[0] = endv[0]; p[1] = endv[1]; }
      if (eq) { pos = c + 1; break; }
      c++; v[0] = endv[0]; v[1] = endv[1];
    }
  }
  if (lane == 0) { ax.ctl[V3_CTL_SEQ] = done; ax.ctl[V3_CTL_ACC + 2] += done; }
}
template <int NTB> __global__ __launch_bounds__(64) void viterbi_repair_seq_kernel(const uint8_t *__restrict__ in, uint8_t *__restrict__ out, const RxState *st,
                                                      long long steps_fixed, VitParams vp, V3Aux ax, long long in_base, long long out_lo, int force)
{
  V3_LDS_DECL(1)
  const V3Lds S = V3_LDS(1, 0);
  v3_init_lut(sh_.lut, threadIdx.x & 63);
  V3Lane L; v3_init_lane(threadIdx.x & 15, L);
  v3_seq_walk<NTB, 1>(in, out, st ? st->n_vit_steps : steps_fixed, vp, ax, in_base, out_lo, S, L, force);
}

constexpr long long V3_FIX_SMALL = 1024;
template <int NTB> __global__ __launch_bounds__(64 * V3_WGW) void viterbi_fix_kernel(const uint8_t *__restrict__ in, uint8_t *__restrict__ out, const RxState *st,
                                                      long long steps_fixed, VitParams vp, V3Aux ax, long long in_base, long long out_lo, int force)
{
  V3_LDS_DECL(V3_WGW)
  const int wv = V3_WGW > 1 ? (int)(threadIdx.x >> 6) : 0;
  const long long total_steps = st ? st->n_vit_steps : steps_fixed;
  const long long nch = v3_nchunks(total_steps / 8 - vp.ntb, ax.grid0, vp.chunk_bytes);
  if (threadIdx.x == 0) ax.ctl[V3_CTL_CHUNKS] = (int)(nch < INT_MAX ? nch : INT_MAX);
  for (long long c = 1 + threadIdx.x; c < nch && c <= ax.cap; c += 64 * V3_WGW) {
    ax.ctl[V3_CTL_HDR + (ax.cap + 2) + c] = 0;
    if (!v3_slots_equal(v3_own(ax, c), v3_pred(ax, c))) ax.ctl[V3_CTL_HDR + atomicAdd(ax.ctl + V3_CTL_MISMATCH, 1)] = (int)c;
  }
  __threadfence(); __syncthreads();
  const int n = *(volatile int *)(ax.ctl + V3_CTL_MISMATCH);
  const V3Lds S = V3_LDS(V3_WGW, wv);
  v3_init_lut(sh_.lut, threadIdx.x & 63);
  V3Lane L; v3_init_lane(threadIdx.x & 15, L);
  if (!force && n > 0) v3_repair_rows<NTB, V3_WGW>(in, out, total_steps, vp, ax, in_base, out_lo, S, L, 4 * V3_WGW, 4 * wv, n);
  __threadfence(); __syncthreads();
  if (wv == 0) v3_seq_walk<NTB, V3_WGW>(in, out, total_steps, vp, ax, in_base, out_lo, S, L, force);
}

}
```

Before: 37600.

## Emit packed Viterbi branch codes from inner kernel and decode from codes

The inner deinterleave kernel now also compacts the bit-deinterleaved symbols into precomputed per-step packed code words (uint32), written to a new device buffer. The hard-decision Viterbi kernels (decode, fix, repair, seq) are templated on input kind, so the RX path reads these codes instead of re-gathering and depuncturing bytes. The standalone decoder block keeps the byte path. This moves depuncture and branch-input preparation into the producer kernel and shrinks Viterbi input traffic, at the cost of more LDS and work in the inner kernel and an extra buffer.

```diff
diff --git a/gr_dvbt_amd/csrc/dvbt_blocks.inc b/gr_dvbt_amd/csrc/dvbt_blocks.inc
--- a/gr_dvbt_amd/csrc/dvbt_blocks.inc
+++ b/gr_dvbt_amd/csrc/dvbt_blocks.inc
@@ -353,7 +353,7 @@
     ax.grid0 = g0; ax.carry_in = h->have_carry ? h->carry + h->cur * V3_SLOT : nullptr;
     const long long b0_last = g0 + (chunks - 1) * B;
     ax.carry_rel = (int)((out_hi - b0_last) / V3_BLK) * V3_BLK; ax.carry_out = h->carry + (h->cur ^ 1) * V3_SLOT;
-    launch_viterbi(s, (const uint8_t *)h->c.din.p, o, (const RxState *)nullptr, h->steps, h->vp, in_base, out_lo, produced, &ax, VIT_REPAIR);
+    launch_viterbi(s, (const uint8_t *)h->c.din.p, o, (const RxState *)nullptr, h->steps, h->vp, in_base, out_lo, produced, ax);
     h->cur ^= 1; h->have_carry = true; h->grid0 = b0_last + ax.carry_rel;
     if (!dev) WCHK(h->c.get(out, h->c.dout.p, (size_t)produced));
   }
diff --git a/gr_dvbt_amd/csrc/dvbt_hip.hip b/gr_dvbt_amd/csrc/dvbt_hip.hip
--- a/gr_dvbt_amd/csrc/dvbt_hip.hip
+++ b/gr_dvbt_amd/csrc/dvbt_hip.hip
@@ -207,63 +207,84 @@
 enum { VIT_PLAIN = -1, VIT_REPAIR = 0, VIT_REPAIR_COUNT = 1, VIT_PROOF_ONLY = 2, VIT_FORCE_SEQ = 3, VIT_FORCE_CONFLICT = 4 };
 constexpr unsigned V3_REPAIR_GRID = 64;
 
-static void launch_viterbi(hipStream_t s, const uint8_t *in, uint8_t *out, const RxState *st, long long steps_fixed, const VitParams &vp,
-                           long long in_base, long long out_lo, long long max_out_bytes, const V3Aux *ax = nullptr, int mode = VIT_PLAIN)
-{
-  const bool proof = ax && mode != VIT_PLAIN;
-  const long long grid0 = proof ? ax->grid0 : out_lo;
+template <bool CODES> struct V3Kern {
+  template <int N, int W, int M> static constexpr auto decode() { if constexpr (CODES) return &viterbi3_kernel<N, W, M>; else return &viterbi3_bytes_kernel<N, W, M>; }
+  template <int N> static constexpr auto fix() { if constexpr (CODES) return &viterbi_fix_kernel<N>; else return &viterbi_fix_bytes_kernel<N>; }
+  template <int N> static constexpr auto repair() { if constexpr (CODES) return &viterbi_repair_kernel<N>; else return &viterbi_repair_bytes_kernel<N>; }
+  template <int N> static constexpr auto seq() { if constexpr (CODES) return &viterbi_repair_seq_kernel<N>; else return &viterbi_repair_seq_bytes_kernel<N>; }
+};
+static dim3 v3_grid(const VitParams &vp, long long grid0, long long out_lo, long long max_out_bytes, long long *chunks_out)
+{
   long long chunks = (out_lo + max_out_bytes - grid0 + vp.chunk_bytes - 1) / vp.chunk_bytes;
   if (chunks < 1) chunks = 1;
-  const dim3 grid((unsigned)((chunks + 4 * V3_WGW - 1) / (4 * V3_WGW))), blk(64 * V3_WGW);
-  V3Aux none; memset(&none, 0, sizeof none);
-  if (proof) {
-    V3Aux a = *ax;
-    if (mode == VIT_FORCE_CONFLICT) { a.debug = 1; mode = VIT_REPAIR_COUNT; }
-    const dim3 cgrid((unsigned)((chunks + 255) / 256));
-    if (vp.warm == V3_WARM) {
-#define V3_CALL(N) hipLaunchKernelGGL((viterbi3_kernel<N, V3_WARM, 1>), grid, blk, 0, s, in, out, st, steps_fixed, vp, a, in_base, out_lo)
-      V3_NTB_SWITCH(vp.ntb, V3_CALL)
+  *chunks_out = chunks;
+  return dim3((unsigned)((chunks + 4 * V3_WGW - 1) / (4 * V3_WGW)));
+}
+template <bool CODES> static void launch_viterbi_proving(hipStream_t s, const uint8_t *in, uint8_t *out, const RxState *st, long long steps_fixed, const VitParams &vp,
+                                                         long long in_base, long long out_lo, long long max_out_bytes, const V3Aux &ax, int mode)
+{
+  using K = V3Kern<CODES>;
+  long long chunks;
+  const dim3 grid = v3_grid(vp, ax.grid0, out_lo, max_out_bytes, &chunks), blk(64 * V3_WGW);
+  V3Aux a = ax;
+  if (mode == VIT_FORCE_CONFLICT) { a.debug = 1; mode = VIT_REPAIR_COUNT; }
+  const dim3 cgrid((unsigned)((chunks + 255) / 256));
+  if (vp.warm == V3_WARM) {
+#define V3_CALL(N) hipLaunchKernelGGL((K::template decode<N, V3_WARM, 1>()), grid, blk, 0, s, in, out, st, steps_fixed, vp, a, in_base, out_lo)
+    V3_NTB_SWITCH(vp.ntb, V3_CALL)
 #undef V3_CALL
-    } else {
-#define V3_CALL(N) hipLaunchKernelGGL((viterbi3_kernel<N, 0, 1>), grid, blk, 0, s, in, out, st, steps_fixed, vp, a, in_base, out_lo)
-      V3_NTB_SWITCH(vp.ntb, V3_CALL)
+  } else {
+#define V3_CALL(N) hipLaunchKernelGGL((K::template decode<N, 0, 1>()), grid, blk, 0, s, in, out, st, steps_fixed, vp, a, in_base, out_lo)
+    V3_NTB_SWITCH(vp.ntb, V3_CALL)
 #undef V3_CALL
-    }
-    if (chunks <= V3_FIX_SMALL && mode != VIT_PROOF_ONLY) {
-#define V3_CALL(N) hipLaunchKernelGGL(viterbi_fix_kernel<N>, dim3(1), blk, 0, s, in, out, st, steps_fixed, vp, a, in_base, out_lo, mode == VIT_FORCE_SEQ ? 1 : 0)
-      V3_NTB_SWITCH(vp.ntb, V3_CALL)
+  }
+  if (chunks <= V3_FIX_SMALL && mode != VIT_PROOF_ONLY) {
+#define V3_CALL(N) hipLaunchKernelGGL((K::template fix<N>()), dim3(1), blk, 0, s, in, out, st, steps_fixed, vp, a, in_base, out_lo, mode == VIT_FORCE_SEQ ? 1 : 0)
+    V3_NTB_SWITCH(vp.ntb, V3_CALL)
 #undef V3_CALL
-      if (mode != VIT_REPAIR) {
-        hipLaunchKernelGGL(viterbi_check_kernel, dim3(1), dim3(256), 0, s, a, st, steps_fixed, vp, 1);
-        hipLaunchKernelGGL(viterbi_count_kernel, cgrid, dim3(256), 0, s, a, st, steps_fixed, vp);
-      }
-      return;
-    }
-    hipLaunchKernelGGL(viterbi_check_kernel, cgrid, dim3(256), 0, s, a, st, steps_fixed, vp, 0);
-    if (mode == VIT_REPAIR || mode == VIT_REPAIR_COUNT) {
-#define V3_CALL(N) hipLaunchKernelGGL(viterbi_repair_kernel<N>, dim3(V3_REPAIR_GRID), blk, 0, s, in, out, st, steps_fixed, vp, a, in_base, out_lo)
-      V3_NTB_SWITCH(vp.ntb, V3_CALL)
-#undef V3_CALL
-    }
-    if (mode != VIT_PROOF_ONLY) {
-      const int force = mode == VIT_FORCE_SEQ ? 1 : 0;
-#define V3_CALL(N) hipLaunchKernelGGL(viterbi_repair_seq_kernel<N>, dim3(1), dim3(64), 0, s, in, out, st, steps_fixed, vp, a, in_base, out_lo, force)
-      V3_NTB_SWITCH(vp.ntb, V3_CALL)
-#undef V3_CALL
-    }
     if (mode != VIT_REPAIR) {
       hipLaunchKernelGGL(viterbi_check_kernel, dim3(1), dim3(256), 0, s, a, st, steps_fixed, vp, 1);
       hipLaunchKernelGGL(viterbi_count_kernel, cgrid, dim3(256), 0, s, a, st, steps_fixed, vp);
     }
     return;
   }
+  hipLaunchKernelGGL(viterbi_check_kernel, cgrid, dim3(256), 0, s, a, st, steps_fixed, vp, 0);
+  if (mode == VIT_REPAIR || mode == VIT_REPAIR_COUNT) {
+#define V3_CALL(N) hipLaunchKernelGGL((K::template repair<N>()), dim3(V3_REPAIR_GRID), blk, 0, s, in, out, st, steps_fixed, vp, a, in_base, out_lo)
+    V3_NTB_SWITCH(vp.ntb, V3_CALL)
+#undef V3_CALL
+  }
+  if (mode != VIT_PROOF_ONLY) {
+    const int force = mode == VIT_FORCE_SEQ ? 1 : 0;
+#define V3_CALL(N) hipLaunchKernelGGL((K::template seq<N>()), dim3(1), dim3(64), 0, s, in, out, st, steps_fixed, vp, a, in_base, out_lo, force)
+    V3_NTB_SWITCH(vp.ntb, V3_CALL)
+#undef V3_CALL
+  }
+  if (mode != VIT_REPAIR) {
+    hipLaunchKernelGGL(viterbi_check_kernel, dim3(1), dim3(256), 0, s, a, st, steps_fixed, vp, 1);
+    hipLaunchKernelGGL(viterbi_count_kernel, cgrid, dim3(256), 0, s, a, st, steps_fixed, vp);
+  }
+}
+static void launch_viterbi(hipStream_t s, const uint8_t *in, uint8_t *out, const RxState *st, long long steps_fixed, const VitParams &vp,
+                           long long in_base, long long out_lo, long long max_out_bytes, const V3Aux &ax)
+{
+  launch_viterbi_proving<false>(s, in, out, st, steps_fixed, vp, in_base, out_lo, max_out_bytes, ax, VIT_REPAIR);
+}
+static void launch_viterbi_codes(hipStream_t s, const uint32_t *codes, uint8_t *out, const RxState *st, long long steps_fixed, const VitParams &vp,
+                                 long long out_lo, long long max_out_bytes, const V3Aux *ax = nullptr, int mode = VIT_PLAIN)
+{
+  const uint8_t *in = reinterpret_cast<const uint8_t *>(codes);
+  if (ax && mode != VIT_PLAIN) { launch_viterbi_proving<true>(s, in, out, st, steps_fixed, vp, 0ll, out_lo, max_out_bytes, *ax, mode); return; }
+  long long chunks;
+  const dim3 grid = v3_grid(vp, out_lo, out_lo, max_out_bytes, &chunks), blk(64 * V3_WGW);
+  V3Aux none; memset(&none, 0, sizeof none);
   if (vp.warm != V3_WARM) {
-#define V3_CALL(N) hipLaunchKernelGGL((viterbi3_kernel<N, 0, 0>), grid, blk, 0, s, in, out, st, steps_fixed, vp, none, in_base, out_lo)
+#define V3_CALL(N) hipLaunchKernelGGL((viterbi3_kernel<N, 0, 0>), grid, blk, 0, s, in, out, st, steps_fixed, vp, none, 0ll, out_lo)
     V3_NTB_SWITCH(vp.ntb, V3_CALL)
 #undef V3_CALL
     return;
   }
-#define V3_CALL(N) hipLaunchKernelGGL((viterbi3_kernel<N, V3_WARM, 0>), grid, blk, 0, s, in, out, st, steps_fixed, vp, none, in_base, out_lo)
+#define V3_CALL(N) hipLaunchKernelGGL((viterbi3_kernel<N, V3_WARM, 0>), grid, blk, 0, s, in, out, st, steps_fixed, vp, none, 0ll, out_lo)
   V3_NTB_SWITCH(vp.ntb, V3_CALL)
 #undef V3_CALL
 }
@@ -327,6 +348,8 @@
   float2 *acq_tap = nullptr, *fft_out = nullptr, *eq = nullptr, *tpsval = nullptr; SymInfo *info = nullptr; int *maj = nullptr, *sym_index = nullptr;
   uint8_t *labels = nullptr, *symdeint_tap = nullptr, *bitdeint = nullptr, *vit = nullptr, *deint_tap = nullptr, *rs_out = nullptr, *ts_out = nullptr;
   uint8_t *bitdeint_lp = nullptr;
+  uint32_t *vit_codes = nullptr;
+  VitCodeParams vcp;
   uint8_t *bd_log = nullptr; std::vector<dvbt_period_tap> plog; size_t plog_bytes = 0;
   VitProof vproof; bool vit_checked = false;
   size_t vit_cap = 0; RsDefer *rs_defer = nullptr; int rs_defer_cap = 0;
@@ -361,7 +384,7 @@
 
 static void rx_free(dvbt_rx *h)
 {
-  void *all[] = {h->bd_log, h->bitdeint_lp, h->st_ctx[0], h->st_ctx[1], h->st_ctx[2], h->meta_ctx[0], h->meta_ctx[1], h->meta_ctx[2], h->tps_prev_snap[0], h->tps_prev_snap[1], h->tps_snap[0], h->tps_snap[1], h->csi, h->soft_a, h->soft_tab, h->soft_scratch, h->rs_defer, h->rs_sync, h->drift_mem, h->drift.delta, h->drift_flags_ctx[0], h->drift_flags_ctx[1], h->drift_flags_ctx[2], h->tps_prev, h->descr_runs, h->descr_nruns, h->centre, h->anchor_pos, h->sym_ticket_ctx[0], h->sym_ticket_ctx[1], h->sym_ticket_ctx[2], h->tps_edges, h->trk_cp_a, h->trk_cp_b, h->trk_flags_ctx[0], h->trk_flags_ctx[1], h->trk_flags_ctx[2], h->trk_eps, h->d_iq, h->rs_iq, h->acq_carry, h->g_init, h->l_init, h->g_trk, h->l_trk, h->tps_state, h->acq_tap, h->fft_out, h->eq, h->tpsval,
+  void *all[] = {h->bd_log, h->bitdeint_lp, h->vit_codes, h->st_ctx[0], h->st_ctx[1], h->st_ctx[2], h->meta_ctx[0], h->meta_ctx[1], h->meta_ctx[2], h->tps_prev_snap[0], h->tps_prev_snap[1], h->tps_snap[0], h->tps_snap[1], h->csi, h->soft_a, h->soft_tab, h->soft_scratch, h->rs_defer, h->rs_sync, h->drift_mem, h->drift.delta, h->drift_flags_ctx[0], h->drift_flags_ctx[1], h->drift_flags_ctx[2], h->tps_prev, h->descr_runs, h->descr_nruns, h->centre, h->anchor_pos, h->sym_ticket_ctx[0], h->sym_ticket_ctx[1], h->sym_ticket_ctx[2], h->tps_edges, h->trk_cp_a, h->trk_cp_b, h->trk_flags_ctx[0], h->trk_flags_ctx[1], h->trk_flags_ctx[2], h->trk_eps, h->d_iq, h->rs_iq, h->acq_carry, h->g_init, h->l_init, h->g_trk, h->l_trk, h->tps_state, h->acq_tap, h->fft_out, h->eq, h->tpsval,
                  h->info, h->maj, h->sym_index, h->labels, h->symdeint_tap, h->bitdeint, h->vit, h->deint_tap, h->rs_out, h->ts_out};
   for (void *q : all) if (q) (void)hipFree(q);
   for (auto &ge : h->graphs) if (ge.exec) (void)hipGraphExecDestroy(ge.exec);
@@ -440,6 +463,8 @@
   RXHIP(hipMalloc((void **)&h->maj, sizeof(int) * C)); RXHIP(hipMalloc((void **)&h->sym_index, sizeof(int) * C));
   RXHIP(hipMalloc((void **)&h->bitdeint, C * P + 64));
   if (d.hierarchy != 0) RXHIP(hipMalloc((void **)&h->bitdeint_lp, C * P + 64));
+  h->vcp = make_vit_code_params(d.m, d.n, d.plen, h->vp.punct_mask, d.payload * d.m * d.k / d.n);
+  if (!p->soft_decision) RXHIP(hipMalloc((void **)&h->vit_codes, sizeof(uint32_t) * vit_code_dwords(C, h->vcp.sym_steps)));
   { int ncu = 256; (void)hipDeviceGetAttribute(&ncu, hipDeviceAttributeMultiprocessorCount, h->prm.device); h->sym_grid = s8_grid(ncu); h->ncu = ncu; }
   if (p->viterbi_verify != VIT_PLAIN && !p->soft_decision) {
     const long long mv = (long long)C * P * d.m * d.k / (8 * d.n) + 1;
@@ -478,7 +503,7 @@
   RXCHK(set_lds((const void *)symbol8k_kernel<true, false>, S8_LDS_BYTES)); RXCHK(set_lds((const void *)symbol8k_kernel<true, true>, S8_LDS_BYTES));
   RXCHK(set_lds((const void *)symbol2k_kernel<false, false>, S2_LDS_BYTES)); RXCHK(set_lds((const void *)symbol2k_kernel<false, true>, S2_LDS_BYTES));
   RXCHK(set_lds((const void *)symbol2k_kernel<true, false>, S2_LDS_BYTES)); RXCHK(set_lds((const void *)symbol2k_kernel<true, true>, S2_LDS_BYTES));
-  RXCHK(set_lds((const void *)inner_kernel<6>, inner_lds_bytes(P)));
+  RXCHK(set_lds((const void *)inner_kernel<6>, inner_code_lds_bytes(P)));
   RXCHK(set_lds((const void *)acq_anchor_kernel, acq_anchor_lds_bytes((int)N, d.cp)));
   RXCHK(set_lds((const void *)acq_small_kernel, (size_t)acq_small_cpc(d.cp) * 2 * (d.cp + 2 * ACQ_R) * sizeof(float2)));
   *out = h;
@@ -730,9 +755,11 @@
     hipLaunchKernelGGL(viterbi_soft4_kernel, dim3(grid), dim3(64 * S4_WAVES), 0, s, (const int8_t *)h->soft_a, h->vit + o.vit_off, (const RxState *)h->st, h->vp,
                        h->soft_scratch, sp.B, sp.nsteps);
   } else {
-  hipLaunchKernelGGL(inner_kernel<6>, dim3(C), dim3(INNER_THREADS), inner_lds_bytes((size_t)d.payload), s, (const float2 *)nullptr, (const uint8_t *)h->labels, ip,
+  const int codes_lp = (h->prm.hier_stream && h->bitdeint_lp) ? 1 : 0;
+  hipLaunchKernelGGL(inner_kernel<6>, dim3(C), dim3(INNER_THREADS), inner_code_lds_bytes((size_t)d.payload), s, (const float2 *)nullptr, (const uint8_t *)h->labels, ip,
                      (const RxState *)h->st, 0, (const int *)h->sym_index, (const float2 *)nullptr, (const unsigned char *)nullptr,
-                     (const uint16_t *)h->T.H, (const uint16_t *)h->T.Hinv, (uint8_t *)nullptr, h->symdeint_tap, h->bitdeint, h->bitdeint_lp);
+                     (const uint16_t *)h->T.H, (const uint16_t *)h->T.Hinv, (uint8_t *)nullptr, h->symdeint_tap, h->bitdeint, h->bitdeint_lp,
+                     h->vit_codes, h->vcp, codes_lp);
   { int r = join_front(); if (r) return r; }
   if (tmv) HIPCHK(hipEventRecord(h->ev[ST_VIT], s));
   VitParams vp = h->vp;
@@ -743,8 +770,7 @@
     if (max_vit / vp.chunk_bytes + 2 > h->vproof.cap) return fail(DVBT_ERR_CAPACITY, "Viterbi proof: state buffer too small for this segment's chunks");
     h->vit_checked = true;
   }
-  launch_viterbi(s, (const uint8_t *)((h->prm.hier_stream && h->bitdeint_lp) ? h->bitdeint_lp : h->bitdeint), h->vit + o.vit_off, (const RxState *)h->st, 0ll, vp, 0ll, 0ll, max_vit,
-                 proof ? &ax : nullptr, h->prm.viterbi_verify);
+  launch_viterbi_codes(s, (const uint32_t *)h->vit_codes, h->vit + o.vit_off, (const RxState *)h->st, 0ll, vp, 0ll, max_vit, proof ? &ax : nullptr, h->prm.viterbi_verify);
   }
   if (tmv) HIPCHK(hipEventRecord(h->ev[ST_RS], s));
   if (o.tail) { int r = enqueue_tail(h, s, max_vit / 204 + 1, -1); if (r) return r; }
diff --git a/gr_dvbt_amd/csrc/k_backend.hpp b/gr_dvbt_amd/csrc/k_backend.hpp
--- a/gr_dvbt_amd/csrc/k_backend.hpp
+++ b/gr_dvbt_amd/csrc/k_backend.hpp
@@ -2,6 +2,7 @@
 #include <hip/hip_runtime.h>
 #include <stdint.h>
 #include "k_frontend.hpp"
+#include "k_vit_codes.hpp"
 
 namespace dvbt {
 
@@ -55,7 +56,7 @@
 #ifndef DVBT_INNER_THREADS
 #define DVBT_INNER_THREADS 256
 #endif
-template <int VB> __device__ __forceinline__ void bit_deint_words(const uint8_t *v, uint8_t *o, int payload, int tid)
+template <int VB> __device__ __forceinline__ void bit_deint_words(const uint8_t *v, uint8_t *o, int payload, int tid, uint8_t *keep = nullptr)
 {
   constexpr int hv = VB / 2;
   const int nitems = (payload / 126) * 32;
@@ -75,10 +76,15 @@
     uint8_t *dst = o + blk * 126 + 4 * j;
     *reinterpret_cast<uint16_t *>(dst) = (uint16_t)val;
     if (j < 31) *reinterpret_cast<uint16_t *>(dst + 2) = (uint16_t)(val >> 16);
-  }
-}
-
-__device__ __forceinline__ void bit_deint_hier(const uint8_t *v, uint8_t *o_hp, uint8_t *o_lp, int payload, int m, int tid)
+    if (keep) {
+      uint8_t *kd = keep + blk * 126 + 4 * j;
+      *reinterpret_cast<uint16_t *>(kd) = (uint16_t)val;
+      if (j < 31) *reinterpret_cast<uint16_t *>(kd + 2) = (uint16_t)(val >> 16);
+    }
+  }
+}
+
+__device__ __forceinline__ void bit_deint_hier(const uint8_t *v, uint8_t *o_hp, uint8_t *o_lp, int payload, int m, int tid, uint8_t *keep = nullptr, int keep_lp = 0)
 {
   constexpr int offs[6] = {0, 63, 105, 42, 21, 84};
   for (int idx = tid; idx < payload; idx += DVBT_INNER_THREADS) {
@@ -94,6 +100,25 @@
     }
     o_hp[idx] = (uint8_t)hp;
     if (o_lp) o_lp[idx] = (uint8_t)lp;
+    if (keep) keep[idx] = (uint8_t)(keep_lp ? lp : hp);
+  }
+}
+
+__host__ __device__ inline size_t inner_code_lds_bytes(size_t payload) { return inner_lds_bytes(payload) + ((payload + 15) & ~(size_t)15) + ((payload * 6 / 8 + 15) & ~(size_t)15) + 16 + VC_PHASES_MAX * VC_PHASE_WORDS * 4; }
+__device__ __forceinline__ void emit_vit_codes(const uint8_t *db, unsigned *cb, uint32_t *codes, int payload, int u, int tid, const VitCodeParams &c)
+{
+  unsigned *tab = cb + (((payload * 6 / 8 + 15) & ~15) + 16) / 4;
+  if (tid < c.plen / 2) vit_code_phase(tid, c, tab + tid * VC_PHASE_WORDS);
+  for (int it = tid; it < payload / 8; it += DVBT_INNER_THREADS) vit_compact8(db, cb, it, c.m);
+  __syncthreads();
+  const long long g0 = (long long)u * c.sym_steps + VC_ORIGIN;
+  const int g0m = (int)(g0 & 7), nd = (g0m + c.sym_steps + 7) >> 3;
+  uint32_t *dst = codes + (g0 >> 3);
+  for (int d = tid; d < nd; d += DVBT_INNER_THREADS) {
+    int b_lo, b_hi;
+    const unsigned w = vit_code_dword(cb, d, g0m, c, tab, b_lo, b_hi);
+    if (b_hi - b_lo == 4) dst[d] = w;
+    else for (int b = b_lo; b < b_hi; b++) reinterpret_cast<uint8_t *>(dst + d)[b] = (uint8_t)(w >> (8 * b));
   }
 }
 
@@ -104,7 +129,8 @@
                                                    const float2 *__restrict__ points, const unsigned char *__restrict__ label_tab,
                                                    const uint16_t *__restrict__ H, const uint16_t *__restrict__ Hinv,
                                                    uint8_t *__restrict__ tap_demap, uint8_t *__restrict__ tap_symdeint,
-                                                   uint8_t *__restrict__ out, uint8_t *__restrict__ out_lp = nullptr)
+                                                   uint8_t *__restrict__ out, uint8_t *__restrict__ out_lp = nullptr,
+                                                   uint32_t *__restrict__ codes = nullptr, VitCodeParams cp = VitCodeParams{}, int codes_lp = 0)
 {
   extern __shared__ __attribute__((aligned(16))) unsigned char smem_raw[];
   uint8_t *v = smem_raw;
@@ -150,10 +176,16 @@
   uint8_t *o = out + (size_t)u * p.payload;
   if (tap_symdeint) for (int q = tid; q < p.payload; q += INNER_THREADS) tap_symdeint[(size_t)u * p.payload + q] = v[ipos(q)];
   if (!(mode & 4)) { for (int q = tid; q < p.payload; q += INNER_THREADS) o[q] = v[ipos(q)]; return; }
-  if (p.hier) bit_deint_hier(v, o, out_lp ? out_lp + (size_t)u * p.payload : nullptr, p.payload, p.m, tid);
-  else if (p.m == 2) bit_deint_words<2>(v, o, p.payload, tid);
-  else if (p.m == 4) bit_deint_words<4>(v, o, p.payload, tid);
-  else bit_deint_words<6>(v, o, p.payload, tid);
+  const bool emit = MODE == 6 && codes != nullptr;
+  uint8_t *db = emit ? smem_raw + inner_lds_bytes((size_t)p.payload) : nullptr;
+  if (p.hier) bit_deint_hier(v, o, out_lp ? out_lp + (size_t)u * p.payload : nullptr, p.payload, p.m, tid, db, codes_lp && out_lp);
+  else if (p.m == 2) bit_deint_words<2>(v, o, p.payload, tid, db);
+  else if (p.m == 4) bit_deint_words<4>(v, o, p.payload, tid, db);
+  else bit_deint_words<6>(v, o, p.payload, tid, db);
+  if (emit) {
+    __syncthreads();
+    emit_vit_codes(db, reinterpret_cast<unsigned *>(db + ((p.payload + 15) & ~15)), codes, p.payload, u, tid, cp);
+  }
 }
 
 struct VitParams {
diff --git a/gr_dvbt_amd/csrc/k_vit_codes.hpp b/gr_dvbt_amd/csrc/k_vit_codes.hpp
--- /dev/null
+++ b/gr_dvbt_amd/csrc/k_vit_codes.hpp
@@ -0,0 +1,125 @@
+#pragma once
+#include <stdint.h>
+#include <stddef.h>
+
+#if defined(__HIPCC__)
+#define VC_HD __host__ __device__
+#else
+#define VC_HD
+#endif
+
+namespace dvbt {
+
+constexpr int VC_ORIGIN = 18;
+constexpr int VC_SLACK_DWORDS = 2;
+static_assert(VC_ORIGIN % 8 == 2 && VC_ORIGIN >= 12 + 4, "blocks are whole dwords, a symbol's codes whole bytes; the front pad holds a straddling lane's read");
+static_assert(VC_SLACK_DWORDS >= 2, "the last lane's 8-byte read ends one dword behind the block; one more for the rounding of the origin shift");
+
+struct VitCodeParams {
+  int m, n, plen;
+  int sym_steps;
+  unsigned punct_mask;
+  unsigned magic_plen;
+  unsigned long long punct_rep;
+};
+inline VitCodeParams make_vit_code_params(int m, int n, int plen, unsigned punct_mask, int sym_steps)
+{
+  VitCodeParams c;
+  c.m = m; c.n = n; c.plen = plen; c.sym_steps = sym_steps; c.punct_mask = punct_mask;
+  c.magic_plen = (unsigned)((0x100000000ull + (unsigned)plen - 1) / (unsigned)plen);
+  c.punct_rep = 0;
+  for (int i = 0; i < 64; i++) c.punct_rep |= (unsigned long long)((punct_mask >> (i % plen)) & 1u) << i;
+  return c;
+}
+inline size_t vit_code_dwords(size_t symbols, int sym_steps) { return (symbols * (size_t)sym_steps + VC_ORIGIN + 7) / 8 + VC_SLACK_DWORDS; }
+
+VC_HD inline unsigned vc_popc(unsigned x)
+{
+#if defined(__HIP_DEVICE_COMPILE__)
+  return (unsigned)__popc(x);
+#else
+  return (unsigned)__builtin_popcount(x);
+#endif
+}
+VC_HD inline unsigned vc_brev(unsigned x)
+{
+#if defined(__HIP_DEVICE_COMPILE__)
+  return __brev(x);
+#else
+  x = (x >> 16) | (x << 16); x = ((x & 0xff00ff00u) >> 8) | ((x & 0x00ff00ffu) << 8); x = ((x & 0xf0f0f0f0u) >> 4) | ((x & 0x0f0f0f0fu) << 4);
+  x = ((x & 0xccccccccu) >> 2) | ((x & 0x33333333u) << 2); return ((x & 0xaaaaaaaau) >> 1) | ((x & 0x55555555u) << 1);
+#endif
+}
+
+VC_HD inline void vit_compact8(const uint8_t *db, unsigned *cb, int it, int m)
+{
+  const unsigned *dw = reinterpret_cast<const unsigned *>(db + 8 * it);
+  const unsigned mk = (1u << m) - 1;
+  const unsigned d0 = dw[0], d1 = dw[1];
+  const unsigned g0 = ((d0 & mk) << (3 * m)) | (((d0 >> 8) & mk) << (2 * m)) | (((d0 >> 16) & mk) << m) | ((d0 >> 24) & mk);
+  const unsigned g1 = ((d1 & mk) << (3 * m)) | (((d1 >> 8) & mk) << (2 * m)) | (((d1 >> 16) & mk) << m) | ((d1 >> 24) & mk);
+  uint16_t *hw = reinterpret_cast<uint16_t *>(cb);
+  if (m == 2) hw[it ^ 1] = (uint16_t)((g0 << 8) | g1);
+  else if (m == 4) cb[it] = (g0 << 16) | g1;
+  else { hw[(3 * it) ^ 1] = (uint16_t)(g0 >> 8); hw[(3 * it + 1) ^ 1] = (uint16_t)((g0 << 8) | (g1 >> 16)); hw[(3 * it + 2) ^ 1] = (uint16_t)g1; }
+}
+
+constexpr int VC_PHASE_WORDS = 12, VC_PHASES_MAX = 7;
+VC_HD inline void vit_code_phase(int p, const VitCodeParams &c, unsigned *t)
+{
+  const unsigned ph = 2u * (unsigned)p;
+  const unsigned km = (unsigned)(c.punct_rep >> ph) & 0xffffu;
+  unsigned acc = 0;
+  for (int j = 0; j < 8; j++) { t[j] = acc; acc += vc_popc((km >> (2 * j)) & 3u); }
+  unsigned K = km;
+  K = (K | (K << 8)) & 0x00ff00ffu; K = (K | (K << 4)) & 0x0f0f0f0fu; K = (K | (K << 2)) & 0x33333333u;
+  const unsigned e = K & 0x11111111u, o = (K >> 1) & 0x11111111u;
+  t[8] = K << 2;
+  t[9] = ((e | o) << 1) | (e & o);
+  t[10] = vc_popc(c.punct_mask & ((1u << ph) - 1u));
+  t[11] = 0;
+}
+
+VC_HD inline unsigned vit_codes8(const unsigned *cb, int i0, const VitCodeParams &c, const unsigned *tab)
+{
+  const unsigned x = 2u * (unsigned)i0;
+  const unsigned dq = (unsigned)(((unsigned long long)x * c.magic_plen) >> 32);
+  const unsigned ph = x - dq * (unsigned)c.plen;
+  const unsigned *t = tab + (ph >> 1) * VC_PHASE_WORDS;
+  const unsigned pos = dq * (unsigned)c.n + t[10];
+  const unsigned cw0 = cb[pos >> 5], cw1 = cb[(pos >> 5) + 1];
+  const unsigned win = vc_brev((unsigned)(((((unsigned long long)cw0) << 32) | cw1) >> (32 - (pos & 31))));
+  unsigned T = 0;
+  for (int j = 0; j < 8; j++) T = (T >> 4) | ((win >> t[j]) << 28);
+  T = ((T & 0x11111111u) << 1) | ((T >> 1) & 0x11111111u);
+  return t[8] | (T & t[9]);
+}
+
+VC_HD inline unsigned vit_code_dword(const unsigned *cb, int d, int g0mod8, const VitCodeParams &c, const unsigned *tab, int &b_lo, int &b_hi)
+{
+  const int i0 = 8 * d - g0mod8;
+  const int ic = i0 < 0 ? 0 : i0;
+  const int end = c.sym_steps - i0 < 8 ? c.sym_steps - i0 : 8;
+  b_lo = (ic - i0) >> 1; b_hi = end >> 1;
+  return vit_codes8(cb, ic, c, tab) << (4 * (ic - i0));
+}
+
+VC_HD inline long long vit_code_lane_dword(long long tb, int pl) { return ((tb + VC_ORIGIN) >> 3) + ((6 * pl) >> 2); }
+VC_HD inline int vit_code_lane_shift(int pl) { return 16 * (pl & 1); }
+VC_HD inline long long vit_code_clamp_dword(long long dw, long long total_steps)
+{
+  const long long dw_max = (total_steps + VC_ORIGIN) >> 3;
+  return dw < 0 ? 0 : dw > dw_max ? dw_max : dw;
+}
+VC_HD inline unsigned long long vit_code_lane_bits(unsigned lo, unsigned hi, int pl) { return ((((unsigned long long)hi) << 32) | lo) >> vit_code_lane_shift(pl); }
+
+VC_HD inline unsigned long long vit_code_keep(long long t, long long total_steps)
+{
+  const long long lo = t >= 0 ? 0 : -t < 12 ? -t : 12;
+  long long hi = total_steps - t; hi = hi < 0 ? 0 : hi > 12 ? 12 : hi;
+  if (hi < lo) hi = lo;
+  const unsigned long long below_hi = hi >= 12 ? 0xffffffffffffull : (1ull << (4 * hi)) - 1ull;
+  return below_hi & ~((1ull << (4 * lo)) - 1ull);
+}
+
+}
diff --git a/gr_dvbt_amd/csrc/k_viterbi3.hpp b/gr_dvbt_amd/csrc/k_viterbi3.hpp
--- a/gr_dvbt_amd/csrc/k_viterbi3.hpp
+++ b/gr_dvbt_amd/csrc/k_viterbi3.hpp
@@ -289,7 +289,9 @@
   }
 }
 
-template <int NTB, int WARM, int MODE, int NW>
+constexpr int V3_BYTES = 0, V3_CODES = 1;
+struct __attribute__((packed, aligned(4))) V3CodePair { unsigned x, y; };
+template <int NTB, int WARM, int MODE, int NW, int KIND>
 __device__ __forceinline__ void v3_decode(const uint8_t *__restrict__ in, uint8_t *__restrict__ out, long long total_steps, long long total_out, const VitParams &vp,
                                           long long in_base, long long out_lo, long long b0, bool dec_active, const V3Lds &S, const V3Lane &L, int (&v)[2], int (&endv)[2],
                                           int *own, int *predn, const int *inject, int *carry, int carry_rel)
@@ -325,9 +327,19 @@
     u_first = max(max(__builtin_amdgcn_readlane(first, 0), __builtin_amdgcn_readlane(first, 16)), max(__builtin_amdgcn_readlane(first, 32), __builtin_amdgcn_readlane(first, 48)));
     u_last = min(min(__builtin_amdgcn_readlane(last, 0), __builtin_amdgcn_readlane(last, 16)), min(__builtin_amdgcn_readlane(last, 32), __builtin_amdgcn_readlane(last, 48)));
   }
+  if (KIND == V3_CODES) { u_first = __builtin_amdgcn_readfirstlane(u_first); u_last = __builtin_amdgcn_readfirstlane(u_last); }
   auto pfx = [&](int ph) { return (int)__popc(vp.punct_mask & ((1u << ph) - 1u)); };
   int ph0 = 0, pf0 = 0, bo0 = 0, off = 0; long long byte0 = 0; uint4 q = make_uint4(0, 0, 0, 0);
+  static_assert(VC_ORIGIN % 8 == 2, "a block is whole dwords of the code stream: tb0 == 6 (mod 8)");
+  const long long cdw0 = vit_code_lane_dword(tb0, pl);
   auto stage_load = [&](int jb) {
+    if constexpr (KIND == V3_CODES) {
+      long long dw = cdw0 + jb;
+      if (jb < u_first || jb > u_last) dw = vit_code_clamp_dword(dw, total_steps);
+      q = make_uint4(0, 0, 0, 0);
+      if (dec_active) { const V3CodePair c2 = *reinterpret_cast<const V3CodePair *>(in + 4 * dw); q.x = c2.x; q.y = c2.y; }
+      return;
+    }
     const long long tb = tb0 + (long long)jb * 8;
     if (jb > 0 && jb - V3_BLK >= u_first) {
       const int pf_old = pf0;
@@ -363,6 +375,24 @@
     }
   };
   auto stage_words = [&](int jb) {
+    if constexpr (KIND == V3_CODES) {
+      constexpr int SPL = V3_BLK * 8 / 16;
+      static_assert(SPL == 12, "a lane's codes are 48 bits");
+      unsigned long long X = vit_code_lane_bits(q.x, q.y, pl);
+      if (jb < u_first || jb > u_last) X &= vit_code_keep(tb0 + (long long)jb * 8 + pl * SPL, dec_active ? total_steps : 0);
+      const unsigned xl = (unsigned)X, xh = (unsigned)(X >> 32);
+      const unsigned ev = (xl << 2) & 0x3c3c3c3cu, od = (xl >> 2) & 0x3c3c3c3cu, evh = (xh << 2) & 0x3c3cu, odh = (xh >> 2) & 0x3c3cu;
+      const unsigned a4[SPL] = {ev & 0xffu, od & 0xffu, (ev >> 8) & 0xffu, (od >> 8) & 0xffu, (ev >> 16) & 0xffu, (od >> 16) & 0xffu, ev >> 24, od >> 24,
+                                evh & 0xffu, odh & 0xffu, evh >> 8, odh >> 8};
+      unsigned sw[SPL];
+#pragma unroll
+      for (int i = 0; i < SPL; i++) sw[i] = *reinterpret_cast<const unsigned *>(reinterpret_cast<const unsigned char *>(lut) + a4[i]);
+      uint4 *const wdst = reinterpret_cast<uint4 *>(wbuf + dd * (V3_BLK * 8) + pl * SPL);
+#pragma unroll
+      for (int i = 0; i < SPL / 4; i++) wdst[i] = make_uint4(sw[4 * i], sw[4 * i + 1], sw[4 * i + 2], sw[4 * i + 3]);
+      __builtin_amdgcn_fence(__ATOMIC_SEQ_CST, "wavefront");
+      return;
+    }
     {
       const unsigned mk = (1u << m) - 1;
       auto grp = [&](unsigned d) { return ((d & mk) << (3 * m)) | (((d >> 8) & mk) << (2 * m)) | (((d >> 16) & mk) << m) | ((d >> 24) & mk); };
@@ -438,15 +468,17 @@
 
   stage_load(0);
   for (int jb = 0; jb < J; jb += V3_BLK) {
+    int jbo = jb;
+    asm("" : "+s"(jbo));
     if (MODE == 1 && dec_active) {
-      if (jb == warm) { if (inject) { v[0] = inject[0]; v[1] = inject[1]; } own[0] = v[0]; own[1] = v[1]; }
-      if (jb == warm + B) { predn[0] = v[0]; predn[1] = v[1]; }
-      if (carry && jb == warm + carry_rel) { carry[0] = v[0]; carry[1] = v[1]; }
+      if (jbo == warm) { if (inject) { v[0] = inject[0]; v[1] = inject[1]; } own[0] = v[0]; own[1] = v[1]; }
+      if (jbo == warm + B) { predn[0] = v[0]; predn[1] = v[1]; }
+      if (carry && jbo == warm + carry_rel) { carry[0] = v[0]; carry[1] = v[1]; }
     }
     if (MODE == 2) {
-      if (jb == 0 && dec_active) { own[0] = v[0]; own[1] = v[1]; }
-      if (jb == B) { endv[0] = v[0]; endv[1] = v[1]; }
-      if (carry && dec_active && jb == carry_rel) { carry[0] = v[0]; carry[1] = v[1]; }
+      if (jbo == 0 && dec_active) { own[0] = v[0]; own[1] = v[1]; }
+      if (jbo == B) { endv[0] = v[0]; endv[1] = v[1]; }
+      if (carry && dec_active && jbo == carry_rel) { carry[0] = v[0]; carry[1] = v[1]; }
     }
     bests_read(jb - V3_BLK, bb);
     if (!(V3_EXP & 8) || jb == 0) stage_words(jb);
@@ -485,8 +517,8 @@
 #define V3_LDS_DECL(NW) __shared__ V3Shared<NW> sh_;
 #define V3_LDS(NW, wv) V3Lds{sh_.tab, sh_.wbuf[wv], sh_.bests[wv], sh_.lut, wv}
 
-template <int NTB, int WARM = V3_WARM, int MODE = 0> __global__ __launch_bounds__(64 * V3_WGW) void viterbi3_kernel(const uint8_t *__restrict__ in, uint8_t *__restrict__ out, const RxState *st,
-                                                      long long steps_fixed, VitParams vp, V3Aux ax, long long in_base, long long out_lo)
+template <int NTB, int WARM, int MODE, int KIND> __device__ __forceinline__ void v3_kernel_body(const uint8_t *__restrict__ in, uint8_t *__restrict__ out, const RxState *st,
+                                                      long long steps_fixed, const VitParams &vp, const V3Aux &ax, long long in_base, long long out_lo)
 {
   V3_LDS_DECL(V3_WGW)
   const int wv = V3_WGW > 1 ? (int)(threadIdx.x >> 6) : 0;
@@ -515,7 +547,7 @@
     if (c == 0 && ax.carry_in) inject = ax.carry_in + 2 * pl;
     if (ax.carry_out && b0 + B >= total_out) carry = ax.carry_out + 2 * pl;
   }
-  v3_decode<NTB, WARM, MODE, V3_WGW>(in, out, total_steps, total_out, vp, in_base, out_lo, b0, dec_active, S, L, v, endv, own, predn, inject, carry, ax.carry_rel);
+  v3_decode<NTB, WARM, MODE, V3_WGW, KIND>(in, out, total_steps, total_out, vp, in_base, out_lo, b0, dec_active, S, L, v, endv, own, predn, inject, carry, ax.carry_rel);
 #if V3_EXP & 16
   if (lane == 0) {
     unsigned id, xcc;
@@ -525,6 +557,16 @@
     d[0] = (id & 0xffffu) | ((xcc & 0xfu) << 16); d[1] = dbg_t0; d[2] = wall_clock64();
   }
 #endif
+}
+template <int NTB, int WARM = V3_WARM, int MODE = 0> __global__ __launch_bounds__(64 * V3_WGW) void viterbi3_kernel(const uint8_t *__restrict__ in, uint8_t *__restrict__ out, const RxState *st,
+                                                      long long steps_fixed, VitParams vp, V3Aux ax, long long in_base, long long out_lo)
+{
+  v3_kernel_body<NTB, WARM, MODE, V3_CODES>(in, out, st, steps_fixed, vp, ax, in_base, out_lo);
+}
+template <int NTB, int WARM = V3_WARM, int MODE = 0> __global__ __launch_bounds__(64 * V3_WGW) void viterbi3_bytes_kernel(const uint8_t *__restrict__ in, uint8_t *__restrict__ out, const RxState *st,
+                                                      long long steps_fixed, VitParams vp, V3Aux ax, long long in_base, long long out_lo)
+{
+  v3_kernel_body<NTB, WARM, MODE, V3_BYTES>(in, out, st, steps_fixed, vp, ax, in_base, out_lo);
 }
 
 __device__ __forceinline__ long long v3_nchunks(long long total_out, long long grid0, int B) { return total_out > grid0 ? (total_out - grid0 + B - 1) / B : 0; }
@@ -565,7 +607,7 @@
   return ((ne >> (16 * dd)) & 0xffffull) == 0;
 }
 
-template <int NTB, int NW> __device__ __forceinline__ void v3_repair_rows(const uint8_t *__restrict__ in, uint8_t *__restrict__ out, long long total_steps, const VitParams &vp, const V3Aux &ax,
+template <int NTB, int NW, int KIND> __device__ __forceinline__ void v3_repair_rows(const uint8_t *__restrict__ in, uint8_t *__restrict__ out, long long total_steps, const VitParams &vp, const V3Aux &ax,
                                                                   long long in_base, long long out_lo, const V3Lds &S, const V3Lane &L, long long rows, long long row0, int n)
 {
   const int lane = threadIdx.x & 63, dd = lane >> 4, pl = lane & 15;
@@ -579,7 +621,7 @@
     int v[2], endv[2] = {0, 0};
     { const int *p = v3_pred(ax, c) + 2 * pl; v[0] = p[0]; v[1] = p[1]; }
     int *carry = (act && ax.carry_out && b0 + B >= total_out) ? ax.carry_out + 2 * pl : nullptr;
-    v3_decode<NTB, 0, 2, NW>(in, out, total_steps, total_out, vp, in_base, out_lo, b0, act && b0 < total_out, S, L, v, endv, v3_own(ax, c) + 2 * pl, nullptr, nullptr, carry, ax.carry_rel);
+    v3_decode<NTB, 0, 2, NW, KIND>(in, out, total_steps, total_out, vp, in_base, out_lo, b0, act && b0 < total_out, S, L, v, endv, v3_own(ax, c) + 2 * pl, nullptr, nullptr, carry, ax.carry_rel);
     int pn[2] = {endv[0], endv[1]};
     if (act && c + 1 < nch) { const int *p = v3_pred(ax, c + 1) + 2 * pl; pn[0] = p[0]; pn[1] = p[1]; }
     if (!v3_row_equal(endv, pn, dd) || ((ax.debug & 1) && act && c + 1 < nch)) {
@@ -589,8 +631,8 @@
     __builtin_amdgcn_fence(__ATOMIC_SEQ_CST, "wavefront");
   }
 }
-template <int NTB> __global__ __launch_bounds__(64 * V3_WGW) void viterbi_repair_kernel(const uint8_t *__restrict__ in, uint8_t *__restrict__ out, const RxState *st,
-                                                      long long steps_fixed, VitParams vp, V3Aux ax, long long in_base, long long out_lo)
+template <int NTB, int KIND> __device__ __forceinline__ void v3_repair_body(const uint8_t *__restrict__ in, uint8_t *__restrict__ out, const RxState *st,
+                                                      long long steps_fixed, const VitParams &vp, const V3Aux &ax, long long in_base, long long out_lo)
 {
   V3_LDS_DECL(V3_WGW)
   const int n = ax.ctl[V3_CTL_MISMATCH];
@@ -600,10 +642,20 @@
   const V3Lds S = V3_LDS(V3_WGW, wv);
   v3_init_lut(sh_.lut, threadIdx.x & 63);
   V3Lane L; v3_init_lane(threadIdx.x & 15, L);
-  v3_repair_rows<NTB, V3_WGW>(in, out, st ? st->n_vit_steps : steps_fixed, vp, ax, in_base, out_lo, S, L, rows, row0, n);
-}
-
-template <int NTB, int NW> __device__ __forceinline__ void v3_seq_walk(const uint8_t *__restrict__ in, uint8_t *__restrict__ out, long long total_steps, const VitParams &vp, const V3Aux &ax,
+  v3_repair_rows<NTB, V3_WGW, KIND>(in, out, st ? st->n_vit_steps : steps_fixed, vp, ax, in_base, out_lo, S, L, rows, row0, n);
+}
+template <int NTB> __global__ __launch_bounds__(64 * V3_WGW) void viterbi_repair_kernel(const uint8_t *__restrict__ in, uint8_t *__restrict__ out, const RxState *st,
+                                                      long long steps_fixed, VitParams vp, V3Aux ax, long long in_base, long long out_lo)
+{
+  v3_repair_body<NTB, V3_CODES>(in, out, st, steps_fixed, vp, ax, in_base, out_lo);
+}
+template <int NTB> __global__ __launch_bounds__(64 * V3_WGW) void viterbi_repair_bytes_kernel(const uint8_t *__restrict__ in, uint8_t *__restrict__ out, const RxState *st,
+                                                      long long steps_fixed, VitParams vp, V3Aux ax, long long in_base, long long out_lo)
+{
+  v3_repair_body<NTB, V3_BYTES>(in, out, st, steps_fixed, vp, ax, in_base, out_lo);
+}
+
+template <int NTB, int NW, int KIND> __device__ __forceinline__ void v3_seq_walk(const uint8_t *__restrict__ in, uint8_t *__restrict__ out, long long total_steps, const VitParams &vp, const V3Aux &ax,
                                                                long long in_base, long long out_lo, const V3Lds &S, const V3Lane &L, int force)
 {
   const int lane = threadIdx.x & 63, dd = lane >> 4, pl = lane & 15;
@@ -635,7 +687,7 @@
       int st0[2] = {v[0], v[1]}, endv[2] = {0, 0};
       if (act) { int *p = v3_pred(ax, c) + 2 * pl; p[0] = v[0]; p[1] = v[1]; }
       int *carry = (act && ax.carry_out && b0 + B >= total_out) ? ax.carry_out + 2 * pl : nullptr;
-      v3_decode<NTB, 0, 2, NW>(in, out, total_steps, total_out, vp, in_base, out_lo, b0, act, S, L, st0, endv, v3_own(ax, c) + 2 * pl, nullptr, nullptr, carry, ax.carry_rel);
+      v3_decode<NTB, 0, 2, NW, KIND>(in, out, total_steps, total_out, vp, in_base, out_lo, b0, act, S, L, st0, endv, v3_own(ax, c) + 2 * pl, nullptr, nullptr, carry, ax.carry_rel);
       __builtin_amdgcn_fence(__ATOMIC_SEQ_CST, "wavefront");
       done++;
       if (c + 1 >= nch) { pos = nch; break; }
@@ -648,19 +700,29 @@
   }
   if (lane == 0) { ax.ctl[V3_CTL_SEQ] = done; ax.ctl[V3_CTL_ACC + 2] += done; }
 }
-template <int NTB> __global__ __launch_bounds__(64) void viterbi_repair_seq_kernel(const uint8_t *__restrict__ in, uint8_t *__restrict__ out, const RxState *st,
-                                                      long long steps_fixed, VitParams vp, V3Aux ax, long long in_base, long long out_lo, int force)
+template <int NTB, int KIND> __device__ __forceinline__ void v3_repair_seq_body(const uint8_t *__restrict__ in, uint8_t *__restrict__ out, const RxState *st,
+                                                      long long steps_fixed, const VitParams &vp, const V3Aux &ax, long long in_base, long long out_lo, int force)
 {
   V3_LDS_DECL(1)
   const V3Lds S = V3_LDS(1, 0);
   v3_init_lut(sh_.lut, threadIdx.x & 63);
   V3Lane L; v3_init_lane(threadIdx.x & 15, L);
-  v3_seq_walk<NTB, 1>(in, out, st ? st->n_vit_steps : steps_fixed, vp, ax, in_base, out_lo, S, L, force);
+  v3_seq_walk<NTB, 1, KIND>(in, out, st ? st->n_vit_steps : steps_fixed, vp, ax, in_base, out_lo, S, L, force);
+}
+template <int NTB> __global__ __launch_bounds__(64) void viterbi_repair_seq_kernel(const uint8_t *__restrict__ in, uint8_t *__restrict__ out, const RxState *st,
+                                                      long long steps_fixed, VitParams vp, V3Aux ax, long long in_base, long long out_lo, int force)
+{
+  v3_repair_seq_body<NTB, V3_CODES>(in, out, st, steps_fixed, vp, ax, in_base, out_lo, force);
+}
+template <int NTB> __global__ __launch_bounds__(64) void viterbi_repair_seq_bytes_kernel(const uint8_t *__restrict__ in, uint8_t *__restrict__ out, const RxState *st,
+                                                      long long steps_fixed, VitParams vp, V3Aux ax, long long in_base, long long out_lo, int force)
+{
+  v3_repair_seq_body<NTB, V3_BYTES>(in, out, st, steps_fixed, vp, ax, in_base, out_lo, force);
 }
 
 constexpr long long V3_FIX_SMALL = 1024;
-template <int NTB> __global__ __launch_bounds__(64 * V3_WGW) void viterbi_fix_kernel(const uint8_t *__restrict__ in, uint8_t *__restrict__ out, const RxState *st,
-                                                      long long steps_fixed, VitParams vp, V3Aux ax, long long in_base, long long out_lo, int force)
+template <int NTB, int KIND> __device__ __forceinline__ void v3_fix_body(const uint8_t *__restrict__ in, uint8_t *__restrict__ out, const RxState *st,
+                                                      long long steps_fixed, const VitParams &vp, const V3Aux &ax, long long in_base, long long out_lo, int force)
 {
   V3_LDS_DECL(V3_WGW)
   const int wv = V3_WGW > 1 ? (int)(threadIdx.x >> 6) : 0;
@@ -676,9 +738,19 @@
   const V3Lds S = V3_LDS(V3_WGW, wv);
   v3_init_lut(sh_.lut, threadIdx.x & 63);
   V3Lane L; v3_init_lane(threadIdx.x & 15, L);
-  if (!force && n > 0) v3_repair_rows<NTB, V3_WGW>(in, out, total_steps, vp, ax, in_base, out_lo, S, L, 4 * V3_WGW, 4 * wv, n);
+  if (!force && n > 0) v3_repair_rows<NTB, V3_WGW, KIND>(in, out, total_steps, vp, ax, in_base, out_lo, S, L, 4 * V3_WGW, 4 * wv, n);
   __threadfence(); __syncthreads();
-  if (wv == 0) v3_seq_walk<NTB, V3_WGW>(in, out, total_steps, vp, ax, in_base, out_lo, S, L, force);
-}
-
-}
+  if (wv == 0) v3_seq_walk<NTB, V3_WGW, KIND>(in, out, total_steps, vp, ax, in_base, out_lo, S, L, force);
+}
+template <int NTB> __global__ __launch_bounds__(64 * V3_WGW) void viterbi_fix_kernel(const uint8_t *__restrict__ in, uint8_t *__restrict__ out, const RxState *st,
+                                                      long long steps_fixed, VitParams vp, V3Aux ax, long long in_base, long long out_lo, int force)
+{
+  v3_fix_body<NTB, V3_CODES>(in, out, st, steps_fixed, vp, ax, in_base, out_lo, force);
+}
+template <int NTB> __global__ __launch_bounds__(64 * V3_WGW) void viterbi_fix_bytes_kernel(const uint8_t *__restrict__ in, uint8_t *__restrict__ out, const RxState *st,
+                                                      long long steps_fixed, VitParams vp, V3Aux ax, long long in_base, long long out_lo, int force)
+{
+  v3_fix_body<NTB, V3_BYTES>(in, out, st, steps_fixed, vp, ax, in_base, out_lo, force);
+}
+
+}
```

After: 38590 (median of 6 runs). 1.03x the previous value.
